# Peterande/SAST

Hardware: AMD Instinct MI355X
Metric: frames/sec (B=4) SAST backbone fwd+bwd, 1Mpx 640x360 (higher is better)
Workload: dtype f32; 1 GPU; 1Mpx 640x360 (padded 384x640) full SAST backbone + PAFPN, fwd+bwd + AdamW, B=4/GPU, binary events (rand>0.5), random-init, AMP=0.0002; global_batch=4, seq_len=1, parallelism=dp1, hipgraph=True, library=sast_amd/libsast_hip.so, product_library=True, segmented_backward_overlap=False, deferred_weight_gradients=False, backward_cuts=3, dw_discard_TIMING_PROBE_gradients_invalid=False, collective_ranks=1, collective_ranks_verified=1, gradient_bytes_per_rank=67663616, sync_batchnorm=False, event_dtype=int32, grads_finite=True

## Files before the change

### include/sast_hip.h

```cpp
#ifndef SAST_HIP_H
#define SAST_HIP_H
#include <stddef.h>
#include <stdint.h>

#ifdef __cplusplus
extern "C" {
#endif

typedef void* sast_stream_t;

enum { SAST_DT_F32 = 0, SAST_DT_I32 = 1, SAST_DT_U8 = 2, SAST_DT_I64 = 3, SAST_DT_I16 = 4, SAST_DT_I8 = 5 };

int sast_version(void);
int sast_mfma_split3(void);

int sast_nzratio(const void* x, int dtype, int B, int Cin, int H, int W, int32_t* cnt_ws, float* r, sast_stream_t stream);
int sast_nzratio_padded(const void* x, int dtype, int B, int Cin, int H, int W, int Hp, int Wp, int32_t* cnt_ws, float* r,
                        sast_stream_t stream);

int sast_input_prep(const void* x, int dtype, int B, int C, int H, int W, int Hp, int Wp, int32_t* ws, float* r, float* y,
                    sast_stream_t stream);
int sast_input_prep_flag(const void* x, int dtype, int B, int C, int H, int W, int Hp, int Wp, int32_t* ws, float* r, float* y,
                         uint32_t* nonexact, sast_stream_t stream);
int sast_input_prep_u8(const uint8_t* x, int B, int C, int H, int W, int Hp, int Wp, int32_t* ws, float* r, uint8_t* y, sast_stream_t stream);

int sast_nchw_to_nhwc(const void* x, int dtype, int B, int C, int H, int W, float* y, sast_stream_t stream);
int sast_nchw_to_nhwc_padded(const void* x, int dtype, int B, int C, int H, int W, int Hp, int Wp, float* y, sast_stream_t stream);
int sast_nhwc_to_nchw(const float* x, int B, int C, int H, int W, float* y, sast_stream_t stream);

int sast_add_rows(const float* x, const float* table, float* y, int rows, int C, int table_rows, sast_stream_t stream);

#define SAST_MEAN_SQUARE_BLOCKS 128
int sast_mean_square_fwd(const float* const* x, const size_t* n, int count, float* partials, sast_stream_t stream);
int sast_mean_square_bwd(const float* const* x, const size_t* n, int count, const float* d_partials, int d_stride, float* const* dx,
                         sast_stream_t stream);
int sast_mask_token_fwd(float* x, const uint8_t* mask, const float* token, const float* pos_emb, int rows, int C, int L, sast_stream_t stream);
int sast_mask_token_bwd(const float* dy, const uint8_t* mask, float* dx, float* d_token, int rows, int C, sast_stream_t stream);

typedef struct SastDownArgs {
  int32_t B, H, W, Cin, Cout, factor;
  const float* x;
  const float* w;
  const float* ln_w; const float* ln_b;
  const float* pe;
  float* conv_out;
  float* mean; float* rstd;
  float* y;
  const float* dy; float* dx;
  float* dw; float* d_ln_w; float* d_ln_b;
  float* ws;
  int32_t x_dtype;
  int32_t no_overlap;
  const uint32_t* x_nonexact;
} SastDownArgs;
int sast_downsample_ln_fwd(const SastDownArgs* a, sast_stream_t stream);
int sast_downsample_ln_bwd(const SastDownArgs* a, sast_stream_t stream);

typedef struct SastScoreArgs {
  int32_t B, L, C, r_stride;
  float amp;
  const float* xp;
  const float* r;
  const float* ws_w; const float* ws_b;
  const float* wc;
  float* scale;
  float* s;
  float* xw;
  float* tok;
  const float* dxw; float* dxp;
  float* d_ws_w; float* d_ws_b; float* d_wc;
  float* ws;
  float* dscale_ws;
} SastScoreArgs;
int sast_score_stp_fwd(const SastScoreArgs* a, sast_stream_t stream);
int sast_score_stp_bwd(const SastScoreArgs* a, sast_stream_t stream);

typedef struct SastSel {
  int32_t* win_keep;
  uint64_t* mask;
  int32_t* K;
  int32_t* row_off;
  int32_t* win_rank;
  int32_t* counts;
  int32_t* tok_slot;
  int32_t* row_tok;
  int32_t* pack_rows;
  int32_t* row_seg;
} SastSel;
int sast_select_packs(const SastSel* sel, int W, int T, sast_stream_t stream);
// ... 30 lines not shown
  float* d_act_w;
} SastMswsaArgs;
size_t sast_mswsa_fused_ws_floats(int C, int inner, int T, int dim_head, int cb_tps);
size_t sast_mswsa_raw_ws_floats(int C, int inner);
size_t sast_mswsa_bwd_ws_floats(int rows, int C, int inner);
int sast_mswsa_fwd(const SastMswsaArgs* a, sast_stream_t stream);
int sast_mswsa_bwd(const SastMswsaArgs* a, sast_stream_t stream);

typedef struct SastLstmArgs {
  int32_t B, L, C;
  const float* x; const float* h0; const float* c0;
  const float* w; const float* b;
  float* h1; float* c1;
  float* gates;
  const float* dh1; const float* dc1;
  float* dx; float* dh0; float* dc0;
  float* dw; float* db;
  float* ws;
  const float* dh1b;
  const float* drop;
} SastLstmArgs;
int sast_lstm_fwd(const SastLstmArgs* a, sast_stream_t stream);
int sast_lstm_bwd(const SastLstmArgs* a, sast_stream_t stream);

int sast_dwconv_fwd(const float* x, const float* w, const float* b, float* y, int B, int H, int W, int C, int k, sast_stream_t stream);
int sast_dwconv_bwd(const float* x, const float* w, const float* dy, float* dx, float* dw, float* db, int B, int H, int W, int C, int k,
                    sast_stream_t stream);

#define SAST_BN_STAT_COPIES 4
#define SAST_BN_WS_FLOATS(Cout) ((4 * SAST_BN_STAT_COPIES + 2 * SAST_BN_STAT_COPIES) * (Cout))
int sast_conv_bn_ws_floats(int Cout);
typedef struct SastConvBnArgs {
  int32_t B, H, W, Cin, Cout, ksize, stride, training;
  int32_t ldx, ldy, lddy, lddx;
  int32_t bn_ws_zeroed;
  int32_t bn_red_done;
  int32_t Cin1, ldx2;
  float momentum, eps;
  const float* x; const float* w; const float* bn_w; const float* bn_b;
  float* run_mean; float* run_var;
  float* conv_out;
  float* stats;
  float* y;
  const float* dy; float* dx; float* dw; float* d_bn_w; float* d_bn_b;
  float* bn_ws;
  float* ws;
  const float* x2;
  float* dx2;
  const float* p_conv_out; const float* p_stats; const float* p_bn_w; const float* p_bn_b; float* p_bn_ws;
  const float* p2_conv_out; const float* p2_stats; const float* p2_bn_w; const float* p2_bn_b; float* p2_bn_ws;
  const float* dy2;
  int32_t sync_phase, m_total;
  int32_t groups;
} SastConvBnArgs;
int sast_conv_bn_silu_fwd(const SastConvBnArgs* a, sast_stream_t stream);
int sast_conv_bn_silu_bwd(const SastConvBnArgs* a, sast_stream_t stream);

typedef struct SastConvBn2Args {
  int32_t B, H, W, Cin, Cout, ldx, Cin1, ldx2;
  int32_t bn_ws_zeroed, bn_red_done0, bn_red_done1;
  int32_t training;
  int32_t ksize;
  float momentum0, momentum1, eps0, eps1;
  const float* x; const float* x2;
  const float* w0; const float* w1; const float* bn_w0; const float* bn_w1; const float* bn_b0; const float* bn_b1;
  float* run_mean0; float* run_mean1; float* run_var0; float* run_var1;
  float* conv_out0; float* conv_out1; float* stats0; float* stats1; float* y0; float* y1; float* bn_ws0; float* bn_ws1;
  const float* dy0; const float* dy1; float* dw0; float* dw1; float* d_bn_w0; float* d_bn_w1; float* d_bn_b0; float* d_bn_b1;
  float* ws0; float* ws1;
  float* dx; float* dx2;
  const float* p_conv_out; const float* p_stats; const float* p_bn_w; const float* p_bn_b; float* p_bn_ws;
  const float* p2_conv_out; const float* p2_stats; const float* p2_bn_w; const float* p2_bn_b; float* p2_bn_ws;
} SastConvBn2Args;
int sast_conv_bn_silu2_fwd(const SastConvBn2Args* a, sast_stream_t stream);
int sast_conv_bn_silu2_bwd(const SastConvBn2Args* a, sast_stream_t stream);

int sast_upsample_cat_fwd(const float* a, const float* b, float* out, int B, int H, int W, int C1, int C2, sast_stream_t stream);
int sast_upsample_cat_bwd(const float* dout, float* da, float* db, int B, int H, int W, int C1, int C2, sast_stream_t stream);
int sast_cat2_fwd(const float* a, const float* b, float* out, int rows, int C1, int C2, sast_stream_t stream);
int sast_cat2_bwd(const float* dout, float* da, float* db, int rows, int C1, int C2, sast_stream_t stream);

typedef struct SastHeadGeom {
  int32_t n_levels;
  int32_t H[4], W[4];
  float stride[4];
} SastHeadGeom;
int sast_head_pred_fwd(const float* reg_feat, const float* cls_feat, const float* w_reg, const float* b_reg, const float* w_obj,
                       const float* b_obj, const float* w_cls, const float* b_cls, float* pred, float* train, int B, int H, int W, int hidden,
                       int num_classes, float stride, int anchor_offset, int anchors_total, int decode, sast_stream_t stream);
int sast_head_pred_decode(const float* reg_feat, const float* cls_feat, const float* w_reg, const float* b_reg, const float* w_obj,
                          const float* b_obj, const float* w_cls, const float* b_cls, float* out, int B, int H, int W, int hidden,
                          int num_classes, float stride, int anchor_offset, int anchors_total, int decode, sast_stream_t stream);
int sast_head_pred_bwd(const float* draw, const float* reg_feat, const float* cls_feat, const float* w_reg, const float* w_obj,
                       const float* w_cls, float* d_reg_feat, float* d_cls_feat, float* dw_reg, float* db_reg, float* dw_obj, float* db_obj,
                       float* dw_cls, float* db_cls, int B, int H, int W, int hidden, int num_classes, int anchor_offset, int anchors_total,
                       sast_stream_t stream);
size_t sast_yolox_loss_ws_bytes(int B, int anchors_total, int max_labels);
int sast_yolox_loss(const float* train_out, const float* labels, const SastHeadGeom* geom, int B, int max_labels, int num_classes, int use_l1,
                    float* losses, float* draw, int32_t* fg_mask, int32_t* matched_gt, float* matched_iou, void* ws, sast_stream_t stream);

size_t sast_postprocess_ws_bytes(int B, int anchors_total);
int sast_postprocess(const float* prediction, int B, int anchors_total, int num_classes, float conf_thre, float nms_thre, int class_agnostic,
                     float* out, int32_t* n_out, void* ws, sast_stream_t stream);

#define SAST_GATHER_MAX_SRC 32
#define SAST_GATHER_MAX_OUT 256
typedef struct {
  int32_t n_src, n_out, B, _pad;
  size_t sample_floats;
  const float* src[SAST_GATHER_MAX_SRC];
  float* dsrc[SAST_GATHER_MAX_SRC];
  float* out;
  uint8_t t_of[SAST_GATHER_MAX_OUT], b_of[SAST_GATHER_MAX_OUT];
} SastSampleGather;
int sast_gather_samples(const SastSampleGather* a, sast_stream_t stream);
int sast_gather_samples_bwd(const SastSampleGather* a, sast_stream_t stream);
typedef struct { uint8_t sel[256]; } SastSampleMask;
int sast_zero_samples(float* x, int B, size_t sample_floats, const SastSampleMask* sel, sast_stream_t stream);

int sast_adamw(float* p, const float* g, float* m, float* v, size_t n,
               const float* lr_step ,
               double beta1, double beta2, float eps, float weight_decay, float grad_scale,
               float clip_value , sast_stream_t stream);
int sast_adamw_onecycle(float* p, const float* g, float* m, float* v, size_t n, float* lr_step, double beta1, double beta2, float eps,
                        float weight_decay, float grad_scale, float clip_value, double initial_lr, double max_lr, double min_lr,
                        double end1, double end2, sast_stream_t stream);

int sast_dw_defer(int on);
int sast_dw_defer_rows(long min_rows, long max_rows);
int sast_dw_pending(void);
int sast_dw_discard(void);
// ... 178 lines not shown
```

### sast_amd/_lib.py

```python
from __future__ import annotations

import ctypes as C
import os
import re

_HERE = os.path.dirname(os.path.abspath(__file__))
DEFAULT_LIB_PATH = os.path.join(_HERE, "libsast_hip.so")
LIB_PATH = os.environ.get("SAST_LIB_PATH") or DEFAULT_LIB_PATH
HEADER_PATH = os.path.join(os.path.dirname(_HERE), "include", "sast_hip.h")

P = C.c_void_p
I32 = C.c_int32
F32 = C.c_float

DT_F32, DT_I32, DT_U8, DT_I64, DT_I16, DT_I8 = 0, 1, 2, 3, 4, 5
EVENT_WINDOW_DURATION, EVENT_WINDOW_COUNT = 0, 1
EVENT_SCAN_BLOCKS = 512
EVQUEUE_DT_DAT = 6
AUGMENT_PARAM_WORDS = 16
AUGMENT_NONE, AUGMENT_ZOOM_IN, AUGMENT_ZOOM_OUT = 0, 1, 2
EVAL_STATE_WORDS, EVAL_MAX_CLASSES = 32, 4
EVAL_IOU_THRS, EVAL_REC_THRS, EVAL_AREAS = 10, 101, 4
(LABELS_UNSORTED, LABELS_NEGATIVE_SIZE, LABELS_NO_LABELS, LABELS_BAD_RATE, LABELS_NO_ALIGNED_LABEL, LABELS_ZERO_COUNT, LABELS_TOO_MANY_FRAMES,
 LABELS_TOO_MANY_WINDOWS, LABELS_FRAME_OVERFULL, LABELS_FRAMES_TOO_CLOSE, LABELS_WINDOW_INDEX) = (1 << k for k in range(11))


def _struct(name, spec):
    fields = []
    for ct, names in spec:
        for n in names.split():
            fields.append((n, ct))
    return type(name, (C.Structure,), {"_fields_": fields})


SastDownArgs = _struct("SastDownArgs", [
    (I32, "B H W Cin Cout factor"),
    (P, "x w ln_w ln_b pe conv_out mean rstd y dy dx dw d_ln_w d_ln_b ws"),
    (I32, "x_dtype no_overlap"),
    (P, "x_nonexact"),
])
SastScoreArgs = _struct("SastScoreArgs", [
    (I32, "B L C r_stride"), (F32, "amp"),
    (P, "xp r ws_w ws_b wc scale s xw tok dxw dxp d_ws_w d_ws_b d_wc ws dscale_ws"),
])
SastSel = _struct("SastSel", [(P, "win_keep mask K row_off win_rank counts tok_slot row_tok pack_rows row_seg")])
SastMswsaArgs = _struct("SastMswsaArgs", [
    (I32, "B H W C ph pw mode inner"), (F32, "eps"), (I32, "cb_tps dim_head mlp_act"),
    (P, "xin out"), (SastSel, "sel"),
    (P, "ln1_w ln1_b ln2_w ln2_b qkv_w qkv_b proj_w proj_b ls1 fc1_w fc1_b fc2_w fc2_b ls2"),
    (P, "mean1 rstd1 mean2 rstd2 S QKV O lse Y UG Hh"),
    (P, "dout dxin"),
    (P, "d_ln1_w d_ln1_b d_ln2_w d_ln2_b d_qkv_w d_qkv_b d_proj_w d_proj_b d_ls1 d_fc1_w d_fc1_b d_fc2_w d_fc2_b d_ls2"),
    (P, "ws cb_m cb_sum raw_ws drop1 drop2 drop_ws drop_mlp fused_ws act_w d_act_w"),
])
SastConvBn2Args = _struct("SastConvBn2Args", [
    (I32, "B H W Cin Cout ldx Cin1 ldx2 bn_ws_zeroed bn_red_done0 bn_red_done1 training ksize"), (F32, "momentum0 momentum1 eps0 eps1"),
    (P, "x x2 w0 w1 bn_w0 bn_w1 bn_b0 bn_b1 run_mean0 run_mean1 run_var0 run_var1 conv_out0 conv_out1 stats0 stats1 y0 y1 "
        "bn_ws0 bn_ws1 dy0 dy1 dw0 dw1 d_bn_w0 d_bn_w1 d_bn_b0 d_bn_b1 ws0 ws1 dx dx2 "
        "p_conv_out p_stats p_bn_w p_bn_b p_bn_ws p2_conv_out p2_stats p2_bn_w p2_bn_b p2_bn_ws"),
])
SastHeadGeom = _struct("SastHeadGeom", [(I32, "n_levels"), (I32 * 4, "H"), (I32 * 4, "W"), (F32 * 4, "stride")])
SastLstmArgs = _struct("SastLstmArgs", [
    (I32, "B L C"),
    (P, "x h0 c0 w b h1 c1 gates dh1 dc1 dx dh0 dc0 dw db ws dh1b drop"),
])
SastConvBnArgs = _struct("SastConvBnArgs", [
    (I32, "B H W Cin Cout ksize stride training ldx ldy lddy lddx bn_ws_zeroed bn_red_done Cin1 ldx2"), (F32, "momentum eps"),
    (P, "x w bn_w bn_b run_mean run_var conv_out stats y dy dx dw d_bn_w d_bn_b bn_ws ws x2 dx2 "
        "p_conv_out p_stats p_bn_w p_bn_b p_bn_ws p2_conv_out p2_stats p2_bn_w p2_bn_b p2_bn_ws dy2"),
    (I32, "sync_phase m_total groups"),
])

SastSampleGather = _struct("SastSampleGather", [
    (I32, "n_src n_out B _pad"), (C.c_size_t, "sample_floats"), (P * 32, "src"), (P * 32, "dsrc"), (P, "out"),
    (C.c_uint8 * 256, "t_of"), (C.c_uint8 * 256, "b_of"),
])
SastSampleMask = _struct("SastSampleMask", [(C.c_uint8 * 256, "sel")])
SastEventArgs = _struct("SastEventArgs", [
    (P, "x y p t bounds out err ws"), (C.c_int64, "capacity window_capacity"),
    (I32, "x_dtype y_dtype p_dtype t_dtype B bins height width count_cutoff fastmode downsample_by_2 clip_negative_polarity"),
])
SastMdStackArgs = _struct("SastMdStackArgs", [
    (P, "x y p t bounds out err ws"), (C.c_int64, "capacity window_capacity"),
    (I32, "x_dtype y_dtype p_dtype t_dtype B bins height width count_cutoff downsample_by_2 clip_negative_polarity"),
])
SastEvQueueArgs = _struct("SastEvQueueArgs", [
    (P, "x y p t head count t_last retired retired_t err ws"), (C.c_int64, "capacity"), (I32, "S reserved"),
])
SastLabelArgs = _struct("SastLabelArgs", [
    (P, "ws ends_us n_windows frame_ts_us n_frames frame_2_window window_2_frame labels frame_start frame_count status"),
    (C.c_int64, "capacity base_delta_us align_t_us delta_t_us"), (I32, "S width height class_max"), (F32, "min_diag2 min_side max_width"),
    (I32, "reprs_per_frame downsample_by_2 max_frames max_windows max_labels_per_frame reserved"),
])
SastEvalArgs = _struct("SastEvalArgs", [
    (P, "labels counts det n_det"), (I32, "N M A K"), (F32, "min_diag2 min_side"), (I32, "max_images max_labels_per_frame"),
    (C.c_int64, "max_detections"),
    (P, "state info gt_box gt_cls gt_img img_t det_box det_cls det_img rec_key rec_match rec_ign iou_thr rec_thr sorted sort_ws"),
    (C.c_size_t, "sort_ws_bytes"), (P, "precision result"),
])

_SIGNATURES = {
    "sast_version": (C.c_int, []),
    "sast_mfma_split3": (C.c_int, []),
    "sast_nzratio": (C.c_int, [P, C.c_int, C.c_int, C.c_int, C.c_int, C.c_int, P, P, P]),
    "sast_nchw_to_nhwc": (C.c_int, [P, C.c_int, C.c_int, C.c_int, C.c_int, C.c_int, P, P]),
    "sast_nzratio_padded": (C.c_int, [P, C.c_int, C.c_int, C.c_int, C.c_int, C.c_int, C.c_int, C.c_int, P, P, P]),
    "sast_nchw_to_nhwc_padded": (C.c_int, [P, C.c_int, C.c_int, C.c_int, C.c_int, C.c_int, C.c_int, C.c_int, P, P]),
    "sast_nhwc_to_nchw": (C.c_int, [P, C.c_int, C.c_int, C.c_int, C.c_int, P, P]),
    "sast_input_prep": (C.c_int, [P] + [C.c_int] * 7 + [P, P, P, P]),
    "sast_input_prep_flag": (C.c_int, [P] + [C.c_int] * 7 + [P, P, P, P, P]),
    "sast_input_prep_u8": (C.c_int, [P] + [C.c_int] * 6 + [P, P, P, P]),
    "sast_add_rows": (C.c_int, [P, P, P, C.c_int, C.c_int, C.c_int, P]),
    "sast_mean_square_fwd": (C.c_int, [P, P, C.c_int, P, P]),
    "sast_mean_square_bwd": (C.c_int, [P, P, C.c_int, P, C.c_int, P, P]),
    "sast_downsample_ln_fwd": (C.c_int, [C.POINTER(SastDownArgs), P]),
    "sast_downsample_ln_bwd": (C.c_int, [C.POINTER(SastDownArgs), P]),
    "sast_score_stp_fwd": (C.c_int, [C.POINTER(SastScoreArgs), P]),
    "sast_score_stp_bwd": (C.c_int, [C.POINTER(SastScoreArgs), P]),
    "sast_select": (C.c_int, [P, C.c_int, C.c_int, C.c_int, C.c_int, C.c_int, C.c_int, C.c_double, C.POINTER(SastSel), P]),
    "sast_select_packs": (C.c_int, [C.POINTER(SastSel), C.c_int, C.c_int, P]),
    "sast_head_pred_decode": (C.c_int, [P] * 9 + [C.c_int] * 5 + [C.c_float, C.c_int, C.c_int, C.c_int, P]),
    "sast_head_pred_fwd": (C.c_int, [P] * 10 + [C.c_int] * 5 + [C.c_float, C.c_int, C.c_int, C.c_int, P]),
    "sast_head_pred_bwd": (C.c_int, [P] * 14 + [C.c_int] * 7 + [P]),
    "sast_postprocess_ws_bytes": (C.c_size_t, [C.c_int, C.c_int]),
    "sast_postprocess": (C.c_int, [P, C.c_int, C.c_int, C.c_int, C.c_float, C.c_float, C.c_int, P, P, P, P]),
    "sast_yolox_loss_ws_bytes": (C.c_size_t, [C.c_int, C.c_int, C.c_int]),
    "sast_yolox_loss": (C.c_int, [P, P, C.POINTER(SastHeadGeom), C.c_int, C.c_int, C.c_int, C.c_int, P, P, P, P, P, P, P]),
    "sast_mask_token_fwd": (C.c_int, [P, P, P, P, C.c_int, C.c_int, C.c_int, P]),
    "sast_mask_token_bwd": (C.c_int, [P, P, P, P, C.c_int, C.c_int, P]),
    "sast_select_pair": (C.c_int, [P, C.c_int, C.c_int, C.c_int, C.c_int, C.c_int, C.c_double, C.POINTER(SastSel), C.POINTER(SastSel), P]),
    "sast_mswsa_bwd_ws_floats": (C.c_size_t, [C.c_int, C.c_int, C.c_int]),
    "sast_mswsa_raw_ws_floats": (C.c_size_t, [C.c_int, C.c_int]),
    "sast_mswsa_fused_ws_floats": (C.c_size_t, [C.c_int] * 5),
    "sast_mswsa_fwd": (C.c_int, [C.POINTER(SastMswsaArgs), P]),
    "sast_mswsa_bwd": (C.c_int, [C.POINTER(SastMswsaArgs), P]),
    "sast_lstm_fwd": (C.c_int, [C.POINTER(SastLstmArgs), P]),
    "sast_lstm_bwd": (C.c_int, [C.POINTER(SastLstmArgs), P]),
    "sast_dwconv_fwd": (C.c_int, [P, P, P, P] + [C.c_int] * 5 + [P]),
    "sast_dwconv_bwd": (C.c_int, [P, P, P, P, P, P] + [C.c_int] * 5 + [P]),
    "sast_conv_bn_ws_floats": (C.c_int, [C.c_int]),
    "sast_conv_bn_silu_fwd": (C.c_int, [C.POINTER(SastConvBnArgs), P]),
    "sast_conv_bn_silu_bwd": (C.c_int, [C.POINTER(SastConvBnArgs), P]),
    "sast_conv_bn_silu2_fwd": (C.c_int, [C.POINTER(SastConvBn2Args), P]),
    "sast_conv_bn_silu2_bwd": (C.c_int, [C.POINTER(SastConvBn2Args), P]),
    "sast_upsample_cat_fwd": (C.c_int, [P, P, P, C.c_int, C.c_int, C.c_int, C.c_int, C.c_int, P]),
    "sast_upsample_cat_bwd": (C.c_int, [P, P, P, C.c_int, C.c_int, C.c_int, C.c_int, C.c_int, P]),
    "sast_cat2_fwd": (C.c_int, [P, P, P, C.c_int, C.c_int, C.c_int, P]),
    "sast_cat2_bwd": (C.c_int, [P, P, P, C.c_int, C.c_int, C.c_int, P]),
    "sast_gather_samples": (C.c_int, [C.POINTER(SastSampleGather), P]),
    "sast_gather_samples_bwd": (C.c_int, [C.POINTER(SastSampleGather), P]),
    "sast_zero_samples": (C.c_int, [P, C.c_int, C.c_size_t, C.POINTER(SastSampleMask), P]),
    "sast_adamw_onecycle": (C.c_int, [P, P, P, P, C.c_size_t, P, C.c_double, C.c_double, F32, F32, F32, F32, C.c_double, C.c_double, C.c_double,
                                      C.c_double, C.c_double, P]),
    "sast_dw_defer": (C.c_int, [C.c_int]),
    "sast_dw_defer_rows": (C.c_int, [C.c_long, C.c_long]),
    "sast_dw_pending": (C.c_int, []),
    "sast_dw_discard": (C.c_int, []),
    "sast_dw_flush": (C.c_int, [P]),
    "sast_launch_count": (C.c_ulonglong, []),
    "sast_config_reload": (C.c_int, []),
    "sast_config_get": (C.c_int, [C.c_char_p, C.c_int]),
    "sast_config_report": (C.c_size_t, [C.c_char_p, C.c_size_t]),
    "sast_prof_enable": (C.c_int, [C.c_int]),
    "sast_prof_calibrate": (C.c_float, [P, C.c_int]),
    "sast_prof_report": (C.c_size_t, [C.c_char_p, C.c_size_t]),
    "sast_adamw": (C.c_int, [P, P, P, P, C.c_size_t, P, C.c_double, C.c_double, F32, F32, F32, F32, P]),
    "sast_event_correct_time": (C.c_int, [P, C.c_int, P, C.c_int64, P, P, P, P]),
    "sast_event_window_bounds": (C.c_int, [P, P, C.c_int64, P, C.c_int, C.c_int, C.c_int64, P, P]),
    "sast_event_frames_ws_bytes": (C.c_size_t, [C.c_int] * 5 + [C.c_int64]),
    "sast_event_frames": (C.c_int, [C.POINTER(SastEventArgs), P]),
    "sast_mdstack_frames_ws_bytes": (C.c_size_t, [C.c_int] * 5 + [C.c_int64]),
    "sast_mdstack_frames": (C.c_int, [C.POINTER(SastMdStackArgs), P]),
    "sast_evstreams_ws_count": (C.c_size_t, [C.c_int]),
    "sast_evstreams_correct_time": (C.c_int, [P, C.c_int, P, C.c_int, C.c_int64, P, P, P, P, P]),
    "sast_evstreams_window_bounds": (C.c_int, [P, P, C.c_int, C.c_int64, P, C.c_int, C.c_int, C.c_int64, P, P]),
    "sast_evqueue_ws_count": (C.c_size_t, [C.c_int]),
    "sast_evqueue_push": (C.c_int, [C.POINTER(SastEvQueueArgs), P, P, P, P, C.c_int, C.c_int, C.c_int, C.c_int, P, C.c_int64, P, P]),
    "sast_evqueue_window_bounds": (C.c_int, [C.POINTER(SastEvQueueArgs), P, C.c_int, C.c_int, C.c_int64, P, P]),
    "sast_evqueue_retire": (C.c_int, [C.POINTER(SastEvQueueArgs), P, C.c_int, P]),
    "sast_labels_ws_bytes": (C.c_size_t, [C.c_int, C.c_int64, C.c_int]),
    "sast_labels_load": (C.c_int, [C.POINTER(SastLabelArgs), P, P, P, P]),
    "sast_labels_gather": (C.c_int, [C.POINTER(SastLabelArgs), P, C.c_int, P, P, P, P, P]),
    "sast_augment_frames": (C.c_int, [P, P, P] + [C.c_int] * 5 + [P]),
    "sast_augment_labels": (C.c_int, [P, P, P] + [C.c_int] * 4 + [P, P, P, P]),
    "sast_eval_reset": (C.c_int, [C.POINTER(SastEvalArgs), P]),
    "sast_eval_add": (C.c_int, [C.POINTER(SastEvalArgs), P]),
    "sast_eval_sort_ws_bytes": (C.c_size_t, [C.c_int64]),
    "sast_eval_accumulate": (C.c_int, [C.POINTER(SastEvalArgs), P]),
}

_lib = None


def declared_symbols():
    with open(HEADER_PATH) as f:
        src = f.read()
    return sorted(set(re.findall(r"\b(sast_[a-z0-9_]+)\s*\(", src)))


# ... 57 lines not shown
```

### sast_amd/csrc/gemm.cuh

```cuda
#pragma once
#include <type_traits>
#include <hip/hip_ext.h>
#include "common.cuh"
#include "../../include/sast_hip.h"

#if defined(SAST_TL_ENABLE) && !defined(SAST_TL)
static __device__ unsigned long long sast_tl_buf[8 * 8192];
#define SAST_TL(k)                                                                                          \
  do {                                                                                                      \
    const unsigned bid_ = blockIdx.x;                                                                       \
    if (threadIdx.x == 0 && bid_ < 8192) sast_tl_buf[bid_ * 8 + (k)] = wall_clock64();                      \
    if (threadIdx.x == 0 && bid_ < 8192 && (k) == 0) sast_tl_buf[bid_ * 8 + 7] = __smid();                 \
  } while (0)
#define SAST_TL_JOB(j) do { if (threadIdx.x == 0 && blockIdx.x < 8192) sast_tl_buf[blockIdx.x * 8 + 6] = (j); } while (0)
#endif
#ifndef SAST_TL
#define SAST_TL(k)
#endif
#ifndef SAST_TL_JOB
#define SAST_TL_JOB(j)
#endif
#ifndef SAST_TLF
#define SAST_TLF_DECL
#define SAST_TLF(k)
// ... 1480 lines not shown
};
struct EpStoreStats2 {
  static constexpr bool COLSTATS = true;
  float* c1; float* c2; int C; double* sums1; double* sums2;
  using Col = EpNone; using Aux = EpNone;
  __device__ __forceinline__ Col col(int) const { return Col{}; }
  __device__ __forceinline__ Aux pre(int, int) const { return Aux{}; }
  __device__ __forceinline__ void post(int m, int j, const float (&v)[1], const Col&, const Aux&) const {
    if (j < C) c1[(size_t)m * C + j] = v[0];
    else c2[(size_t)m * C + (j - C)] = v[0];
  }
  __device__ __forceinline__ void stat(float v, const Col&, const Aux&, float& a, float& b) const { a += v; b += v * v; }
  __device__ __forceinline__ void flush(int copy, int j, int, float s, float q) const {
    double* sp = (j < C ? sums1 : sums2) + (size_t)copy * 2 * C;
    const int jj = j < C ? j : j - C;
    atomicAdd(sp + jj, (double)s); atomicAdd(sp + C + jj, (double)q);
  }
};
struct EpAtomic2 {
  float* c1; float* c2; int ldc; int M1;
  using Col = EpNone; using Aux = EpNone;
  __device__ __forceinline__ Col col(int) const { return Col{}; }
  __device__ __forceinline__ Aux pre(int, int) const { return Aux{}; }
  __device__ __forceinline__ void post(int m, int j, const float (&v)[1], const Col&, const Aux&) const {
    atomicAdd((m < M1 ? c1 + (size_t)m * ldc : c2 + (size_t)(m - M1) * ldc) + j, v[0]);
  }
};
struct EpAtomic {
  float* c; int ldc;
  using Col = EpNone; using Aux = EpNone;
  __device__ __forceinline__ Col col(int) const { return Col{}; }
  __device__ __forceinline__ Aux pre(int, int) const { return Aux{}; }
  __device__ __forceinline__ void post(int m, int j, const float (&v)[1], const Col&, const Aux&) const {
    atomicAdd(c + (size_t)m * ldc + j, v[0]);
  }
};

struct EpStoreClass {
  float* c; int ldc; int H, W; ConvDxClasses k;
  using Col = EpNone;
  struct Aux { int p; };
  __device__ __forceinline__ Col col(int) const { return Col{}; }
  __device__ __forceinline__ Aux pre(int m, int) const {
    const int cls = fast_div(m, k.Mc, k.mc_mul), ic = m - cls * k.Mc;
    const int t = fast_div(ic, k.Wc, k.wc_mul), xx = ic - t * k.Wc, b = fast_div(t, k.Hc, k.hc_mul), yy = t - b * k.Hc;
    const int q = 3 - cls;
    return Aux{(b * H + 2 * yy + (q >> 1)) * W + 2 * xx + (q & 1)};
  }
  __device__ __forceinline__ void post(int, int j, const float (&v)[1], const Col&, const Aux& a) const {
    c[(size_t)a.p * ldc + j] = v[0];
  }
};

struct EpSplit2BnRed {
  static constexpr bool COLSTATS = true;
  float* a; float* b; int C1, C2; BnProducer pa, pb;
  using Col = BnCol;
  struct Aux { float x; };
  __device__ __forceinline__ Col col(int j) const {
    if (j < C1) return pa.x ? bn_col(pa, j) : BnCol{0.f, 0.f, 0.f, 0.f};
    return pb.x ? bn_col(pb, j - C1) : BnCol{0.f, 0.f, 0.f, 0.f};
  }
  __device__ __forceinline__ Aux pre(int m, int j) const {
    if (j < C1) return Aux{pa.x ? pa.x[(size_t)m * C1 + j] : 0.f};
    return Aux{pb.x ? pb.x[(size_t)m * C2 + (j - C1)] : 0.f};
  }
  __device__ __forceinline__ void post(int m, int j, const float (&v)[1], const Col&, const Aux&) const {
    if (j < C1) a[(size_t)m * C1 + j] = v[0];
    else if (b) b[(size_t)m * C2 + (j - C1)] = v[0];
  }
  __device__ __forceinline__ void stat(float v, const Col& k, const Aux& x, float& s, float& q) const { bn_stat(v, x.x, k, s, q); }
  __device__ __forceinline__ void flush(int copy, int j, int, float s, float q) const {
    if (j < C1) {
      if (pa.x) { float* sp = pa.sums + (size_t)copy * 2 * C1; atomicAdd(sp + j, s); atomicAdd(sp + C1 + j, q); }
    } else if (pb.x) {
      float* sp = pb.sums + (size_t)copy * 2 * C2; atomicAdd(sp + (j - C1), s); atomicAdd(sp + C2 + (j - C1), q);
    }
  }
};

struct EpSplit2 {
  float* a; float* b; int C1, C2;
  using Col = EpNone; using Aux = EpNone;
  __device__ __forceinline__ Col col(int) const { return Col{}; }
  __device__ __forceinline__ Aux pre(int, int) const { return Aux{}; }
  __device__ __forceinline__ void post(int m, int j, const float (&v)[1], const Col&, const Aux&) const {
    if (j < C1) a[(size_t)m * C1 + j] = v[0];
    else if (b) b[(size_t)m * C2 + (j - C1)] = v[0];
  }
};

}
```

### sast_amd/csrc/k_block.hip

```cpp
#include <cstdlib>
#include "gemm_dispatch.cuh"
#include "kernels.h"

using namespace sast;

namespace {

constexpr int ATTN_MAX_T = 256;

struct EpBiasRelu {
  float* c; int ldc; const float* bias;
  struct Col { float b; };
  using Aux = EpNone;
  __device__ __forceinline__ Col col(int j) const { return Col{bias[j]}; }
  __device__ __forceinline__ Aux pre(int, int) const { return Aux{}; }
  __device__ __forceinline__ void post(int m, int j, const float (&v)[1], const Col& k, const Aux&) const {
    c[(size_t)m * ldc + j] = fmaxf(v[0] + k.b, 0.f);
  }
};
struct EpBiasReluCtl : EpBiasRelu {
  static constexpr bool SIDE = true;
  ControlsJob k; int side_blocks;
  __device__ __forceinline__ void side(int sb) const { if (threadIdx.x < 256) controls_fwd_elem(k, sb * 256 + threadIdx.x); }
};
// ... 150 lines not shown
extern "C" {

int sast_version(void) { SAST_ENTRY(); return 100; }
int sast_mfma_split3(void) { SAST_ENTRY(); return SAST_MFMA_BF16 ? 2 : SAST_MFMA_SPLIT3; }

int sast_nzratio(const void* x, int dtype, int B, int Cin, int H, int W, int32_t* cnt_ws, float* r, sast_stream_t stream) { SAST_ENTRY();
  if (!x || !cnt_ws || !r || H % 32 || W % 32) return SAST_EINVAL;
  return nzr_dispatch(x, dtype, cnt_ws, r, B, Cin, H, W, H, W, (hipStream_t)stream);
}
int sast_nzratio_padded(const void* x, int dtype, int B, int Cin, int H, int W, int Hp, int Wp, int32_t* cnt_ws, float* r,
                        sast_stream_t stream) { SAST_ENTRY();
  if (!x || !cnt_ws || !r || Hp % 32 || Wp % 32 || H > Hp || W > Wp || H % 4 || W % 4) return SAST_EINVAL;
  return nzr_dispatch(x, dtype, cnt_ws, r, B, Cin, H, W, Hp, Wp, (hipStream_t)stream);
}
int sast_nchw_to_nhwc(const void* x, int dtype, int B, int C, int H, int W, float* y, sast_stream_t stream) { SAST_ENTRY();
  return nchw_to_nhwc_dispatch(x, dtype, y, B, C, H, W, H, W, (hipStream_t)stream);
}
int sast_nchw_to_nhwc_padded(const void* x, int dtype, int B, int C, int H, int W, int Hp, int Wp, float* y, sast_stream_t stream) { SAST_ENTRY();
  if (!x || !y || H > Hp || W > Wp) return SAST_EINVAL;
  return nchw_to_nhwc_dispatch(x, dtype, y, B, C, H, W, Hp, Wp, (hipStream_t)stream);
}
int sast_input_prep(const void* x, int dtype, int B, int C, int H, int W, int Hp, int Wp, int32_t* ws, float* r, float* y, sast_stream_t stream) { SAST_ENTRY();
  if (!x || !ws || !r || !y || H > Hp || W > Wp || H % 4 || W % 4 || Hp % 32 || Wp % 32 || C != 20 || ((Hp / 32) * (Wp / 32)) % 2) return SAST_EINVAL;
  return input_prep_dispatch(x, dtype, y, ws, r, B, C, H, W, Hp, Wp, (hipStream_t)stream);
}
int sast_input_prep_flag(const void* x, int dtype, int B, int C, int H, int W, int Hp, int Wp, int32_t* ws, float* r, float* y, uint32_t* nonexact,
                         sast_stream_t stream) { SAST_ENTRY();
  if (!x || !ws || !r || !y || !nonexact || H > Hp || W > Wp || H % 4 || W % 4 || Hp % 32 || Wp % 32 || C != 20 || ((Hp / 32) * (Wp / 32)) % 2) return SAST_EINVAL;
  return input_prep_dispatch(x, dtype, y, ws, r, B, C, H, W, Hp, Wp, (hipStream_t)stream, nonexact);
}
int sast_input_prep_u8(const uint8_t* x, int B, int C, int H, int W, int Hp, int Wp, int32_t* ws, float* r, uint8_t* y, sast_stream_t stream) { SAST_ENTRY();
  if (!x || !ws || !r || !y || H > Hp || W > Wp || H % 4 || W % 4 || Hp % 32 || Wp % 32 || C != 20 || ((Hp / 32) * (Wp / 32)) % 2) return SAST_EINVAL;
  return input_prep_u8(x, y, ws, r, B, C, H, W, Hp, Wp, (hipStream_t)stream);
}
int sast_nhwc_to_nchw(const float* x, int B, int C, int H, int W, float* y, sast_stream_t stream) { SAST_ENTRY();
  return nhwc_to_nchw_launch(x, y, B, C, H * W, (hipStream_t)stream);
}

int sast_add_rows(const float* x, const float* table, float* y, int rows, int C, int table_rows, sast_stream_t stream) { SAST_ENTRY();
  if (C % 4) return SAST_EINVAL;
  return add_rows_launch(x, table, y, rows, C, table_rows, (hipStream_t)stream);
}

int sast_mean_square_fwd(const float* const* x, const size_t* n, int count, float* partials, sast_stream_t stream) { SAST_ENTRY();
  if (!x || !n || !partials || count < 1 || count > 4) return SAST_EINVAL;
  for (int t = 0; t < count; ++t) if (!x[t] || n[t] % 4) return SAST_EINVAL;
  return mean_square_launch(x, nullptr, n, count, SAST_MEAN_SQUARE_BLOCKS, partials, nullptr, 1, (hipStream_t)stream);
}
int sast_mean_square_bwd(const float* const* x, const size_t* n, int count, const float* d_partials, int d_stride, float* const* dx,
                         sast_stream_t stream) { SAST_ENTRY();
  if (!x || !n || !d_partials || !dx || count < 1 || count > 4 || (d_stride != 0 && d_stride != 1)) return SAST_EINVAL;
  for (int t = 0; t < count; ++t) if (!x[t] || !dx[t] || n[t] % 4) return SAST_EINVAL;
  return mean_square_launch(x, dx, n, count, SAST_MEAN_SQUARE_BLOCKS, nullptr, d_partials, d_stride, (hipStream_t)stream);
}

int sast_mask_token_fwd(float* x, const uint8_t* mask, const float* token, const float* pos_emb, int rows, int C, int L, sast_stream_t stream) { SAST_ENTRY();
  if (!x || !mask || !token || C % 4 || L < 1) return SAST_EINVAL;
  return mask_token_fwd_launch(x, mask, token, pos_emb, rows, C, L, (hipStream_t)stream);
}
int sast_gather_samples(const SastSampleGather* a, sast_stream_t stream) { SAST_ENTRY();
  if (!a || !a->out || a->n_src < 1 || a->n_src > SAST_GATHER_MAX_SRC || a->n_out < 0 || a->n_out > SAST_GATHER_MAX_OUT || a->sample_floats % 4) return SAST_EINVAL;
  for (int j = 0; j < a->n_out; ++j) if (a->t_of[j] >= a->n_src || a->b_of[j] >= a->B || !a->src[a->t_of[j]]) return SAST_EINVAL;
  if (a->n_out == 0) return SAST_OK;
  return sample_gather_launch(*a, false, (hipStream_t)stream);
}
int sast_gather_samples_bwd(const SastSampleGather* a, sast_stream_t stream) { SAST_ENTRY();
  if (!a || a->n_src < 1 || a->n_src > SAST_GATHER_MAX_SRC || a->n_out < 0 || a->n_out > SAST_GATHER_MAX_OUT || a->B < 1 || a->B > 256 ||
      a->sample_floats % 4 || (a->n_out && !a->out)) return SAST_EINVAL;
  for (int t = 0; t < a->n_src; ++t) if (!a->dsrc[t]) return SAST_EINVAL;
  return sample_gather_launch(*a, true, (hipStream_t)stream);
}
int sast_zero_samples(float* x, int B, size_t sample_floats, const SastSampleMask* sel, sast_stream_t stream) { SAST_ENTRY();
  if (!x || !sel || B < 1 || B > 256 || sample_floats % 4) return SAST_EINVAL;
  return zero_samples_launch(x, B, sample_floats, *sel, (hipStream_t)stream);
}
int sast_mask_token_bwd(const float* dy, const uint8_t* mask, float* dx, float* d_token, int rows, int C, sast_stream_t stream) { SAST_ENTRY();
  if (!dy || !mask || !dx || !d_token || C % 4) return SAST_EINVAL;
  return mask_token_bwd_launch(dy, mask, dx, d_token, rows, C, (hipStream_t)stream);
}

int sast_select(const float* tok, int B, int H, int W, int ph, int pw, int mode, double bounce, const SastSel* s,
                sast_stream_t stream) { SAST_ENTRY();
  if (!tok || !s) return SAST_EINVAL;
  const int N = (H / ph) * (W / pw), T = ph * pw;
  const float thr_w = (float)((1.0 / N) / (1.0 + bounce));
  const float thr_t = (float)((1.0 / T) / (1.0 + bounce));
  return select_launch(tok, B, H, W, ph, pw, mode, thr_w, thr_t, s, (hipStream_t)stream);
}
int sast_select_packs(const SastSel* s, int W, int T, sast_stream_t stream) { SAST_ENTRY();
  if (!s || !s->K || !s->row_off || !s->pack_rows || !s->row_seg || W < 1 || T < 1 || T > ATTN_MAX_T) return SAST_EINVAL;
  return select_packs_launch(s, W, T, (hipStream_t)stream);
}

int sast_select_pair(const float* tok, int B, int H, int W, int ph, int pw, double bounce, const SastSel* win, const SastSel* grid,
                     sast_stream_t stream) { SAST_ENTRY();
  if (!tok || !win || !grid) return SAST_EINVAL;
  const int N = (H / ph) * (W / pw), T = ph * pw;
  const float thr_w = (float)((1.0 / N) / (1.0 + bounce));
  const float thr_t = (float)((1.0 / T) / (1.0 + bounce));
  return select_pair_launch(tok, B, H, W, ph, pw, thr_w, thr_t, win, grid, (hipStream_t)stream);
}

int sast_score_stp_fwd(const SastScoreArgs* a, sast_stream_t stream) { SAST_ENTRY();
  hipStream_t st = (hipStream_t)stream;
  ProfScope ps_("score_fwd", a ? a->C : 0, a ? a->B * a->L : 0, st);
  if (!a || a->C % 4) return SAST_EINVAL;
// ... 243 lines not shown
```

### sast_amd/csrc/k_conv.hip

```cpp
#include <cstdlib>
#include "gemm_dispatch.cuh"
#include "kernels.h"

using namespace sast;

namespace {

inline double bn_unbias(long M) { return M > 1 ? (double)M / (double)(M - 1) : 1.0; }
struct BnFwdJob {
  const float* x; const double* sums; float* run_mean; float* run_var; float* stats; const float* gamma; const float* beta;
  float* y; int ldy; float momentum, eps;
};
__global__ __launch_bounds__(256) void bn_silu_apply_kernel(BnFwdJob j0, BnFwdJob j1, double invM, double unbias, size_t n4, int C, int training, int iters,
                                                            unsigned c4_mul) {
  SAST_KERNARG_WARM_SELF(bn_silu_apply_kernel);
  const BnFwdJob& jb = blockIdx.y == 0 ? j0 : j1;
  const float* __restrict__ x = jb.x; const double* __restrict__ sums = jb.sums;
  float* __restrict__ run_mean = jb.run_mean; float* __restrict__ run_var = jb.run_var; float* __restrict__ stats = jb.stats;
  const float* __restrict__ gamma = jb.gamma; const float* __restrict__ beta = jb.beta; float* __restrict__ y = jb.y;
  const int ldy = jb.ldy; const float momentum = jb.momentum, eps = jb.eps;
  extern __shared__ float bn_sm[];
  const int c4 = C / 4;
  const size_t e0 = (size_t)blockIdx.x * 256 * iters + threadIdx.x;
#ifndef SAST_BN_EARLY_LOADS
#define SAST_BN_EARLY_LOADS 0
#endif
  float4 v0 = zero4(), g0 = zero4(), b0 = zero4();
  size_t m0 = 0; int cc0 = 0;
  if (SAST_BN_EARLY_LOADS) {
    const size_t ec = e0 < n4 ? e0 : 0;
    m0 = fast_div((int)ec, c4, c4_mul); cc0 = (int)(ec - m0 * c4) * 4;
    v0 = ld4(x + m0 * C + cc0); g0 = ld4(gamma + cc0); b0 = ld4(beta + cc0);
  }
  for (int c = threadIdx.x; c < C; c += 256) {
    float mu, rs;
    if (training) {
      double sk[BN_STAT_COPIES], qk[BN_STAT_COPIES];
#pragma unroll
      for (int k = 0; k < BN_STAT_COPIES; ++k) { sk[k] = sums[(size_t)k * 2 * C + c]; qk[k] = sums[(size_t)k * 2 * C + C + c]; }
      double s = 0.0, q = 0.0;
#pragma unroll
      for (int k = 0; k < BN_STAT_COPIES; ++k) { s += sk[k]; q += qk[k]; }
      const double mean = s * invM;
      double var = q * invM - mean * mean;
      if (var < 0) var = 0;
      mu = (float)mean;
#if SAST_FAST_DIV
      rs = rsqrt_hw((float)var + eps);
#else
      rs = (float)(1.0 / sqrt(var + (double)eps));
#endif
      if (blockIdx.x == 0 && run_mean) {
        const double unb = var * unbias;
        run_mean[c] = (1.f - momentum) * run_mean[c] + momentum * (float)mean;
        run_var[c] = (1.f - momentum) * run_var[c] + momentum * (float)unb;
      }
    } else {
      mu = run_mean[c];
      rs = rsqrt_hw(run_var[c] + eps);
    }
    if (blockIdx.x == 0) { stats[c] = mu; stats[C + c] = rs; }
    bn_sm[c] = mu; bn_sm[C + c] = rs;
  }
  __syncthreads();
  for (int it = 0; it < iters; ++it) {
    const size_t e = e0 + (size_t)it * 256;
    if (e >= n4) return;
    size_t m; int c; float4 v, g, b;
    if (SAST_BN_EARLY_LOADS && it == 0) { m = m0; c = cc0; v = v0; g = g0; b = b0; }
    else { m = fast_div((int)e, c4, c4_mul); c = (int)(e - m * c4) * 4; v = ld4(x + m * C + c); g = ld4(gamma + c); b = ld4(beta + c); }
    const float4 mu = *(const float4*)(bn_sm + c), rs = *(const float4*)(bn_sm + C + c);
    float4 z = make_float4((v.x - mu.x) * rs.x * g.x + b.x, (v.y - mu.y) * rs.y * g.y + b.y, (v.z - mu.z) * rs.z * g.z + b.z,
                           (v.w - mu.w) * rs.w * g.w + b.w);
    z.x *= sigmoid_hw(z.x); z.y *= sigmoid_hw(z.y); z.z *= sigmoid_hw(z.z); z.w *= sigmoid_hw(z.w);
    st4(y + m * ldy + c, z);
  }
}
struct EpBnSilu {
  float* y; int ldy; const float* run_mean; const float* run_var; const float* gamma; const float* beta; float eps;
  struct Col { float mu, rs, g, b; };
  using Aux = EpNone;
  __device__ __forceinline__ Col col(int j) const { return Col{run_mean[j], 1.0f / sqrtf(run_var[j] + eps), gamma[j], beta[j]}; }
  __device__ __forceinline__ Aux pre(int, int) const { return Aux{}; }
  __device__ __forceinline__ void post(int m, int j, const float (&v)[1], const Col& k, const Aux&) const {
    const float z = (v[0] - k.mu) * k.rs * k.g + k.b;
    y[(size_t)m * ldy + j] = z * sigmoid_hw(z);
  }
};
struct EpBnSilu2 {
  float* y0; float* y1; int C; const float* rm0; const float* rv0; const float* g0; const float* b0; float eps0;
  const float* rm1; const float* rv1; const float* g1; const float* b1; float eps1;
  struct Col { float mu, rs, g, b; };
  using Aux = EpNone;
  __device__ __forceinline__ Col col(int j) const {
    return j < C ? Col{rm0[j], 1.0f / sqrtf(rv0[j] + eps0), g0[j], b0[j]} : Col{rm1[j - C], 1.0f / sqrtf(rv1[j - C] + eps1), g1[j - C], b1[j - C]};
  }
  __device__ __forceinline__ Aux pre(int, int) const { return Aux{}; }
  __device__ __forceinline__ void post(int m, int j, const float (&v)[1], const Col& k, const Aux&) const {
    const float z = (v[0] - k.mu) * k.rs * k.g + k.b;
    (j < C ? y0 + (size_t)m * C + j : y1 + (size_t)m * C + (j - C))[0] = z * sigmoid_hw(z);
  }
};
__global__ __launch_bounds__(256) void bn_stats_kernel(const float* __restrict__ x, int M, int C, double* __restrict__ sums,
                                                       int rows_per_block) {
  extern __shared__ double redd[];
  const int c4n = C / 4;
  const int RP = 256 / c4n > 0 ? 256 / c4n : 1;
  const int r0 = blockIdx.x * rows_per_block, r1 = min(M, r0 + rows_per_block);
  for (int cq = threadIdx.x % min(c4n, 256); cq < c4n; cq += 256) {
    const int rl = threadIdx.x / c4n, c = cq * 4;
    double s[4] = {0, 0, 0, 0}, q[4] = {0, 0, 0, 0};
    if (rl < RP) {
      for (int r = r0 + rl; r < r1; r += RP) {
        const float4 v = ld4(x + (size_t)r * C + c);
        s[0] += v.x; s[1] += v.y; s[2] += v.z; s[3] += v.w;
        q[0] += (double)v.x * v.x; q[1] += (double)v.y * v.y; q[2] += (double)v.z * v.z; q[3] += (double)v.w * v.w;
      }
#pragma unroll
      for (int e = 0; e < 4; ++e) { redd[((rl * C) + c + e) * 2] = s[e]; redd[((rl * C) + c + e) * 2 + 1] = q[e]; }
    }
    __syncthreads();
    if (rl == 0) {
#pragma unroll
      for (int e = 0; e < 4; ++e) {
        double a = s[e], b = q[e];
        for (int k = 1; k < RP; ++k) { a += redd[((k * C) + c + e) * 2]; b += redd[((k * C) + c + e) * 2 + 1]; }
        atomicAdd(sums + c + e, a);
        atomicAdd(sums + C + c + e, b);
// ... 109 lines not shown
  }
}
__global__ __launch_bounds__(256) void bn_publish_affine_kernel(const float* __restrict__ sums, float* __restrict__ dgamma, float* __restrict__ dbeta, int C) {
  const int c = blockIdx.x * 256 + threadIdx.x;
  if (c >= C) return;
  float s1 = 0.f, s2 = 0.f;
#pragma unroll
  for (int k = 0; k < BN_STAT_COPIES; ++k) { s1 += sums[(size_t)k * 2 * C + c]; s2 += sums[(size_t)k * 2 * C + C + c]; }
  dbeta[c] += s1;
  dgamma[c] += s2;
}
template <class IDX>
__global__ __launch_bounds__(256) void upsample_cat_fwd_kernel(const float* __restrict__ a, const float* __restrict__ b,
                                                               float* __restrict__ out, int H, int W, int C1, int C2, size_t n4) {
  const size_t e64 = (size_t)blockIdx.x * 256 + threadIdx.x;
  if (e64 >= n4) return;
  const IDX e = (IDX)e64;
  const int Ct = C1 + C2;
  const IDX c4n = (IDX)(Ct / 4);
  const IDX row = e / c4n; const int c = (int)(e - row * c4n) * 4;
  float4 v;
  if (c < C1) {
    const IDX W2 = (IDX)(2 * W), H2 = (IDX)(2 * H);
    const IDX t = row / W2; const int x = (int)(row - t * W2); const IDX bb = t / H2; const int y = (int)(t - bb * H2);
    v = ld4(a + (((size_t)bb * H + (y >> 1)) * W + (x >> 1)) * C1 + c);
  } else {
    v = ld4(b + (size_t)row * C2 + (c - C1));
  }
  st4(out + (size_t)row * Ct + c, v);
}
template <class IDX>
__global__ __launch_bounds__(256) void upsample_cat_bwd_kernel(const float* __restrict__ dout, float* __restrict__ da, float* __restrict__ db,
                                                               int H, int W, int C1, int Ct, size_t n4, size_t n4b) {
  const size_t e64 = (size_t)blockIdx.x * 256 + threadIdx.x;
  if (e64 >= n4) {
    const size_t eb64 = e64 - n4;
    if (eb64 >= n4b) return;
    const IDX eb = (IDX)eb64;
    const int C2 = Ct - C1;
    const IDX c4b = (IDX)(C2 / 4);
    const IDX row = eb / c4b; const int c = (int)(eb - row * c4b) * 4;
    st4(db + (size_t)row * C2 + c, ld4(dout + (size_t)row * Ct + C1 + c));
    return;
  }
  const IDX e = (IDX)e64;
  const IDX c4n = (IDX)(C1 / 4);
  const IDX row = e / c4n; const int c = (int)(e - row * c4n) * 4;
  const IDX t = row / (IDX)W; const int x = (int)(row - t * (IDX)W); const IDX bb = t / (IDX)H; const int y = (int)(t - bb * (IDX)H);
  const size_t base = (((size_t)bb * 2 * H + 2 * y) * 2 * W + 2 * x);
  const float4 p = ld4(dout + base * Ct + c), q = ld4(dout + (base + 1) * Ct + c);
  const float4 r = ld4(dout + (base + 2 * W) * Ct + c), s = ld4(dout + (base + 2 * W + 1) * Ct + c);
  st4(da + (size_t)row * C1 + c, make_float4((p.x + q.x) + (r.x + s.x), (p.y + q.y) + (r.y + s.y), (p.z + q.z) + (r.z + s.z), (p.w + q.w) + (r.w + s.w)));
}
__global__ __launch_bounds__(256) void slice_copy_kernel(const float* __restrict__ src, int lds, int soff, float* __restrict__ dst,
                                                         int ldd, int doff, int Cs, size_t n4) {
  const size_t e = (size_t)blockIdx.x * 256 + threadIdx.x;
  if (e >= n4) return;
  const int c4n = Cs / 4;
  const size_t row = e / c4n; const int c = (int)(e % c4n) * 4;
  st4(dst + row * ldd + doff + c, ld4(src + row * lds + soff + c));
}
int slice_copy(const float* src, int lds, int soff, float* dst, int ldd, int doff, int Cs, size_t rows, hipStream_t st) {
  const size_t n4 = rows * (Cs / 4);
  if (!n4) return SAST_OK;
  SAST_LAUNCH(slice_copy_kernel, dim3((unsigned)((n4 + 255) / 256)), dim3(256), 0, st, src, lds, soff, dst, ldd, doff, Cs, n4);
  SAST_CHECK_LAUNCH();
  return SAST_OK;
}

struct OneCycle { int on; double initial_lr, max_lr, min_lr, end1, end2; };
__global__ __launch_bounds__(256) void adamw_kernel(float* __restrict__ p, const float* __restrict__ g, float* __restrict__ m,
                                                    float* __restrict__ v, size_t n4, const float* __restrict__ lr_step, double b1d,
                                                    double b2d, float eps, float wd, float gscale, float clip, OneCycle oc) {
  SAST_KERNARG_WARM_SELF(adamw_kernel);
  __shared__ float s_bc[3];
  if (threadIdx.x == 0) {
    const double step = (double)lr_step[1];
    s_bc[0] = (float)(1.0 - pow(b1d, step));
    s_bc[1] = (float)sqrt(1.0 - pow(b2d, step));
    double lr = (double)lr_step[0];
    if (oc.on) {
      const double sn = step - 1.0;
      if (sn <= oc.end1) lr = oc.initial_lr + (oc.max_lr - oc.initial_lr) * (oc.end1 > 0.0 ? sn / oc.end1 : 1.0);
      else lr = oc.max_lr + (oc.min_lr - oc.max_lr) * ((sn - oc.end1) / (oc.end2 - oc.end1));
    }
    s_bc[2] = (float)lr;
  }
  __syncthreads();
  const size_t e = (size_t)blockIdx.x * 256 + threadIdx.x;
  if (e >= n4) return;
  const float lr = s_bc[2];
  const float bc1 = s_bc[0], bc2s = s_bc[1];
  const float b1 = (float)b1d, b2 = (float)b2d, omb1 = (float)(1.0 - b1d), omb2 = (float)(1.0 - b2d);
  float4 pv = ld4(p + e * 4), gv = ld4(g + e * 4), mv = ld4(m + e * 4), vv = ld4(v + e * 4);
  float* pp = &pv.x; float* gp = &gv.x; float* mp = &mv.x; float* vp = &vv.x;
#pragma unroll
  for (int k = 0; k < 4; ++k) {
    float gr = gp[k] * gscale;
    if (clip > 0.f) gr = fminf(fmaxf(gr, -clip), clip);
    pp[k] *= 1.f - lr * wd;
    mp[k] = b1 * mp[k] + omb1 * gr;
    vp[k] = b2 * vp[k] + omb2 * gr * gr;
    const float denom = sqrtf(vp[k]) / bc2s + eps;
    pp[k] -= (lr / bc1) * (mp[k] / denom);
  }
  st4(p + e * 4, pv); st4(m + e * 4, mv); st4(v + e * 4, vv);
}

void bn_bwd_reduce_launch(const BnBwdJob& j0, const BnBwdJob& j1, int njobs, int M, int C, hipStream_t st) {
  const int target = SAST_KNOB("SAST_BN_BLOCKS", 32);
  int rpb = (M + target - 1) / target;
  rpb = rpb < 8 ? 8 : (rpb > 512 ? 512 : rpb);
  const int c4n = C / 4, RP = BN_RED_THREADS / c4n > 0 ? BN_RED_THREADS / c4n : 1;
  SAST_LAUNCH(bn_bwd_reduce_kernel, dim3((M + rpb - 1) / rpb, njobs), dim3(BN_RED_THREADS), sizeof(float4) * 2 * RP * c4n, st, j0, j1, M, C,
                     rpb);
}
void bn_bwd_apply_launch(const BnBwdJob& j0, const BnBwdJob& j1, int njobs, int M, int C, int training, hipStream_t st, int m_stat = 0) {
  const size_t n4 = (size_t)M * (C / 4);
  int iters = (int)(n4 / (256 * 512));
  iters = iters < 1 ? 1 : (iters > 8 ? 8 : iters);
  SAST_LAUNCH(bn_bwd_apply_kernel, dim3((unsigned)((n4 + 256 * iters - 1) / (256 * iters)), njobs), dim3(256), sizeof(float) * 6 * C, st,
                     j0, j1, n4, C, 1.0f / (float)(m_stat > 0 ? m_stat : M), training, iters, div_mul_of((unsigned)(C / 4), n4));
}

inline ConvGeom geom_of(int B, int H, int W, int Cin, int k, int stride, int pad, int replicate, int ldx) {
  ConvGeom g;
  g.B = B; g.H = H; g.W = W; g.Cin = Cin; g.KH = k; g.KW = k; g.stride = stride; g.pad = pad; g.replicate = replicate; g.ldx = ldx;
  g.Ho = (H + 2 * pad - k) / stride + 1;
  g.Wo = (W + 2 * pad - k) / stride + 1;
  g.stride_shift = pow2_shift(stride);
  g.kw_mul = small_div_mul(k);
  const unsigned long long rows = (unsigned long long)B * g.Ho * g.Wo;
  g.wo_mul = div_mul_of((unsigned)g.Wo, rows);
  g.ho_mul = div_mul_of((unsigned)g.Ho, rows);
  g.cin_mul = div_mul_of((unsigned)Cin, (unsigned long long)k * k * Cin);
  g.w_mul = div_mul_of((unsigned)W, (unsigned long long)B * H * W);
  g.h_mul = div_mul_of((unsigned)H, (unsigned long long)B * H * W);
  return g;
}

template <class LB, class EP>
int conv_gemm(const float* x, const ConvGeom& g, const LB& lb, const EP& ep, int M, int NJ, int K, hipStream_t st) {
  if (!g.cin_mul) return SAST_EINVAL;
  if (g.Cin % 16 == 0) return gemm_auto(LdIm2colU{{x, g}}, lb, ep, M, NJ, K, st);
  return gemm_auto(LdIm2col{x, g}, lb, ep, M, NJ, K, st);
}

int conv_bwd_pair(const float* dconv, const float* x, const ConvGeom& g, int Cout, const float* w, float* dw, float* dx, int lddx,
                  hipStream_t st, const BnProducer* prod = nullptr) {
  const int k = g.KH, K = k * k * g.Cin, M = g.B * g.Ho * g.Wo;
  const unsigned shift = div_mul_of((unsigned)Cout, (unsigned long long)k * k * Cout);
  if (!shift || !g.cin_mul || g.stride_shift < 0) return SAST_EINVAL;
  const LdRowsT ta{dconv, Cout};
  const LdIm2colT tb{x, g};
  if (!dx) return gemm_tn(ta, tb, dw, K, Cout, K, M, st);
  const int parity = SAST_KNOB("SAST_CONVDX_PARITY", 1);
  const int Mc = g.B * (g.H / 2) * (g.W / 2);
  if (prod && prod->x) {
    if (g.stride != 1 || lddx != g.Cin || prod->C != g.Cin) return SAST_EINVAL;
    if (Cout % 16 == 0)
      return gemm_pair(ta, tb, dw, K, Cout, K, M, nullptr, nullptr, LdConvDxU{{dconv, g, Cout, Cout, shift}},
                       LdWeightConvDxU{{w, Cout, k * k, g.Cin, shift}}, EpStoreBnRed{dx, lddx, *prod}, g.B * g.H * g.W, g.Cin, k * k * Cout, nullptr, st, pair_tn_blocks_conv());
    return gemm_pair(ta, tb, dw, K, Cout, K, M, nullptr, nullptr, LdConvDx{dconv, g, Cout, Cout, shift},
                     LdWeightConvDx{w, Cout, k * k, g.Cin, shift}, EpStoreBnRed{dx, lddx, *prod}, g.B * g.H * g.W, g.Cin, k * k * Cout, nullptr, st, pair_tn_blocks_conv());
  }
  if (!(parity && g.stride == 2 && k == 3 && g.pad == 1 && g.H % 2 == 0 && g.W % 2 == 0 && Mc % 64 == 0)) {
    if (Cout % 16 == 0)
      return gemm_pair(ta, tb, dw, K, Cout, K, M, nullptr, nullptr, LdConvDxU{{dconv, g, Cout, Cout, shift}},
                       LdWeightConvDxU{{w, Cout, k * k, g.Cin, shift}}, EpStore{dx, lddx, nullptr}, g.B * g.H * g.W, g.Cin, k * k * Cout, nullptr, st, pair_tn_blocks_conv());
    return gemm_pair(ta, tb, dw, K, Cout, K, M, nullptr, nullptr, LdConvDx{dconv, g, Cout, Cout, shift},
                     LdWeightConvDx{w, Cout, k * k, g.Cin, shift}, EpStore{dx, lddx, nullptr}, g.B * g.H * g.W, g.Cin, k * k * Cout, nullptr, st, pair_tn_blocks_conv());
  }
  ConvDxClasses c;
  c.Hc = g.H / 2; c.Wc = g.W / 2; c.Mc = Mc;
  c.mc_mul = div_mul_of((unsigned)c.Mc, 4ull * Mc); c.wc_mul = div_mul_of((unsigned)c.Wc, 4ull * Mc); c.hc_mul = div_mul_of((unsigned)c.Hc, 4ull * Mc);
  for (int cls = 0; cls < 4; ++cls) {
    const int py = (3 - cls) >> 1, px = (3 - cls) & 1;
    int ty[2] = {15, 15}, tx[2] = {15, 15}, ny = 0, nx = 0;
    for (int kk = 0; kk < k; ++kk) {
      if ((py + g.pad - kk) % 2 == 0 || (g.replicate && py == 0 && kk < g.pad)) ty[ny++] = kk;
      if ((px + g.pad - kk) % 2 == 0 || (g.replicate && px == 0 && kk < g.pad)) tx[nx++] = kk;
    }
    c.kh_pack[cls] = c.kw_pack[cls] = 0;
    int slot = 0;
    for (int pass = 0; pass < 2; ++pass)
      for (int a = 0; a < 2; ++a)
        for (int b = 0; b < 2; ++b) {
          const bool used = ty[a] != 15 && tx[b] != 15;
          if (used != (pass == 0)) continue;
          c.kh_pack[cls] |= (unsigned)(used ? ty[a] : 15) << (4 * slot);
          c.kw_pack[cls] |= (unsigned)(used ? tx[b] : 15) << (4 * slot);
          ++slot;
        }
    c.nslot[cls] = ny * nx;
  }
  return gemm_pair(ta, tb, dw, K, Cout, K, M, nullptr, nullptr, LdConvDxP{dconv, g, Cout, Cout, shift, c},
                   LdWeightConvDxP{w, Cout, k * k, g.Cin, shift, g.KW, c}, EpStoreClass{dx, lddx, g.H, g.W, c}, 4 * Mc, g.Cin, 4 * Cout,
                   nullptr, st, pair_tn_blocks_conv());
}

inline bool stem_exact_bf16() { return SAST_KNOB("SAST_STEM_EXACT_BF16", 1) != 0; }
bool down_size_ok(const SastDownArgs* a) {
  if (a->factor < 1 || a->B < 1 || a->H < a->factor || a->W < a->factor) return false;
  return a->no_overlap || (a->H % a->factor == 0 && a->W % a->factor == 0);
}

}

extern "C" {

int sast_downsample_ln_fwd(const SastDownArgs* a, sast_stream_t stream) { SAST_ENTRY();
  hipStream_t st = (hipStream_t)stream;
  ProfScope ps_("down_fwd", a ? a->Cout : 0, a ? a->B * a->H * a->W : 0, st);
  if (!a || a->Cin % 4 || a->Cout % 4 || !down_size_ok(a)) return SAST_EINVAL;
  const int k = a->no_overlap ? a->factor : 2 * a->factor - 1;
  const ConvGeom g = geom_of(a->B, a->H, a->W, a->Cin, k, a->factor, a->no_overlap ? 0 : a->factor - 1, 1, a->Cin);
  const int M = a->B * g.Ho * g.Wo, K = k * k * a->Cin;
  int rc;
  const bool exact_ok = stem_exact_bf16();
  if (a->x_dtype == SAST_DT_U8 && exact_ok)
    rc = !g.cin_mul ? SAST_EINVAL : gemm_auto(LdIm2colQ8X{{(const unsigned char*)a->x, g}}, LdWeightNT{a->w, K, 0}, EpStore{a->conv_out, a->Cout, nullptr}, M, a->Cout, K, st);
  else if (a->x_dtype == SAST_DT_U8)
    rc = !g.cin_mul ? SAST_EINVAL : gemm_auto(LdIm2colQ8{(const unsigned char*)a->x, g}, LdWeightNT{a->w, K, 0}, EpStore{a->conv_out, a->Cout, nullptr}, M, a->Cout, K, st);
  else if (a->x_dtype != SAST_DT_F32) return SAST_EINVAL;
  else if (a->x_nonexact && exact_ok && g.Cin % 16)
    rc = !g.cin_mul ? SAST_EINVAL : gemm_auto(LdIm2colX{{a->x, g}, a->x_nonexact}, LdWeightNT{a->w, K, 0}, EpStore{a->conv_out, a->Cout, nullptr}, M, a->Cout, K, st);
  else rc = conv_gemm(a->x, g, LdWeightNT{a->w, K, 0}, EpStore{a->conv_out, a->Cout, nullptr}, M, a->Cout, K, st);
  if (rc) return rc;
  return ln_fwd_launch(a->conv_out, a->y, a->ln_w, a->ln_b, a->pe, g.Ho * g.Wo, a->mean, a->rstd, M, a->Cout, 1e-5f, st);
}

int sast_downsample_ln_bwd(const SastDownArgs* a, sast_stream_t stream) { SAST_ENTRY();
  hipStream_t st = (hipStream_t)stream;
  ProfScope ps_("down_bwd", a->Cout, a->B * a->H * a->W, st);
  if (a->Cin % 4 || a->Cout % 4 || !down_size_ok(a) || (a->x_dtype == SAST_DT_U8 && a->dx)) return SAST_EINVAL;
  const int k = a->no_overlap ? a->factor : 2 * a->factor - 1;
  const ConvGeom g = geom_of(a->B, a->H, a->W, a->Cin, k, a->factor, a->no_overlap ? 0 : a->factor - 1, 1, a->Cin);
  const int M = a->B * g.Ho * g.Wo, K = k * k * a->Cin;
  float* dconv = a->ws;
  int rc = ln_bwd_launch(a->conv_out, a->dy, a->ln_w, a->mean, a->rstd, dconv, a->d_ln_w, a->d_ln_b, M, a->Cout, st);
  if (rc) return rc;
  if (a->x_dtype == SAST_DT_U8) {
    if (a->dx || !g.cin_mul) return SAST_EINVAL;
    if (stem_exact_bf16()) return gemm_tn(LdRowsT{dconv, a->Cout}, LdIm2colTQ8X{{(const unsigned char*)a->x, g}}, a->dw, K, a->Cout, K, M, st);
    return gemm_tn(LdRowsT{dconv, a->Cout}, LdIm2colTQ8{(const unsigned char*)a->x, g}, a->dw, K, a->Cout, K, M, st);
  }
  if (a->x_dtype != SAST_DT_F32) return SAST_EINVAL;
  if (a->x_nonexact && !a->dx && stem_exact_bf16() && g.Cin % 16) {
// ... 21 lines not shown
  if (phase < 0 || phase > 2 || (phase == 2 && a->m_total < M)) return SAST_EINVAL;
  if (a->training && !a->bn_ws_zeroed && phase != 2) zero_fill(a->bn_ws, sizeof(float) * SAST_BN_WS_FLOATS(C), st);
  int rc = SAST_OK;
  const int sep = SAST_KNOB("SAST_BN_STATS_SEPARATE", 0);
  const bool one = k == 1 && a->stride == 1;
  if (a->x2 && (!one || a->Cin1 % 4 || a->Cin1 <= 0 || a->Cin1 >= a->Cin)) return SAST_EINVAL;
  const LdRows2 la2{a->x, a->ldx, a->Cin1, a->x2, a->ldx2};
  if (!a->training && !a->conv_out) {
    if (!a->run_mean || !a->run_var) return SAST_EINVAL;
    if (dw) {
      if (a->ldy != C) return SAST_EINVAL;
      const DwBnSilu bn{a->run_mean, a->run_var, a->bn_w, a->bn_b, a->eps};
      rc = dwconv_fwd_launch(a->x, a->w, nullptr, a->y, a->B, dg, &bn, st);
      if (rc) return rc;
      SAST_CHECK_LAUNCH();
      return SAST_OK;
    }
    const EpBnSilu ep{a->y, a->ldy, a->run_mean, a->run_var, a->bn_w, a->bn_b, a->eps};
    return one ? (a->x2 ? gemm_auto(la2, LdWeightNT{a->w, K, 0}, ep, M, C, K, st)
                        : gemm_auto(LdRows{a->x, a->ldx, nullptr}, LdWeightNT{a->w, K, 0}, ep, M, C, K, st))
               : conv_gemm(a->x, g, LdWeightNT{a->w, K, 0}, ep, M, C, K, st);
  }
  if (phase == 2) {
  } else if (dw) {
    rc = dwconv_fwd_launch(a->x, a->w, nullptr, a->conv_out, a->B, dg, nullptr, st);
    if (!rc && a->training) {
      int rpb = (M + 127) / 128;
      rpb = rpb < 8 ? 8 : rpb;
      const int c4n = C / 4, RP = 256 / c4n > 0 ? 256 / c4n : 1;
      SAST_LAUNCH(bn_stats_kernel, dim3((M + rpb - 1) / rpb), dim3(256), sizeof(double) * 2 * RP * C, st, a->conv_out, M, C, sums, rpb);
    }
  } else if (a->training && !sep) {
    const EpStoreStats ep{a->conv_out, C, sums};
    rc = one ? (a->x2 ? gemm_auto(la2, LdWeightNT{a->w, K, 0}, ep, M, C, K, st)
                      : gemm_auto(LdRows{a->x, a->ldx, nullptr}, LdWeightNT{a->w, K, 0}, ep, M, C, K, st))
             : conv_gemm(a->x, g, LdWeightNT{a->w, K, 0}, ep, M, C, K, st);
  } else {
    const EpStore ep{a->conv_out, C, nullptr};
    rc = one ? (a->x2 ? gemm_auto(la2, LdWeightNT{a->w, K, 0}, ep, M, C, K, st)
                      : gemm_auto(LdRows{a->x, a->ldx, nullptr}, LdWeightNT{a->w, K, 0}, ep, M, C, K, st))
             : conv_gemm(a->x, g, LdWeightNT{a->w, K, 0}, ep, M, C, K, st);
  }
  if (rc) return rc;
  if (a->training && sep && phase != 2 && !dw) {
    int rpb = (M + sep - 1) / sep;
    rpb = rpb < 8 ? 8 : rpb;
    const int c4n = C / 4, RP = 256 / c4n > 0 ? 256 / c4n : 1;
    SAST_LAUNCH(bn_stats_kernel, dim3((M + rpb - 1) / rpb), dim3(256), sizeof(double) * 2 * RP * C, st, a->conv_out, M, C, sums, rpb);
  }
  if (phase == 1) { SAST_CHECK_LAUNCH(); return SAST_OK; }
  const size_t n4 = (size_t)M * (C / 4);
  int iters = (int)(n4 / (256 * 512));
  iters = iters < 1 ? 1 : (iters > 8 ? 8 : iters);
  {
    const BnFwdJob jb{a->conv_out, sums, a->run_mean, a->run_var, a->stats, a->bn_w, a->bn_b, a->y, a->ldy, a->momentum, a->eps};
    SAST_LAUNCH(bn_silu_apply_kernel, dim3((unsigned)((n4 + 256 * iters - 1) / (256 * iters)), 1), dim3(256), sizeof(float) * 2 * C, st,
                       jb, jb, 1.0 / (double)(phase == 2 ? a->m_total : M), bn_unbias(phase == 2 ? a->m_total : M), n4, C, a->training, iters,
                       div_mul_of((unsigned)(C / 4), n4));
  }
  SAST_CHECK_LAUNCH();
  return SAST_OK;
}

int sast_conv_bn_silu_bwd(const SastConvBnArgs* a, sast_stream_t stream) { SAST_ENTRY();
  hipStream_t st = (hipStream_t)stream;
  ProfScope ps_("convbn_bwd", a->Cout * 10 + a->ksize, a->B * a->H * a->W, st);
  const int k = a->ksize, pad = (k - 1) / 2;
  const ConvGeom g = geom_of(a->B, a->H, a->W, a->Cin, k, a->stride, pad, 0, a->ldx);
  const int M = a->B * g.Ho * g.Wo, K = k * k * a->Cin, C = a->Cout;
  float* sums = a->bn_ws + 4 * BN_STAT_COPIES * C;
  float* dconv = a->ws;
  const int phase = a->training ? a->sync_phase : 0;
  if (phase < 0 || phase > 2 || (phase == 2 && a->m_total < M)) return SAST_EINVAL;
  if (!a->bn_ws_zeroed && phase != 2) {
    if (a->bn_red_done) return SAST_EINVAL;
    zero_fill(sums, sizeof(float) * 2 * BN_STAT_COPIES * C, st);
  }
  const BnBwdJob jb{a->conv_out, a->stats, a->bn_w, a->bn_b, a->dy, a->lddy, sums, dconv, a->d_bn_w, a->d_bn_b, a->dy2, C};
  if (!a->bn_red_done && phase != 2) bn_bwd_reduce_launch(jb, jb, 1, M, C, st);
  if (phase == 1) {
    if (a->d_bn_w && a->d_bn_b) SAST_LAUNCH(bn_publish_affine_kernel, dim3((C + 255) / 256), dim3(256), 0, st, sums, a->d_bn_w, a->d_bn_b, C);
    SAST_CHECK_LAUNCH();
    return SAST_OK;
  }
  bn_bwd_apply_launch(jb, jb, 1, M, C, a->training, st, phase == 2 ? a->m_total : 0);
  SAST_CHECK_LAUNCH();
  const int C2 = a->Cin - a->Cin1;
  BnProducer p1{a->p_conv_out, a->p_stats, a->p_bn_w, a->p_bn_b, a->p_bn_ws ? a->p_bn_ws + 4 * BN_STAT_COPIES * a->Cin1 : nullptr, a->Cin1};
  BnProducer p2{a->p2_conv_out, a->p2_stats, a->p2_bn_w, a->p2_bn_b, a->p2_bn_ws ? a->p2_bn_ws + 4 * BN_STAT_COPIES * C2 : nullptr, C2};
  const bool fold = a->training && a->dx && (p1.x || p2.x);
  if (a->groups > 1) {
    if (a->groups != a->Cin || a->Cin != C || a->x2 || fold || a->ldx != a->Cin || (a->dx && a->lddx != a->Cin)) return SAST_EINVAL;
    int rc = dwconv_bwd_launch(a->x, a->w, dconv, a->dx, a->dw, nullptr, a->B, DwGeom{a->H, a->W, g.Ho, g.Wo, C, k, a->stride}, st);
    if (rc) return rc;
    SAST_CHECK_LAUNCH();
    return SAST_OK;
  }
  if (fold && (a->stride != 1 || (p1.x && !(p1.stats && p1.gamma && p1.beta && p1.sums)) || (p2.x && !(a->x2 && p2.stats && p2.gamma && p2.beta && p2.sums))))
    return SAST_EINVAL;
  if (k == 1 && a->stride == 1 && a->x2) {
    const LdRowsT2 tb{a->x, a->ldx, a->Cin1, a->x2, a->ldx2};
    if (!a->dx) return gemm_tn(LdRowsT{dconv, C}, tb, a->dw, K, C, K, M, st);
    if (a->lddx != a->Cin1) return SAST_EINVAL;
    if (fold) {
      if ((p1.x && a->ldx != a->Cin1) || (p2.x && (a->ldx2 != C2 || !a->dx2))) return SAST_EINVAL;
      return gemm_pair(LdRowsT{dconv, C}, tb, a->dw, K, C, K, M, nullptr, nullptr, LdRows{dconv, C, nullptr}, LdWeightNN{a->w, K},
                       EpSplit2BnRed{a->dx, a->dx2, a->Cin1, C2, p1, p2}, M, a->Cin, C, nullptr, st, pair_tn_blocks_1x1());
    }
    return gemm_pair(LdRowsT{dconv, C}, tb, a->dw, K, C, K, M, nullptr, nullptr,
                     LdRows{dconv, C, nullptr}, LdWeightNN{a->w, K}, EpSplit2{a->dx, a->dx2, a->Cin1, C2}, M, a->Cin, C, nullptr, st, pair_tn_blocks_1x1());
  }
  if (k == 1 && a->stride == 1) {
    if (!a->dx) return gemm_tn(LdRowsT{dconv, C}, LdRowsT{a->x, a->ldx}, a->dw, K, C, K, M, st);
    if (fold) {
      if (a->lddx != a->Cin || a->ldx != a->Cin) return SAST_EINVAL;
      return gemm_pair(LdRowsT{dconv, C}, LdRowsT{a->x, a->ldx}, a->dw, K, C, K, M, nullptr, nullptr, LdRows{dconv, C, nullptr},
                       LdWeightNN{a->w, K}, EpStoreBnRed{a->dx, a->lddx, p1}, M, a->Cin, C, nullptr, st, pair_tn_blocks_1x1());
    }
    return gemm_pair(LdRowsT{dconv, C}, LdRowsT{a->x, a->ldx}, a->dw, K, C, K, M, nullptr, nullptr,
                     LdRows{dconv, C, nullptr}, LdWeightNN{a->w, K}, EpStore{a->dx, a->lddx, nullptr}, M, a->Cin, C, nullptr, st, pair_tn_blocks_1x1());
  }
  return conv_bwd_pair(dconv, a->x, g, C, a->w, a->dw, a->dx, a->lddx, st, fold ? &p1 : nullptr);
}

int sast_conv_bn_silu2_fwd(const SastConvBn2Args* a, sast_stream_t stream) { SAST_ENTRY();
  hipStream_t st = (hipStream_t)stream;
  if (!a || a->Cin % 4 || a->Cout % 4 || a->Cin1 % 4 || a->Cin1 <= 0 || a->Cin1 > a->Cin || (a->Cin1 < a->Cin && !a->x2)) return SAST_EINVAL;
  ProfScope ps_("convbn2_fwd", a->Cout * 10 + 1, a->B * a->H * a->W, st);
  const int M = a->B * a->H * a->W, C = a->Cout;
  if (!a->training) {
    if (!a->run_mean0 || !a->run_var0 || !a->run_mean1 || !a->run_var1 || (a->ksize != 1 && a->ksize != 3)) return SAST_EINVAL;
    const EpBnSilu2 ep{a->y0, a->y1, C, a->run_mean0, a->run_var0, a->bn_w0, a->bn_b0, a->eps0, a->run_mean1, a->run_var1, a->bn_w1, a->bn_b1, a->eps1};
    if (a->ksize == 3) {
      if (a->Cin1 != a->Cin) return SAST_EINVAL;
      const ConvGeom g = geom_of(a->B, a->H, a->W, a->Cin, 3, 1, 1, 0, a->ldx);
      return conv_gemm(a->x, g, LdWeightNT2{a->w0, a->w1, 9 * a->Cin, C}, ep, M, 2 * C, 9 * a->Cin, st);
    }
    return gemm_auto(LdRows2{a->x, a->ldx, a->Cin1, a->Cin1 < a->Cin ? a->x2 : nullptr, a->ldx2}, LdWeightNT2{a->w0, a->w1, a->Cin, C}, ep, M,
                     2 * C, a->Cin, st);
  }
  if (a->ksize != 1 && !(a->ksize == 3 && a->Cin1 == a->Cin)) return SAST_EINVAL;
  const int K = a->ksize * a->ksize * a->Cin;
  if (!a->bn_ws_zeroed) {
    zero_fill(a->bn_ws0, sizeof(float) * SAST_BN_WS_FLOATS(C), st);
    zero_fill(a->bn_ws1, sizeof(float) * SAST_BN_WS_FLOATS(C), st);
  }
  const LdRows2 la{a->x, a->ldx, a->Cin1, a->Cin1 < a->Cin ? a->x2 : nullptr, a->ldx2};
  const EpStoreStats2 ep{a->conv_out0, a->conv_out1, C, (double*)a->bn_ws0, (double*)a->bn_ws1};
  int rc = a->ksize == 3 ? conv_gemm(a->x, geom_of(a->B, a->H, a->W, a->Cin, 3, 1, 1, 0, a->ldx), LdWeightNT2{a->w0, a->w1, K, C}, ep, M,
                                     2 * C, K, st)
                         : gemm_auto(la, LdWeightNT2{a->w0, a->w1, K, C}, ep, M, 2 * C, K, st);
// ... 34 lines not shown
  const EpAtomic2 ep1{a->dw0, a->dw1, K, C};
  BnProducer p1{a->p_conv_out, a->p_stats, a->p_bn_w, a->p_bn_b, a->p_bn_ws ? a->p_bn_ws + 4 * BN_STAT_COPIES * a->Cin1 : nullptr, a->Cin1};
  if (a->ksize == 3) {
    const ConvGeom g = geom_of(a->B, a->H, a->W, a->Cin, 3, 1, 1, 0, a->ldx);
    const LdIm2colT tbc{a->x, g};
    if (!a->dx) return launch_gemm_split<TileSplitR>(ta, tbc, ep1, 2 * C, K, M, nullptr, tn_splits(2 * C, K, M), nullptr, st);
    const unsigned shift = div_mul_of((unsigned)(2 * C), 9ull * 2 * C);
    if (!shift || !g.cin_mul) return SAST_EINVAL;
    const LdConvDx lac{dconv, g, 2 * C, 2 * C, shift};
    const LdWeightConvDx2 lbc{a->w0, a->w1, 2 * C, C, 9, a->Cin, shift};
    if (p1.x) {
      if (a->ldx != a->Cin || !(p1.stats && p1.gamma && p1.beta && p1.sums)) return SAST_EINVAL;
      return gemm_pair_ep(ta, tbc, ep1, 2 * C, K, M, nullptr, nullptr, lac, lbc, EpStoreBnRed{a->dx, a->Cin, p1}, M, a->Cin, 9 * 2 * C, nullptr, st,
                          pair_tn_blocks_conv());
    }
    return gemm_pair_ep(ta, tbc, ep1, 2 * C, K, M, nullptr, nullptr, lac, lbc, EpStore{a->dx, a->Cin, nullptr}, M, a->Cin, 9 * 2 * C, nullptr, st,
                        pair_tn_blocks_conv());
  }
  const LdRowsT2 tb{a->x, a->ldx, a->Cin1, C2 > 0 ? a->x2 : nullptr, a->ldx2};
  if (!a->dx) return launch_gemm_split<TileSplitR>(ta, tb, ep1, 2 * C, K, M, nullptr, tn_splits(2 * C, K, M), nullptr, st);
  if (C2 > 0 && !a->dx2) return SAST_EINVAL;
  const LdRows la{dconv, 2 * C, nullptr};
  const LdWeightNN2 lb{a->w0, a->w1, K, C};
  BnProducer p2{a->p2_conv_out, a->p2_stats, a->p2_bn_w, a->p2_bn_b, a->p2_bn_ws ? a->p2_bn_ws + 4 * BN_STAT_COPIES * C2 : nullptr, C2};
  if (p1.x || p2.x) {
    if ((p1.x && (a->ldx != a->Cin1 || !(p1.stats && p1.gamma && p1.beta && p1.sums))) ||
        (p2.x && (C2 <= 0 || a->ldx2 != C2 || !(p2.stats && p2.gamma && p2.beta && p2.sums))))
      return SAST_EINVAL;
    return gemm_pair_ep(ta, tb, ep1, 2 * C, K, M, nullptr, nullptr, la, lb, EpSplit2BnRed{a->dx, a->dx2, a->Cin1, C2, p1, p2}, M, K, 2 * C,
                        nullptr, st, pair_tn_blocks_1x1());
  }
  return gemm_pair_ep(ta, tb, ep1, 2 * C, K, M, nullptr, nullptr, la, lb, EpSplit2{a->dx, a->dx2, a->Cin1, C2}, M, K, 2 * C, nullptr, st, pair_tn_blocks_1x1());
}

int sast_upsample_cat_fwd(const float* a, const float* b, float* out, int B, int H, int W, int C1, int C2, sast_stream_t stream) { SAST_ENTRY();
  if (C1 % 4 || C2 % 4) return SAST_EINVAL;
  const size_t n4 = (size_t)B * 4 * H * W * ((C1 + C2) / 4);
  if (n4 < (1ull << 32)) SAST_LAUNCH(upsample_cat_fwd_kernel<unsigned>, dim3((unsigned)((n4 + 255) / 256)), dim3(256), 0, (hipStream_t)stream, a, b, out, H, W, C1, C2, n4);
  else SAST_LAUNCH(upsample_cat_fwd_kernel<size_t>, dim3((unsigned)((n4 + 255) / 256)), dim3(256), 0, (hipStream_t)stream, a, b, out, H, W, C1, C2, n4);
  SAST_CHECK_LAUNCH();
  return SAST_OK;
}
int sast_upsample_cat_bwd(const float* dout, float* da, float* db, int B, int H, int W, int C1, int C2, sast_stream_t stream) { SAST_ENTRY();
  hipStream_t st = (hipStream_t)stream;
  if (C1 % 4 || C2 % 4) return SAST_EINVAL;
  const size_t n4 = (size_t)B * H * W * (C1 / 4), n4b = (size_t)B * 4 * H * W * (C2 / 4);
  if (n4 + n4b < (1ull << 32)) SAST_LAUNCH(upsample_cat_bwd_kernel<unsigned>, dim3((unsigned)((n4 + n4b + 255) / 256)), dim3(256), 0, st, dout, da, db, H, W, C1, C1 + C2, n4,
                     n4b);
  else SAST_LAUNCH(upsample_cat_bwd_kernel<size_t>, dim3((unsigned)((n4 + n4b + 255) / 256)), dim3(256), 0, st, dout, da, db, H, W, C1, C1 + C2, n4,
                     n4b);
  SAST_CHECK_LAUNCH();
  return SAST_OK;
}
int sast_cat2_fwd(const float* a, const float* b, float* out, int rows, int C1, int C2, sast_stream_t stream) { SAST_ENTRY();
  hipStream_t st = (hipStream_t)stream;
  if (C1 % 4 || C2 % 4) return SAST_EINVAL;
  int rc = slice_copy(a, C1, 0, out, C1 + C2, 0, C1, rows, st);
  if (rc) return rc;
  return slice_copy(b, C2, 0, out, C1 + C2, C1, C2, rows, st);
}
int sast_cat2_bwd(const float* dout, float* da, float* db, int rows, int C1, int C2, sast_stream_t stream) { SAST_ENTRY();
  hipStream_t st = (hipStream_t)stream;
  int rc = slice_copy(dout, C1 + C2, 0, da, C1, 0, C1, rows, st);
  if (rc) return rc;
  return slice_copy(dout, C1 + C2, C1, db, C2, 0, C2, rows, st);
}

int sast_adamw(float* p, const float* g, float* m, float* v, size_t n, const float* lr_step, double beta1, double beta2, float eps,
               float weight_decay, float grad_scale, float clip_value, sast_stream_t stream) { SAST_ENTRY();
  if (n % 4) return SAST_EINVAL;
  const size_t n4 = n / 4;
  SAST_LAUNCH(adamw_kernel, dim3((unsigned)((n4 + 255) / 256)), dim3(256), 0, (hipStream_t)stream, p, g, m, v, n4, lr_step, beta1,
                     beta2, eps, weight_decay, grad_scale, clip_value, OneCycle{0, 0, 0, 0, 0, 0});
  SAST_CHECK_LAUNCH();
  return SAST_OK;
}
int sast_adamw_onecycle(float* p, const float* g, float* m, float* v, size_t n, float* lr_step, double beta1, double beta2, float eps,
                        float weight_decay, float grad_scale, float clip_value, double initial_lr, double max_lr, double min_lr,
                        double end1, double end2, sast_stream_t stream) { SAST_ENTRY();
  if (n % 4 || !(end2 > end1)) return SAST_EINVAL;
  const size_t n4 = n / 4;
  const OneCycle oc{1, initial_lr, max_lr, min_lr, end1, end2};
  SAST_LAUNCH(adamw_kernel, dim3((unsigned)((n4 + 255) / 256)), dim3(256), 0, (hipStream_t)stream, p, g, m, v, n4, lr_step, beta1,
                     beta2, eps, weight_decay, grad_scale, clip_value, oc);
  SAST_CHECK_LAUNCH();
  return SAST_OK;
}

#ifdef SAST_TL_ENABLE
int sast_tl_reset(void) { SAST_ENTRY();
  static unsigned long long zeros[8 * 8192];
  return hipMemcpyToSymbol(HIP_SYMBOL(sast_tl_buf), zeros, sizeof(zeros)) == hipSuccess ? 0 : -5;
}
int sast_tl_read(unsigned long long* host_out, int nblocks) { SAST_ENTRY();
  if (nblocks > 8192) nblocks = 8192;
  return hipMemcpyFromSymbol(host_out, HIP_SYMBOL(sast_tl_buf), sizeof(unsigned long long) * 8 * nblocks) == hipSuccess ? 0 : -5;
}
#endif

}
```

### sast_amd/csrc/k_rows.hip

```cpp
#include <cstdlib>
#include "common.cuh"
#include "kernels.h"

namespace sast {

__global__ __launch_bounds__(256) void zero_fill_kernel(float* __restrict__ p, size_t n) {
  const size_t i = (size_t)blockIdx.x * 256 + threadIdx.x;
  if (i < n) p[i] = 0.f;
}
int zero_fill(void* p, size_t bytes, hipStream_t st) {
  const size_t n = (bytes + 3) / 4;
  if (!n) return SAST_OK;
  SAST_LAUNCH(zero_fill_kernel, dim3((unsigned)((n + 255) / 256)), dim3(256), 0, st, (float*)p, n);
  SAST_CHECK_LAUNCH();
  return SAST_OK;
}

template <typename T>
__global__ __launch_bounds__(256) void nzr_count_kernel(const T* __restrict__ x, int* __restrict__ cnt, int C, int H, int W) {
  __shared__ float cell[8][33];
  const int plane = blockIdx.z;
  const int cy = threadIdx.x >> 5, cx = threadIdx.x & 31;
  const int y0 = blockIdx.y * 32 + cy * 4;
  int n1 = 0, n2 = 0, n3 = 0, n4 = 0;
// ... 794 lines not shown
__global__ __launch_bounds__(64) void ls_linear_finish_kernel(LsFinish p0, LsFinish p1, int C0) {
  const LsFinish& p = blockIdx.y == 0 ? p0 : p1;
  const int c = blockIdx.x;
  if (blockIdx.y == 0 && c >= C0) return;
  ls_finish_row(p, c, threadIdx.x);
}
int ls_linear_finish_launch(const float* w, const float* b, const float* gamma, const float* raw, const float* s, float* dw,
                            float* db, float* dgamma, int C, int K, hipStream_t st) {
  const LsFinish p{w, b, gamma, raw, s, dw, db, dgamma, K};
  SAST_LAUNCH(ls_linear_finish_kernel, dim3(C, 1), dim3(64), 0, st, p, p, C);
  SAST_CHECK_LAUNCH();
  return SAST_OK;
}
int ls_linear_finish2_launch(const float* w0, const float* b0, const float* g0, const float* raw0, const float* s0, float* dw0, float* db0,
                             float* dg0, int K0, const float* w1, const float* b1, const float* g1, const float* raw1, const float* s1,
                             float* dw1, float* db1, float* dg1, int K1, int C, hipStream_t st) {
  const LsFinish p0{w0, b0, g0, raw0, s0, dw0, db0, dg0, K0}, p1{w1, b1, g1, raw1, s1, dw1, db1, dg1, K1};
  SAST_LAUNCH(ls_linear_finish_kernel, dim3(C, 2), dim3(64), 0, st, p0, p1, C);
  SAST_CHECK_LAUNCH();
  return SAST_OK;
}

struct MsqJob { const float* x[4]; float* dx[4]; unsigned long long n[4]; };
__global__ __launch_bounds__(1024) void mean_square_fwd_kernel(MsqJob j, float* __restrict__ partials) {
  __shared__ float red[16];
  const int t = blockIdx.y;
  const float* __restrict__ x = j.x[t];
  const size_t n4 = j.n[t] / 4;
  float s = 0.f;
  for (size_t i = (size_t)blockIdx.x * 1024 + threadIdx.x; i < n4; i += (size_t)gridDim.x * 1024) {
    const float4 v = ld4(x + 4 * i);
    s += v.x * v.x + v.y * v.y + v.z * v.z + v.w * v.w;
  }
  s = wave_sum(s);
  if ((threadIdx.x & 63) == 0) red[threadIdx.x >> 6] = s;
  __syncthreads();
  if (threadIdx.x == 0) {
    float a = 0.f;
    for (int w = 0; w < 16; ++w) a += red[w];
    partials[t * gridDim.x + blockIdx.x] = a / (float)j.n[t];
  }
}
__global__ __launch_bounds__(1024) void mean_square_bwd_kernel(MsqJob j, const float* __restrict__ g, int g_stride) {
  const int t = blockIdx.y;
  const float* __restrict__ x = j.x[t];
  float* __restrict__ dx = j.dx[t];
  const size_t n4 = j.n[t] / 4;
  const float k = 2.f * g[(size_t)(t * gridDim.x + blockIdx.x) * g_stride] / (float)j.n[t];
  for (size_t i = (size_t)blockIdx.x * 1024 + threadIdx.x; i < n4; i += (size_t)gridDim.x * 1024) {
    const float4 v = ld4(x + 4 * i);
    st4(dx + 4 * i, make_float4(k * v.x, k * v.y, k * v.z, k * v.w));
  }
}
int mean_square_launch(const float* const* x, float* const* dx, const size_t* n, int count, int blocks, float* partials,
                       const float* g, int g_stride, hipStream_t st) {
  MsqJob j{};
  for (int t = 0; t < count; ++t) { j.x[t] = x[t]; j.dx[t] = dx ? dx[t] : nullptr; j.n[t] = n[t]; }
  if (!dx) SAST_LAUNCH(mean_square_fwd_kernel, dim3(blocks, count), dim3(1024), 0, st, j, partials);
  else SAST_LAUNCH(mean_square_bwd_kernel, dim3(blocks, count), dim3(1024), 0, st, j, g, g_stride);
  SAST_CHECK_LAUNCH();
  return SAST_OK;
}

__global__ __launch_bounds__(256) void gather_samples_kernel(SastSampleGather a) {
  const int j = blockIdx.y;
  const float* __restrict__ src = a.src[a.t_of[j]] + (size_t)a.b_of[j] * a.sample_floats;
  float* __restrict__ dst = a.out + (size_t)j * a.sample_floats;
  const size_t n4 = a.sample_floats / 4;
  for (size_t i = (size_t)blockIdx.x * 256 + threadIdx.x; i < n4; i += (size_t)gridDim.x * 256) st4(dst + 4 * i, ld4(src + 4 * i));
}
__global__ __launch_bounds__(256) void scatter_samples_kernel(SastSampleGather a) {
  const int t = blockIdx.y / a.B, b = blockIdx.y % a.B;
  int j = -1;
  for (int k = 0; k < a.n_out; ++k) if (a.t_of[k] == t && a.b_of[k] == b) j = k;
  float* __restrict__ dst = a.dsrc[t] + (size_t)b * a.sample_floats;
  const size_t n4 = a.sample_floats / 4;
  if (j < 0) {
    for (size_t i = (size_t)blockIdx.x * 256 + threadIdx.x; i < n4; i += (size_t)gridDim.x * 256) st4(dst + 4 * i, zero4());
  } else {
    const float* __restrict__ src = a.out + (size_t)j * a.sample_floats;
    for (size_t i = (size_t)blockIdx.x * 256 + threadIdx.x; i < n4; i += (size_t)gridDim.x * 256) st4(dst + 4 * i, ld4(src + 4 * i));
  }
}
int sample_gather_launch(const SastSampleGather& a, bool backward, hipStream_t st) {
  const size_t n4 = a.sample_floats / 4;
  int bx = (int)((n4 + 256 * 8 - 1) / (256 * 8));
  bx = bx < 1 ? 1 : (bx > 64 ? 64 : bx);
  if (!backward) SAST_LAUNCH(gather_samples_kernel, dim3(bx, a.n_out), dim3(256), 0, st, a);
  else SAST_LAUNCH(scatter_samples_kernel, dim3(bx, a.n_src * a.B), dim3(256), 0, st, a);
  SAST_CHECK_LAUNCH();
  return SAST_OK;
}
__global__ __launch_bounds__(256) void zero_samples_kernel(float* __restrict__ x, size_t sample_floats, SastSampleMask m) {
  if (!m.sel[blockIdx.y]) return;
  float* __restrict__ dst = x + (size_t)blockIdx.y * sample_floats;
  const size_t n4 = sample_floats / 4;
  for (size_t i = (size_t)blockIdx.x * 256 + threadIdx.x; i < n4; i += (size_t)gridDim.x * 256) st4(dst + 4 * i, zero4());
}
int zero_samples_launch(float* x, int B, size_t sample_floats, const SastSampleMask& m, hipStream_t st) {
  const size_t n4 = sample_floats / 4;
  int bx = (int)((n4 + 256 * 8 - 1) / (256 * 8));
  bx = bx < 1 ? 1 : (bx > 64 ? 64 : bx);
  SAST_LAUNCH(zero_samples_kernel, dim3(bx, B), dim3(256), 0, st, x, sample_floats, m);
  SAST_CHECK_LAUNCH();
  return SAST_OK;
}

__global__ __launch_bounds__(256) void cb_sample_sum_kernel(const float* __restrict__ src, int ld, const int* __restrict__ gather,
                                                            const int* __restrict__ row_tok, const int* __restrict__ nrows_dev,
                                                            int tps, int C, int strip, float* __restrict__ out, const float* __restrict__ rs) {
  __shared__ float4 red[256];
  const int nrows = *nrows_dev;
// ... 89 lines not shown
```

### sast_amd/csrc/kernels.h

```cpp
#pragma once
#include <hip/hip_runtime.h>
#include "../../include/sast_hip.h"

namespace sast {

int zero_fill(void* p, size_t bytes, hipStream_t st);
int nzr_dispatch(const void* x, int dtype, int* cnt, float* r, int B, int C, int H, int W, int Hp, int Wp, hipStream_t st);
int nchw_to_nhwc_dispatch(const void* x, int dtype, float* y, int B, int C, int H, int W, int Hp, int Wp, hipStream_t st);
int input_prep_dispatch(const void* x, int dtype, float* y, int* ws, float* r, int B, int C, int H, int W, int Hp, int Wp, hipStream_t st,
                        unsigned* nonexact = nullptr);
int input_prep_u8(const unsigned char* x, unsigned char* y, int* ws, float* r, int B, int C, int H, int W, int Hp, int Wp, hipStream_t st);
int nhwc_to_nchw_launch(const float* x, float* y, int B, int C, int HW, hipStream_t st);
int ln_fwd_launch(const float* x, float* y, const float* gamma, const float* beta, const float* add, int add_rows,
                  float* mean, float* rstd, int rows, int C, float eps, hipStream_t st);
int ln_bwd_launch(const float* x, const float* dy, const float* gamma, const float* mean, const float* rstd, float* dx,
                  float* dgamma, float* dbeta, int rows, int C, hipStream_t st);
int ln1_gather_fwd_launch(const float* xin, float* out, float* sc, const int* tok_slot, const float* g1, const float* b1,
                          const float* g2, const float* b2, float* mean1, float* rstd1, float* mean2, float* rstd2,
                          int rows, int C, float eps, float* zero_ptr, size_t zero_floats, hipStream_t st);
int ln1_gather_bwd_launch(const float* xin, const float* dout, const float* dsc, const int* tok_slot, const float* g1,
                          const float* b1, const float* g2, const float* mean1, const float* rstd1, const float* mean2,
                          const float* rstd2, float* dxin, float* dg1, float* db1, float* dg2, float* db2, int rows, int C,
                          hipStream_t st);
int controls_fwd_launch(const float* wc, const float* r, int r_stride, float* scale, int B, int C, int J, float* zero_bc,
                        hipStream_t st);
int controls_bwd_launch(const float* wc, const float* r, int r_stride, const float* dscale, float* dwc, int B, int C, int J,
                        hipStream_t st);
int stp_fwd_launch(const float* xp, const float* s, const float* scale, float amp, float* xw, float* tok, int B, int L, int C,
                   hipStream_t st);
int stp_bwd_launch(const float* xp, const float* s, const float* scale, const float* g, float* direct, float* dz,
                   float* dscale, int B, int L, int C, hipStream_t st);
int add_rows_launch(const float* x, const float* t, float* y, int rows, int C, int table_rows, hipStream_t st);
int row_scale_launch(const float* src, const int* idx, const float* rs, float* dst, const int* nrows_dev, int rows_max, int C, hipStream_t st);
int mask_token_fwd_launch(float* x, const unsigned char* mask, const float* token, const float* pe, int rows, int C, int L, hipStream_t st);
int mask_token_bwd_launch(const float* dy, const unsigned char* mask, float* dx, float* dtoken, int rows, int C, hipStream_t st);
int colsum_launch(const float* x, int ld, const int* idx, int rows, const int* drows, int C, float* out, hipStream_t st);
int mean_square_launch(const float* const* x, float* const* dx, const size_t* n, int count, int blocks, float* partials,
                       const float* g, int g_stride, hipStream_t st);
int ls_linear_finish_launch(const float* w, const float* b, const float* gamma, const float* raw, const float* s, float* dw,
                            float* db, float* dgamma, int C, int K, hipStream_t st);
int ls_linear_finish2_launch(const float* w0, const float* b0, const float* g0, const float* raw0, const float* s0, float* dw0, float* db0,
                             float* dg0, int K0, const float* w1, const float* b1, const float* g1, const float* raw1, const float* s1,
                             float* dw1, float* db1, float* dg1, int K1, int C, hipStream_t st);
int cb_sample_sum_launch(const float* src, int ld, bool gather, const int* row_tok, const int* nrows_dev, int rows_max, int tps,
                         int n_samples, int C, float* out, hipStream_t st, const float* rs = nullptr);
int cb_apply_fwd_launch(const float* m, const float* y, const float* gamma, const float* sum, const int* row_tok,
                        const int* nrows_dev, int rows_max, int tps, int C, float* out, hipStream_t st, const float* rs = nullptr);
int cb_apply_bwd_launch(const float* dout, const float* gsum, const int* row_tok, const int* nrows_dev, int rows_max, int tps, int C,
                        float* dz, hipStream_t st, const float* rs = nullptr);

int sample_gather_launch(const SastSampleGather& a, bool backward, hipStream_t st);
int zero_samples_launch(float* x, int B, size_t sample_floats, const SastSampleMask& m, hipStream_t st);

int select_launch(const float* tok, int B, int H, int W, int ph, int pw, int mode, float thr_win, float thr_tok, const SastSel* s,
                  hipStream_t st);
int select_packs_launch(const SastSel* s, int W, int T, hipStream_t st);
int attn_pack_limit(int T);

int select_pair_launch(const float* tok, int B, int H, int W, int ph, int pw, float thr_win, float thr_tok, const SastSel* win,
                       const SastSel* grid, hipStream_t st);

int attn_fwd_mfma_launch(const float* qkv, float* o, float* lse, const int* row_off, const int* Kw, int W, int T, int C, int dh, hipStream_t st);
struct LsFinish;
int attn_bwd_mfma_launch(const float* qkv, const float* dout, const float* lse, float* dqkv, const int* row_off, const int* Kw,
                         int W, int T, int C, int dh, hipStream_t st,
                         const LsFinish* f0 = nullptr, const LsFinish* f1 = nullptr, int fC = 0, float* dbuf = nullptr);

struct DwGeom { int Hi, Wi, Ho, Wo, C, k, stride; };
struct DwBnSilu { const float* mean; const float* var; const float* gamma; const float* beta; float eps; };
int dwconv_fwd_launch(const float* x, const float* w, const float* bias, float* y, int B, DwGeom g, const DwBnSilu* bn, hipStream_t st);
int dwconv_bwd_launch(const float* x, const float* w, const float* dy, float* dx, float* dw, float* db, int B, DwGeom g, hipStream_t st);

bool mswsa_fused_supported(int C, int inner, int T, int dim_head, int cb_tps);
size_t mswsa_fused_plane_floats(int C, int inner);
int mswsa_fused_planes_launch(const SastMswsaArgs* a, float* planes, hipStream_t st);
int mswsa_fused_fwd_launch(const SastMswsaArgs* a, const float* planes, hipStream_t st);



}
```

### sast_amd/detection/network_blocks.py

```python
from __future__ import annotations

import torch
import torch.nn as nn

from .. import functional as SF
from ..layers.ops import channels_last_conv_weight


class BaseConv(nn.Module):

    def __init__(self, in_channels, out_channels, ksize, stride, groups=1, bias=False, act="silu"):
        super().__init__()
        depthwise = groups > 1 and groups == in_channels == out_channels
        if (groups != 1 and not depthwise) or bias or act != "silu" or ksize not in (1, 3):
            raise NotImplementedError("sast_amd: BaseConv implements groups=1 or groups=in=out (depth-wise), bias=False, act='silu', "
                                      "ksize in {1,3}")
        self.ksize, self.stride, self.groups = ksize, stride, groups
        self.conv = nn.Module()
        self.conv.weight = channels_last_conv_weight(out_channels, in_channels // groups, ksize)
        self.bn = nn.BatchNorm2d(out_channels)
        self.sync_bn = None

    def sync_group(self):
        if self.sync_bn is None and isinstance(self.bn, nn.SyncBatchNorm):
            self.sync_bn = SF.sync_group_for(self.bn.process_group)
        return self.sync_bn

    def forward_nhwc(self, x, arena=None, sole=False, two_outputs=False):
        bn = self.bn
        ws = arena.take(SF.bn_ws_floats(bn.num_features)) if arena is not None else None
        sync = self.sync_group()
        if sync is not None and arena is None and self.training and sync.active():
            x0 = x[0] if isinstance(x, (tuple, list)) else x
            sync.exchange_batch(x0.shape[0], x0.device)
        y = SF.conv_bn_silu(x, self.conv.weight, bn.weight, bn.bias, bn.running_mean, bn.running_var, self.ksize, self.stride,
                            self.training, bn.momentum, bn.eps, ws, sole_consumer=sole, two_outputs=two_outputs, sync=sync)
        if self.training and bn.num_batches_tracked is not None:
            if arena is not None:
                arena.counters.append(bn.num_batches_tracked)
            else:
                bn.num_batches_tracked.add_(1)
        return y

    def sync_item(self, x, arena=None, sole=False, two_outputs=False):
        bn = self.bn
        return dict(x_nhwc=x, w=self.conv.weight, bn_w=bn.weight, bn_b=bn.bias, run_mean=bn.running_mean, run_var=bn.running_var,
                    ksize=self.ksize, stride=self.stride, momentum=bn.momentum, eps=bn.eps, sole_consumer=sole, two_outputs=two_outputs,
                    bn_ws=arena.take(SF.bn_ws_floats(bn.num_features)) if arena is not None else None)

    def forward(self, x):
        if isinstance(x, (tuple, list)):
            raise TypeError("sast_amd: the two-source (virtual concat) input is an internal NHWC feature; use forward_nhwc")
        return SF.as_nchw_view(self.forward_nhwc(SF.as_nhwc(x)))


def forward_sync_group(grp, convs, xs, arena, sole=False):
    soles = sole if isinstance(sole, (tuple, list)) else (sole,) * len(convs)
    if arena is None:
        x0 = xs[0][0] if isinstance(xs[0], (tuple, list)) else xs[0]
        grp.exchange_batch(x0.shape[0], x0.device)
    ys = SF.conv_bn_silu_sync_group(grp, [c.sync_item(x, arena, sole=s) for c, x, s in zip(convs, xs, soles)])
    for c in convs:
        if c.bn.num_batches_tracked is not None:
            if arena is not None:
                arena.counters.append(c.bn.num_batches_tracked)
            else:
                c.bn.num_batches_tracked.add_(1)
    return ys


class DWConv(nn.Module):

    def __init__(self, in_channels, out_channels, ksize, stride=1, act="silu"):
        super().__init__()
        self.dconv = BaseConv(in_channels, in_channels, ksize=ksize, stride=stride, groups=in_channels, act=act)
        self.pconv = BaseConv(in_channels, out_channels, ksize=1, stride=1, groups=1, act=act)

    def forward_nhwc(self, x, arena=None, sole=False, two_outputs=False):
        return self.pconv.forward_nhwc(self.dconv.forward_nhwc(x, arena), arena, sole=True, two_outputs=two_outputs)

    def forward(self, x):
        return SF.as_nchw_view(self.forward_nhwc(SF.as_nhwc(x)))


def sync_active(conv: "BaseConv") -> bool:
    grp = conv.sync_group()
    return grp is not None and grp.active()


def bn_scratch_floats(module: nn.Module) -> int:
    return sum(SF.bn_ws_floats(m.num_features) for m in module.modules() if isinstance(m, nn.modules.batchnorm._BatchNorm))


def pass_sync_group(module: nn.Module):
    grp = getattr(module, "_sync_group", None)
# ... 110 lines not shown
```

### sast_amd/detection/yolo_head.py

```python
from __future__ import annotations

import math
from typing import Dict, Optional

import torch
import torch.nn as nn

from .. import _lib as L
from .. import functional as SF
from .network_blocks import BaseConv, BnArena, DWConv, bn_scratch_floats, forward_sync_group, pass_sync_group


class _PredConv(nn.Module):

    def __init__(self, cin: int, cout: int):
        super().__init__()
        k = 1.0 / math.sqrt(cin)
        self.weight = nn.Parameter((torch.rand(cout, cin, 1, 1) * 2 - 1) * k)
        self.bias = nn.Parameter((torch.rand(cout) * 2 - 1) * k)


class YOLOXHead(nn.Module):
    def __init__(self, num_classes=80, strides=(8, 16, 32), in_channels=(256, 512, 1024), act="silu", depthwise=False,
                 compile_cfg: Optional[Dict] = None):
        super().__init__()
        Conv = DWConv if depthwise else BaseConv
        self.depthwise = bool(depthwise)
        self.num_classes = num_classes
        self.decode_in_inference = True
        self.strides = tuple(strides)
        hidden = int(256 * (in_channels[-1] / 1024))
        self.hidden_dim = hidden
        self.cls_convs, self.reg_convs = nn.ModuleList(), nn.ModuleList()
        self.cls_preds, self.reg_preds, self.obj_preds, self.stems = nn.ModuleList(), nn.ModuleList(), nn.ModuleList(), nn.ModuleList()
        for c in in_channels:
            self.stems.append(BaseConv(int(c), hidden, 1, stride=1, act=act))
            self.cls_convs.append(nn.Sequential(Conv(hidden, hidden, 3, stride=1, act=act), Conv(hidden, hidden, 3, stride=1, act=act)))
            self.reg_convs.append(nn.Sequential(Conv(hidden, hidden, 3, stride=1, act=act), Conv(hidden, hidden, 3, stride=1, act=act)))
            self.cls_preds.append(_PredConv(hidden, num_classes))
            self.reg_preds.append(_PredConv(hidden, 4))
            self.obj_preds.append(_PredConv(hidden, 1))
        self.use_l1 = False
        self._sync_group = None
        self.hw = None
        self.initialize_biases(prior_prob=0.01)

    def initialize_biases(self, prior_prob):
        with torch.no_grad():
            for conv in list(self.cls_preds) + list(self.obj_preds):
                conv.bias.fill_(-math.log((1 - prior_prob) / prior_prob))

    def forward_train_nhwc(self, feats, labels):
        per_level, levels = [], []
        if not hasattr(self, "_bn_floats"):
            self._bn_floats = bn_scratch_floats(self)
        ar = BnArena(self._bn_floats, feats[0].device)
        grp = pass_sync_group(self) if self.training else None
        sync = grp is not None and grp.active()
        if sync and not grp.same_pass(feats[0]):
            grp.exchange_batch(feats[0].shape[0], feats[0].device)
        if sync and SF.SYNC_BN_GROUPS and not self.depthwise:
            n = len(feats)
            xs = forward_sync_group(grp, list(self.stems), list(feats), ar)
            t = forward_sync_group(grp, [self.cls_convs[k][0] for k in range(n)] + [self.reg_convs[k][0] for k in range(n)], xs + xs, ar)
            t = forward_sync_group(grp, [self.cls_convs[k][1] for k in range(n)] + [self.reg_convs[k][1] for k in range(n)], t, ar, sole=True)
            for k, (x, stride) in enumerate(zip(xs, self.strides)):
                cp, rp, op = self.cls_preds[k], self.reg_preds[k], self.obj_preds[k]
                per_level.append((t[n + k], t[k], rp.weight, rp.bias, op.weight, op.bias, cp.weight, cp.bias))
                levels.append((x.shape[1], x.shape[2], stride))
        else:
            for k, (x, stride) in enumerate(zip(feats, self.strides)):
                x = self.stems[k].forward_nhwc(x, ar)
                if SF.CONV_PAIR and not sync and not self.depthwise:
                    c0, r0 = self.cls_convs[k][0], self.reg_convs[k][0]
                    args = [(c.conv.weight, c.bn.weight, c.bn.bias, c.bn.running_mean, c.bn.running_var, c.bn.momentum, c.bn.eps) for c in (c0, r0)]
                    ws = tuple(ar.take(SF.bn_ws_floats(c.bn.num_features)) for c in (c0, r0))
                    cf, rf = SF.conv_bn_silu2(x, args[0], args[1], ws, sole_consumer=True, ksize=3)
                    ar.counters.extend(c.bn.num_batches_tracked for c in (c0, r0) if c.bn.num_batches_tracked is not None)
                    first = 1
                else:
                    cf, rf = x, x
                    first = 0
                for i, conv in enumerate(self.cls_convs[k]):
                    if i >= first:
                        cf = conv.forward_nhwc(cf, ar, sole=i > 0)
                for i, conv in enumerate(self.reg_convs[k]):
                    if i >= first:
                        rf = conv.forward_nhwc(rf, ar, sole=i > 0)
                cp, rp, op = self.cls_preds[k], self.reg_preds[k], self.obj_preds[k]
                per_level.append((rf, cf, rp.weight, rp.bias, op.weight, op.bias, cp.weight, cp.bias))
                levels.append((x.shape[1], x.shape[2], stride))
        ar.finish()
        losses, pred, fg, mg, piou = SF.head_pred_loss(labels, levels, self.num_classes, self.decode_in_inference, per_level, self.use_l1)
        self.last_assignment = (fg, mg, piou)
        self.hw = [(h, w) for h, w, _ in levels]
        det = losses.detach()
        return pred, {"loss": losses[0], "iou_loss": det[1], "conf_loss": det[2], "cls_loss": det[3], "l1_loss": det[4] if self.use_l1 else 0.0,
                      "num_fg": det[5]}

    @torch.no_grad()
    def forward_nhwc(self, feats):
        if self.training:
            raise RuntimeError("sast_amd: YOLOXHead.forward_nhwc is the inference path; in training mode call forward(xin, labels)")
        B = feats[0].shape[0]
        dev = feats[0].device
        hw = [tuple(f.shape[1:3]) for f in feats]
        A = sum(h * w for h, w in hw)
        no = 5 + self.num_classes
        out = torch.empty(B, A, no, device=dev)
        off = 0
        for k, (x, stride) in enumerate(zip(feats, self.strides)):
            x = self.stems[k].forward_nhwc(x)
            if SF.CONV_PAIR and not self.depthwise:
                c0, r0 = self.cls_convs[k][0], self.reg_convs[k][0]
                cf, rf = SF.conv_bn_silu2_infer(x, *[(c.conv.weight, c.bn.weight, c.bn.bias, c.bn.running_mean, c.bn.running_var,
                                                     c.bn.momentum, c.bn.eps) for c in (c0, r0)], ksize=3)
                for conv in list(self.cls_convs[k])[1:]:
                    cf = conv.forward_nhwc(cf)
                for conv in list(self.reg_convs[k])[1:]:
                    rf = conv.forward_nhwc(rf)
            else:
                cf, rf = x, x
                for conv in self.cls_convs[k]:
                    cf = conv.forward_nhwc(cf)
                for conv in self.reg_convs[k]:
# ... 20 lines not shown
```

### sast_amd/detection/yolo_pafpn.py

```python
from __future__ import annotations

from typing import Dict, Optional, Tuple

import torch.nn as nn

from .. import functional as SF
from .network_blocks import BaseConv, BnArena, CSPLayer, DWConv, bn_scratch_floats, pass_sync_group


class YOLOPAFPN(nn.Module):

    def __init__(self, depth: float = 1.0, in_stages: Tuple[int, ...] = (2, 3, 4), in_channels: Tuple[int, ...] = (256, 512, 1024),
                 depthwise: bool = False, act: str = "silu", compile_cfg: Optional[Dict] = None):
        super().__init__()
        assert len(in_stages) == len(in_channels) == 3, 'Current implementation only for 3 feature maps'
        if compile_cfg is not None and compile_cfg.get('enable', False):
            import warnings
            warnings.warn("sast_amd: compile.enable is ignored (no torch.compile: capture the step in a hipGraph, sast_amd.training.TrainStep)")
        self.in_features, self.in_channels = in_stages, in_channels
        c0, c1, c2 = in_channels
        n = round(3 * depth)
        Conv = DWConv if depthwise else BaseConv
        self.lateral_conv0 = BaseConv(c2, c1, 1, 1, act=act)
        self.C3_p4 = CSPLayer(2 * c1, c1, n, False, depthwise=depthwise, act=act)
        self.reduce_conv1 = BaseConv(c1, c0, 1, 1, act=act)
        self.C3_p3 = CSPLayer(2 * c0, c0, n, False, depthwise=depthwise, act=act)
        self.bu_conv2 = Conv(c0, c0, 3, 2, act=act)
        self.C3_n3 = CSPLayer(2 * c0, c1, n, False, depthwise=depthwise, act=act)
        self.bu_conv1 = Conv(c1, c1, 3, 2, act=act)
        self.C3_n4 = CSPLayer(2 * c1, c2, n, False, depthwise=depthwise, act=act)
        self._sync_group = None

    def forward_nhwc(self, feats: Dict[int, object]):
        x2, x1, x0 = (feats[f] for f in self.in_features)
        if not hasattr(self, "_bn_floats"):
            self._bn_floats = bn_scratch_floats(self)
        ar = BnArena(self._bn_floats, x0.device)
        grp = pass_sync_group(self) if self.training else None
        token = None
        if grp is not None and grp.active():
            token = grp.exchange_batch(x0.shape[0], x0.device)
        fpn_out0, fpn_out0b = self.lateral_conv0.forward_nhwc(x0, ar, two_outputs=True)
        f_out0 = self.C3_p4.forward_nhwc(SF.upsample_cat(fpn_out0, x1), ar, sole_input=True)
        fpn_out1, fpn_out1b = self.reduce_conv1.forward_nhwc(f_out0, ar, sole=True, two_outputs=True)
        pan_out2, pan_out2b = self.C3_p3.forward_nhwc(SF.upsample_cat(fpn_out1, x2), ar, sole_input=True, two_outputs=True)
        p_out1 = (self.bu_conv2.forward_nhwc(pan_out2b, ar), fpn_out1b)
        pan_out1, pan_out1b = self.C3_n3.forward_nhwc(p_out1, ar, sole_input=(True, False), two_outputs=True)
        p_out0 = (self.bu_conv1.forward_nhwc(pan_out1b, ar), fpn_out0b)
        pan_out0 = self.C3_n4.forward_nhwc(p_out0, ar, sole_input=(True, False))
        ar.finish()
        if token is not None:
            pan_out2._sast_sync_pass = pan_out1._sast_sync_pass = pan_out0._sast_sync_pass = token
        return pan_out2, pan_out1, pan_out0

    def forward(self, input):
        feats = {f: SF.as_nhwc(input[f]) for f in self.in_features}
        return tuple(SF.as_nchw_view(o) for o in self.forward_nhwc(feats))
```

### sast_amd/functional.py

```python
from __future__ import annotations

import collections
import ctypes as C
import os
from typing import Optional, Tuple

import torch

from . import _lib as L

_DT = {torch.float32: L.DT_F32, torch.int32: L.DT_I32, torch.uint8: L.DT_U8, torch.int8: L.DT_I8}


_raw_stream = getattr(torch._C, "_cuda_getCurrentRawStream", None)


def _stream():
    if _raw_stream is not None:
        return C.c_void_p(_raw_stream(torch.cuda.current_device()))
    return C.c_void_p(torch.cuda.current_stream().cuda_stream)


def _need_gpu(*ts):
    for t in ts:
# ... 185 lines not shown
@torch.no_grad()
def input_prep(x: torch.Tensor, pad_hw=None, ws_cache: Optional[dict] = None, keep_bytes: bool = False):
    _need_gpu(x)
    if x.dtype not in _DT:
        x = x.float()
    x = x.contiguous()
    B, Cc, H, W = x.shape
    Hp, Wp = (int(pad_hw[0]), int(pad_hw[1])) if pad_hw is not None else (H, W)
    if H % 4 or W % 4 or Hp % 32 or Wp % 32 or Cc != 20 or ((Hp // 32) * (Wp // 32)) % 2 or Hp < H or Wp < W:
        pad = (Hp, Wp) if (Hp, Wp) != (H, W) else None
        return non_zero_ratio(x, pad), nchw_to_nhwc_float(x, pad)
    cache = _PREP_WS if ws_cache is None else ws_cache
    key = (x.device, B, Cc) if ws_cache is not None else (x.device, torch.cuda.current_stream().cuda_stream, B, Cc)
    ws = cache.get(key)
    if ws is None:
        if torch.cuda.is_current_stream_capturing():
            raise RuntimeError("sast_amd: input_prep needs one un-captured warm-up call (per model and batch size) before graph capture")
        ws = cache[key] = torch.zeros(B * 4 * Cc + 2, device=x.device, dtype=torch.int32)
    r = torch.empty(B, 4, Cc, device=x.device, dtype=torch.float32)
    u8 = keep_bytes and x.dtype == torch.uint8
    if u8:
        y = torch.empty(B, Hp, Wp, Cc, device=x.device, dtype=torch.uint8)
    else:
        n = B * Hp * Wp * Cc
        buf = torch.empty(n + 4, device=x.device, dtype=torch.float32)
        y = buf[:n].view(B, Hp, Wp, Cc)
        y.sast_nonexact = buf[n:n + 1].view(torch.int32)
    try:
        if u8:
            L.check(L.lib().sast_input_prep_u8(x.data_ptr(), B, Cc, H, W, Hp, Wp, ws.data_ptr(), r.data_ptr(), y.data_ptr(), _stream()), "input_prep_u8")
        else:
            L.check(L.lib().sast_input_prep_flag(x.data_ptr(), _DT[x.dtype], B, Cc, H, W, Hp, Wp, ws.data_ptr(), r.data_ptr(), y.data_ptr(),
                                                 y.sast_nonexact.data_ptr(), _stream()), "input_prep")
    except Exception:
        cache.pop(key, None)
        raise
    return r, y


def as_nhwc(x: torch.Tensor) -> torch.Tensor:
    v = x.permute(0, 2, 3, 1)
    return v if v.is_contiguous() else v.contiguous()


def as_nchw_view(x_nhwc: torch.Tensor) -> torch.Tensor:
    return x_nhwc.permute(0, 3, 1, 2)


MEAN_SQUARE_BLOCKS = 128


class _MeanSquares(torch.autograd.Function):
    @staticmethod
    def forward(ctx, *xs):
        _need_gpu(*xs)
        xs = tuple(x.contiguous() for x in xs)
        k = len(xs)
        ptrs = (C.c_void_p * k)(*[x.data_ptr() for x in xs])
        ns = (C.c_size_t * k)(*[x.numel() for x in xs])
        partials = torch.empty(k * MEAN_SQUARE_BLOCKS, device=xs[0].device, dtype=torch.float32)
        L.check(L.lib().sast_mean_square_fwd(ptrs, ns, k, partials.data_ptr(), _stream()), "mean_square_fwd")
        ctx.save_for_backward(*xs)
        return partials

    @staticmethod
    def backward(ctx, g):
        xs = ctx.saved_tensors
        k = len(xs)
        g_stride = 1
        if g.stride(0) == 0:
            g, g_stride = g.as_strided((1,), (1,)), 0
        else:
            g = g.contiguous()
        dxs = tuple(torch.empty_like(x) for x in xs)
        ptrs = (C.c_void_p * k)(*[x.data_ptr() for x in xs])
        dptrs = (C.c_void_p * k)(*[d.data_ptr() for d in dxs])
        ns = (C.c_size_t * k)(*[x.numel() for x in xs])
        L.check(L.lib().sast_mean_square_bwd(ptrs, ns, k, g.data_ptr(), g_stride, dptrs, _stream()), "mean_square_bwd")
        return dxs


def mean_squares(*xs: torch.Tensor) -> torch.Tensor:
    if not 1 <= len(xs) <= 4 or any(x.dtype != torch.float32 or x.numel() % 4 for x in xs):
        raise ValueError("mean_squares: 1..4 fp32 tensors with numel % 4 == 0")
    return _MeanSquares.apply(*xs).sum()


class _AddRows(torch.autograd.Function):
    @staticmethod
    def forward(ctx, x, table):
        _need_gpu(x, table)
        x = x.contiguous()
        y = torch.empty_like(x)
        Cc = x.shape[-1]
        rows = x.numel() // Cc
        L.check(L.lib().sast_add_rows(x.data_ptr(), table.data_ptr(), y.data_ptr(), rows, Cc, table.numel() // Cc, _stream()), "add_rows")
        return y

    @staticmethod
    def backward(ctx, dy):
        return dy, None


def add_pos_embedding(x: torch.Tensor, table: torch.Tensor) -> torch.Tensor:
    return _AddRows.apply(x, table)


def downsample_out_hw(H: int, W: int, factor: int, k: int) -> Tuple[int, int]:
    H, W, factor, k = int(H), int(W), int(factor), int(k)
    if factor < 1 or k not in (factor, 2 * factor - 1):
        raise RuntimeError(f"sast_amd: a factor-{factor} downsampling conv has a {2 * factor - 1}x{2 * factor - 1} (overlap) or "
                           f"{factor}x{factor} (no overlap) kernel, not {k}x{k}")
    if k == factor:
        if H < factor or W < factor:
            raise RuntimeError(f"sast_amd: downsample_ln: the map H = {H}, W = {W} is smaller than the factor-{factor} patch")
        return H // factor, W // factor
    if H % factor or W % factor or H < factor or W < factor:
        raise RuntimeError(f"sast_amd: downsample_ln: the overlapping factor-{factor} conv needs H and W that are multiples of {factor}, "
                           f"got H = {H}, W = {W} (factor {factor})")
    return H // factor, W // factor


class _DownsampleLN(torch.autograd.Function):
    @staticmethod
    def forward(ctx, x, w, ln_w, ln_b, pe, factor, nonexact=None):
        _need_gpu(x, w)
        x = x.contiguous()
        if not is_channels_last_weight(w):
            raise RuntimeError("sast_amd: conv weights must be stored channels_last ([Cout][KH][KW][Cin])")
        B, H, W, Cin = x.shape
        Cout = w.shape[0]
        k = w.shape[-1]
        if k not in (factor, 2 * factor - 1) or w.shape[-2] != k:
            raise RuntimeError(f"sast_amd: a factor-{factor} downsampling conv has a {2 * factor - 1}x{2 * factor - 1} (overlap) or "
                               f"{factor}x{factor} (no overlap) kernel, not {tuple(w.shape[-2:])}")
        no_overlap = int(k == factor)
        Ho, Wo = downsample_out_hw(H, W, factor, k)
        M = B * Ho * Wo
# ... 471 lines not shown
        dc0 = torch.empty_like(x) if need_c else None
        ws = torch.empty(B * Lt * 4 * Cc, device=x.device)
        pg = _ParamGrads(w, b)
        a = _fill(L.SastLstmArgs(), B=B, L=Lt, C=Cc, x=x, h0=_ptr(h0), c0=_ptr(c0), w=w, b=b, c1=c1, gates=gates, dh1=dh1,
                  dc1=_ptr(dc1), dx=dx, dh0=_ptr(dh0), dc0=_ptr(dc0), dw=pg[0], db=pg[1], ws=ws, dh1b=_ptr(dh1b), drop=_ptr(drop))
        L.check(L.lib().sast_lstm_bwd(C.byref(a), _stream()), "lstm_bwd")
        _dw_hold((x, h0, c0, c1, gates, drop, dh1, dh1b, dc1, ws, pg))
        return (dx, dh0, dc0) + pg.out() + (None,)


def conv_lstm(x_nhwc, h0, c0, w, b, two_h=False, drop_mask=None):
    h1, h1b, c1 = _LSTM.apply(x_nhwc, h0, c0, w, b, drop_mask)
    return (h1, h1b if TWO_OUT else h1, c1) if two_h else (h1, c1)


class _DwConv(torch.autograd.Function):

    @staticmethod
    def forward(ctx, x, w, b, c0):
        _need_gpu(x, w)
        x = x.contiguous()
        B, H, W, Cc = x.shape
        k = w.shape[-1]
        if w.dim() != 4 or w.shape[1] != 1 or w.shape[2] != k or not w.is_contiguous() or c0 < 0 or c0 + Cc > w.shape[0]:
            raise RuntimeError("sast_amd: dwconv needs the contiguous Conv2d(groups=C) weight [C, 1, k, k]")
        y = torch.empty_like(x)
        L.check(L.lib().sast_dwconv_fwd(x.data_ptr(), w.data_ptr() + 4 * c0 * k * k, (b.data_ptr() + 4 * c0) if b is not None else None,
                                        y.data_ptr(), B, H, W, Cc, k, _stream()), "dwconv_fwd")
        ctx.save_for_backward(x)
        ctx.params = (w, b, c0)
        return y

    @staticmethod
    def backward(ctx, dy):
        (x,) = ctx.saved_tensors
        w, b, c0 = ctx.params
        B, H, W, Cc = x.shape
        k = w.shape[-1]
        dy = dy.contiguous()
        dx = torch.empty_like(x) if ctx.needs_input_grad[0] else None
        pg = _ParamGrads(w, b)
        gw = pg[0]
        gb = pg[1] if b is not None else torch.zeros(w.shape[0], device=x.device)
        L.check(L.lib().sast_dwconv_bwd(x.data_ptr(), w.data_ptr() + 4 * c0 * k * k, dy.data_ptr(), _ptr(dx), gw.data_ptr() + 4 * c0 * k * k,
                                        gb.data_ptr() + 4 * c0, B, H, W, Cc, k, _stream()), "dwconv_bwd")
        return (dx,) + pg.out() + (None,)


def dwconv(x_nhwc: torch.Tensor, w: torch.Tensor, b: Optional[torch.Tensor], c0: int = 0) -> torch.Tensor:
    return _DwConv.apply(x_nhwc, w, b, int(c0))


class BnHandle:
    __slots__ = ("conv_out", "stats", "bn_w", "bn_b", "bn_ws", "cout", "red_done")

    def __init__(self):
        self.conv_out = self.stats = self.bn_w = self.bn_b = self.bn_ws = None
        self.cout = -1
        self.red_done = False

    def fill(self, conv_out, stats, bn_w, bn_b, bn_ws, cout):
        self.conv_out, self.stats, self.bn_w, self.bn_b, self.bn_ws, self.cout = conv_out, stats, bn_w, bn_b, bn_ws, cout
        return self


class SyncBatchNormGroup:

    def __init__(self, process_group=None, force: bool = False):
        import torch.distributed as dist
        self.dist, self.group = dist, process_group
        self._world = None
        self._ratio = None
        self._comm = None
        self.force = bool(force)
        self.n_collectives = 0
        self._epoch = None

    def _validate(self):
        d = self.dist
        cur = d.group.WORLD if d.is_initialized() else None
        if cur is not self._epoch:
            self._world = self._ratio = self._comm = None
            self._epoch = cur

    @property
    def world(self) -> int:
        self._validate()
        if self._world is None:
            if not self.dist.is_initialized():
                return 1
            self._world = self.dist.get_world_size(self.group)
        return self._world

    def active(self) -> bool:
        return self.world > 1 or self.force

    def capturable(self) -> bool:
        if not self.dist.is_initialized():
            return True
        return self.dist.get_backend(self.group) == "nccl"

    def communicator(self):
        self._validate()
        if self._comm is None:
            d = self.dist
            if d.get_backend(self.group) == "nccl" and os.environ.get("SAST_SYNC_BN_PRIVATE_COMM", "1") != "0":
                if torch.cuda.is_available() and torch.cuda.is_current_stream_capturing():
                    raise RuntimeError("sast_amd: SyncBatchNormGroup needs one eager pass before a hipGraph capture (it creates the "
                                       "private RCCL communicator of the statistics all-reduces)")
                ranks = d.get_process_group_ranks(self.group if self.group is not None else d.group.WORLD)
                self._comm = d.new_group(ranks=ranks, backend="nccl", use_local_synchronization=True)
            else:
# ... 57 lines not shown


def sync_group_for(process_group=None) -> SyncBatchNormGroup:
    key = id(process_group) if process_group is not None else None
    g = _SYNC_GROUPS.get(key)
    if g is None:
        g = _SYNC_GROUPS[key] = SyncBatchNormGroup(process_group)
    return g


def _bn_ws_blocks(bn_ws, Cout):
    n = bn_ws.numel() // 6
    raw = bn_ws.data
    return raw[:4 * n].view(torch.float64), raw[4 * n:]


def _cbs_fwd_args(x, x2, w, bn_w, bn_b, run_mean, run_var, ksize, stride, training, momentum, eps, bn_ws):
    _need_gpu(x, w)
    x = x.contiguous()
    if not is_channels_last_weight(w):
        raise RuntimeError("sast_amd: conv weights must be stored channels_last ([Cout][KH][KW][Cin])")
    B, H, W, Cin = x.shape
    Cin1 = Cin
    if x2 is not None:
        if ksize != 1 or stride != 1 or x2.shape[:3] != x.shape[:3]:
            raise RuntimeError("sast_amd: a two-source input is supported for 1x1 stride-1 convs of equal spatial size")
        x2 = x2.contiguous()
        Cin = Cin1 + x2.shape[-1]
    Cout = w.shape[0]
    groups = _conv_groups(w, Cin, x2)
    pad = (ksize - 1) // 2
    Ho, Wo = (H + 2 * pad - ksize) // stride + 1, (W + 2 * pad - ksize) // stride + 1
    M = B * Ho * Wo
    dev = x.device
    conv_out = torch.empty(M, Cout, device=dev)
    stats = torch.empty(2 * Cout, device=dev)
    y = torch.empty(B, Ho, Wo, Cout, device=dev)
    if bn_ws is None:
        bn_ws = torch.zeros(bn_ws_floats(Cout), device=dev)
    a = _fill(L.SastConvBnArgs(), B=B, H=H, W=W, Cin=Cin, Cout=Cout, ksize=ksize, stride=stride, training=int(training), ldx=Cin1,
              ldy=Cout, bn_ws_zeroed=1, momentum=momentum, eps=eps, x=x, w=w, bn_w=bn_w, bn_b=bn_b, run_mean=_ptr(run_mean),
              run_var=_ptr(run_var), conv_out=conv_out, stats=stats, y=y, bn_ws=bn_ws, x2=_ptr(x2), Cin1=Cin1, ldx2=Cin - Cin1, groups=groups)
    st = dict(saved=(x, x2, conv_out, stats, bn_ws), params=(w, bn_w, bn_b), groups=groups, y=y,
              meta=(B, H, W, Cin, Cin1, Cout, ksize, stride, int(training), momentum, eps, M))
    return a, st


def _cbs_fwd_links(st, training, producers, handle):
    x, x2, conv_out, stats, bn_ws = st["saved"]
    w, bn_w, bn_b = st["params"]
    B, H, W, Cin, Cin1, Cout, ksize, stride = st["meta"][:8]
    own = handle.fill(conv_out, stats, bn_w, bn_b, bn_ws, Cout) if (training and handle is not None) else None
    p1, p2 = producers if (training and stride == 1 and st["groups"] == 1) else (None, None)
    if p1 is not None and p1.cout != Cin1:
        p1 = None
    if p2 is not None and (x2 is None or p2.cout != Cin - Cin1):
        p2 = None
    return own, (p1, p2)


def _cbs_bwd_args(saved, params, meta, groups, own, producers, need1, need2, dy, dy2):
    x, x2, conv_out, stats, bn_ws = saved
    if dy is None:
        dy, dy2 = dy2, None
    if dy is None:
        dy = torch.zeros(conv_out.shape, device=conv_out.device)
    dy2 = dy2.contiguous() if dy2 is not None else None
    w, bn_w, bn_b = params
    B, H, W, Cin, Cin1, Cout, ksize, stride, training, momentum, eps, M = meta
    dy = dy.contiguous()
    need = need1 or (x2 is not None and need2)
    dx = torch.empty_like(x) if need else None
    dx2 = torch.empty_like(x2) if (need and x2 is not None) else None
    ws = torch.empty(M * Cout, device=x.device)
    p1, p2 = producers if need else (None, None)
    if p1 is not None and p1.red_done:
        p1 = None
    if p2 is not None and (p2.red_done or dx2 is None):
        p2 = None
    pk = {}
    for pre, h in (("p_", p1), ("p2_", p2)):
        if h is not None:
            pk.update({pre + "conv_out": h.conv_out, pre + "stats": h.stats, pre + "bn_w": h.bn_w, pre + "bn_b": h.bn_b,
                       pre + "bn_ws": h.bn_ws})
    pg = _ParamGrads(w, bn_w, bn_b)
    a = _fill(L.SastConvBnArgs(), B=B, H=H, W=W, Cin=Cin, Cout=Cout, ksize=ksize, stride=stride, training=training, ldx=Cin1,
              ldy=Cout, lddy=Cout, lddx=Cin1, bn_ws_zeroed=1, bn_red_done=int(own is not None and own.red_done), momentum=momentum,
              eps=eps, x=x, w=w, bn_w=bn_w, bn_b=bn_b, conv_out=conv_out, stats=stats, dy=dy, dx=_ptr(dx), dw=pg[0],
              d_bn_w=pg[1], d_bn_b=pg[2], bn_ws=bn_ws, ws=ws, x2=_ptr(x2), dx2=_ptr(dx2), Cin1=Cin1, ldx2=Cin - Cin1, dy2=_ptr(dy2),
              groups=groups, **pk)
    return a, dx, dx2, pg, (p1, p2), (dy, dy2, ws)


class _ConvBnSilu(torch.autograd.Function):
    @staticmethod
    def forward(ctx, x, x2, w, bn_w, bn_b, run_mean, run_var, ksize, stride, training, momentum, eps, bn_ws, producers, handle, two_y,
                sync=None):
        a, st = _cbs_fwd_args(x, x2, w, bn_w, bn_b, run_mean, run_var, ksize, stride, training, momentum, eps, bn_ws)
        M, B, Cout = st["meta"][11], st["meta"][0], st["meta"][5]
        bn_ws = st["saved"][4]
        m_total = 0
        if sync is not None and training and sync.active():
            a.sync_phase = 1
            L.check(L.lib().sast_conv_bn_silu_fwd(C.byref(a), _stream()), "conv_bn_silu_fwd")
            sync.all_reduce(_bn_ws_blocks(bn_ws, Cout)[0])
            m_total = sync.rows_total(M, B)
            a.sync_phase, a.m_total = 2, m_total
        L.check(L.lib().sast_conv_bn_silu_fwd(C.byref(a), _stream()), "conv_bn_silu_fwd")
        ctx.sync = (sync, m_total) if m_total else None
        ctx.save_for_backward(*st["saved"])
        ctx.params, ctx.meta, ctx.groups = st["params"], st["meta"], st["groups"]
        ctx.handle, ctx.producers = _cbs_fwd_links(st, training, producers, handle)
        ctx.two_y = bool(two_y)
        y = st["y"]
        return (y, y.view_as(y)) if two_y else y

    @staticmethod
    def backward(ctx, dy, dy2=None):
        _consume(ctx, "conv_bn_silu")
        Cout = ctx.meta[5]
        a, dx, dx2, pg, served, _keep = _cbs_bwd_args(ctx.saved_tensors, ctx.params, ctx.meta, ctx.groups, ctx.handle, ctx.producers,
                                                      ctx.needs_input_grad[0], ctx.needs_input_grad[1], dy, dy2)
        if ctx.sync is not None:
            sync, m_total = ctx.sync
            a.sync_phase = 1
            L.check(L.lib().sast_conv_bn_silu_bwd(C.byref(a), _stream()), "conv_bn_silu_bwd")
            sync.all_reduce(_bn_ws_blocks(ctx.saved_tensors[4], Cout)[1])
            a.sync_phase, a.m_total, a.d_bn_w, a.d_bn_b = 2, m_total, None, None
        L.check(L.lib().sast_conv_bn_silu_bwd(C.byref(a), _stream()), "conv_bn_silu_bwd")
        _dw_hold((ctx.saved_tensors, _keep, pg))
        for h in served:
            if h is not None:
                h.red_done = True
        return (dx, dx2) + pg.out() + (None,) * 12


_CBS_UNIT_IN = 7


class _ConvBnSiluSyncGroup(torch.autograd.Function):

    @staticmethod
    def forward(ctx, sync, units, *tensors):
        n = len(units)
        jobs, saved, outs = [], [], []
        for i, (ksize, stride, momentum, eps, bn_ws, producers, handle, two_y) in enumerate(units):
            x, x2, w, bn_w, bn_b, rm, rv = tensors[_CBS_UNIT_IN * i:_CBS_UNIT_IN * (i + 1)]
            a, st = _cbs_fwd_args(x, x2, w, bn_w, bn_b, rm, rv, ksize, stride, True, momentum, eps, bn_ws)
            a.sync_phase = 1
            L.check(L.lib().sast_conv_bn_silu_fwd(C.byref(a), _stream()), "conv_bn_silu_fwd")
            jobs.append((a, st))
        sync.all_reduce_many([_bn_ws_blocks(st["saved"][4], st["meta"][5])[0] for _a, st in jobs])
        ctx.units = []
        for (a, st), (ksize, stride, momentum, eps, bn_ws, producers, handle, two_y) in zip(jobs, units):
            m_total = sync.rows_total(st["meta"][11], st["meta"][0])
            a.sync_phase, a.m_total = 2, m_total
            L.check(L.lib().sast_conv_bn_silu_fwd(C.byref(a), _stream()), "conv_bn_silu_fwd")
            own, prods = _cbs_fwd_links(st, True, producers, handle)
            ctx.units.append((st["params"], st["meta"], st["groups"], own, prods, bool(two_y), m_total, [t is not None for t in st["saved"]]))
            saved.extend(t for t in st["saved"] if t is not None)
            y = st["y"]
            outs.extend((y, y.view_as(y)) if two_y else (y,))
        ctx.sync = sync
        ctx.save_for_backward(*saved)
        return tuple(outs)

    @staticmethod
    def backward(ctx, *dys):
        _consume(ctx, "conv_bn_silu (SyncBatchNorm group)")
        sv, k, d = list(ctx.saved_tensors), 0, 0
        jobs = []
        for i, (params, meta, groups, own, prods, two_y, m_total, present) in enumerate(ctx.units):
            saved = []
            for has in present:
                saved.append(sv[k] if has else None)
                k += has
            dy, dy2 = (dys[d], dys[d + 1]) if two_y else (dys[d], None)
            d += 2 if two_y else 1
            a, dx, dx2, pg, served, keep = _cbs_bwd_args(tuple(saved), params, meta, groups, own, prods,
                                                         ctx.needs_input_grad[2 + _CBS_UNIT_IN * i], ctx.needs_input_grad[3 + _CBS_UNIT_IN * i], dy, dy2)
            a.sync_phase = 1
            L.check(L.lib().sast_conv_bn_silu_bwd(C.byref(a), _stream()), "conv_bn_silu_bwd")
            jobs.append((a, dx, dx2, pg, served, keep, saved[4], meta[5], m_total))
        ctx.sync.all_reduce_many([_bn_ws_blocks(ws, cout)[1] for (_a, _dx, _dx2, _pg, _s, _k, ws, cout, _m) in jobs])
        grads = [None, None]
        for a, dx, dx2, pg, served, _keep, _ws, _cout, m_total in jobs:
            a.sync_phase, a.m_total, a.d_bn_w, a.d_bn_b = 2, m_total, None, None
            L.check(L.lib().sast_conv_bn_silu_bwd(C.byref(a), _stream()), "conv_bn_silu_bwd")
            for h in served:
                if h is not None:
                    h.red_done = True
            grads.extend((dx, dx2) + pg.out() + (None, None))
        _dw_hold((sv, jobs))
        return tuple(grads)


def conv_bn_silu_sync_group(sync: "SyncBatchNormGroup", items):
    units, tensors = [], []
    for it in items:
        xin = it["x_nhwc"]
        x, x2 = xin if isinstance(xin, (tuple, list)) else (xin, None)
        two = bool(it.get("two_outputs", False)) and TWO_OUT and torch.is_grad_enabled()
        handle = None if two else BnHandle()
        units.append((int(it["ksize"]), int(it["stride"]), float(it.get("momentum", 0.1)), float(it.get("eps", 1e-5)), it.get("bn_ws"),
                      _producers(x, x2, it.get("sole_consumer", False)), handle, two))
        tensors.extend((x, x2, it["w"], it["bn_w"], it["bn_b"], it["run_mean"], it["run_var"]))
    flat = _ConvBnSiluSyncGroup.apply(sync, units, *tensors)
    outs, k = [], 0
    for it, u in zip(items, units):
        if u[7]:
            outs.append((flat[k], flat[k + 1]))
            k += 2
        else:
            y = flat[k]
            y._sast_bn = u[6]
            k += 1
            outs.append((y, y) if it.get("two_outputs", False) else y)
    return outs


def _conv_groups(w, cin: int, x2=None) -> int:
    if w.shape[1] == cin:
        return 1
    if w.shape[1] == 1 and w.shape[0] == cin and x2 is None:
        return cin
    raise RuntimeError(f"sast_amd: conv weight {tuple(w.shape)} fits neither a dense conv of {cin} input channels nor a depth-wise one")


def bn_ws_floats(cout: int) -> int:
    return int(L.lib().sast_conv_bn_ws_floats(int(cout)))


class _ConvBnSilu2(torch.autograd.Function):

    @staticmethod
    def forward(ctx, x, x2, w0, bnw0, bnb0, rm0, rv0, w1, bnw1, bnb1, rm1, rv1, mom0, eps0, mom1, eps1, ws0, ws1, producers, handles, ksize):
        _need_gpu(x, w0, w1)
        x = x.contiguous()
        for w in (w0, w1):
            if not is_channels_last_weight(w):
                raise RuntimeError("sast_amd: conv weights must be stored channels_last ([Cout][KH][KW][Cin])")
        B, H, W, Cin1 = x.shape
        Cin = Cin1
        if x2 is not None:
            if x2.shape[:3] != x.shape[:3]:
                raise RuntimeError("sast_amd: the two sources of a virtual concat need equal spatial size")
            x2 = x2.contiguous()
            Cin = Cin1 + x2.shape[-1]
        Cout = w0.shape[0]
        if w1.shape[0] != Cout or tuple(w0.shape[1:]) != (Cin, ksize, ksize) or tuple(w1.shape[1:]) != (Cin, ksize, ksize) or \
                ksize not in (1, 3) or (ksize == 3 and x2 is not None):
            raise RuntimeError("sast_amd: conv_bn_silu2 needs two 1x1 (or 3x3, single-source) convs of the same input with equal Cout")
        M, dev = B * H * W, x.device
        co = [torch.empty(M, Cout, device=dev) for _ in range(2)]
        st = [torch.empty(2 * Cout, device=dev) for _ in range(2)]
        ys = [torch.empty(B, H, W, Cout, device=dev) for _ in range(2)]
        if ws0 is None or ws1 is None:
            ws0, ws1 = torch.zeros(bn_ws_floats(Cout), device=dev), torch.zeros(bn_ws_floats(Cout), device=dev)
        a = _fill(L.SastConvBn2Args(), B=B, H=H, W=W, Cin=Cin, Cout=Cout, ldx=Cin1, Cin1=Cin1, ldx2=Cin - Cin1, bn_ws_zeroed=1, training=1, ksize=ksize,
                  momentum0=mom0, momentum1=mom1, eps0=eps0, eps1=eps1, x=x, x2=_ptr(x2), w0=w0, w1=w1, bn_w0=bnw0, bn_w1=bnw1,
                  bn_b0=bnb0, bn_b1=bnb1, run_mean0=_ptr(rm0), run_mean1=_ptr(rm1), run_var0=_ptr(rv0), run_var1=_ptr(rv1),
                  conv_out0=co[0], conv_out1=co[1], stats0=st[0], stats1=st[1], y0=ys[0], y1=ys[1], bn_ws0=ws0, bn_ws1=ws1)
        L.check(L.lib().sast_conv_bn_silu2_fwd(C.byref(a), _stream()), "conv_bn_silu2_fwd")
        ctx.save_for_backward(x, x2, co[0], co[1], st[0], st[1], ws0, ws1)
        ctx.params = (w0, bnw0, bnb0, w1, bnw1, bnb1)
        ctx.meta = (B, H, W, Cin, Cin1, Cout, mom0, eps0, mom1, eps1, M, ksize)
        ctx.handles = (handles[0].fill(co[0], st[0], bnw0, bnb0, ws0, Cout), handles[1].fill(co[1], st[1], bnw1, bnb1, ws1, Cout))
        p1, p2 = producers
        if p1 is not None and p1.cout != Cin1:
            p1 = None
        if p2 is not None and (x2 is None or p2.cout != Cin - Cin1):
            p2 = None
        ctx.producers = (p1, p2)
        return ys[0], ys[1]

    @staticmethod
    def backward(ctx, dy0, dy1):
        x, x2, co0, co1, st0, st1, ws0, ws1 = ctx.saved_tensors
        _consume(ctx, "conv_bn_silu2")
        w0, bnw0, bnb0, w1, bnw1, bnb1 = ctx.params
        B, H, W, Cin, Cin1, Cout, mom0, eps0, mom1, eps1, M, ksize = ctx.meta
        dy0 = dy0.contiguous() if dy0 is not None else torch.zeros(B, H, W, Cout, device=x.device)
        dy1 = dy1.contiguous() if dy1 is not None else torch.zeros(B, H, W, Cout, device=x.device)
        need = ctx.needs_input_grad[0] or (x2 is not None and ctx.needs_input_grad[1])
        dx = torch.empty_like(x) if need else None
        dx2 = torch.empty_like(x2) if (need and x2 is not None) else None
        dws = torch.empty(M, 2 * Cout, device=x.device)
        p1, p2 = ctx.producers if need else (None, None)
        if p1 is not None and p1.red_done:
            p1 = None
        if p2 is not None and (p2.red_done or dx2 is None):
            p2 = None
        pk = {}
        for pre, h in (("p_", p1), ("p2_", p2)):
            if h is not None:
                pk.update({pre + "conv_out": h.conv_out, pre + "stats": h.stats, pre + "bn_w": h.bn_w, pre + "bn_b": h.bn_b,
                           pre + "bn_ws": h.bn_ws})
        h0, h1 = ctx.handles
        pg = _ParamGrads(w0, bnw0, bnb0, w1, bnw1, bnb1)
        a = _fill(L.SastConvBn2Args(), B=B, H=H, W=W, Cin=Cin, Cout=Cout, ldx=Cin1, Cin1=Cin1, ldx2=Cin - Cin1, bn_ws_zeroed=1, training=1, ksize=ksize,
                  bn_red_done0=int(h0.red_done), bn_red_done1=int(h1.red_done), momentum0=mom0, momentum1=mom1, eps0=eps0, eps1=eps1,
                  x=x, x2=_ptr(x2), w0=w0, w1=w1, bn_w0=bnw0, bn_w1=bnw1, bn_b0=bnb0, bn_b1=bnb1, conv_out0=co0, conv_out1=co1,
                  stats0=st0, stats1=st1, bn_ws0=ws0, bn_ws1=ws1, dy0=dy0, dy1=dy1, dw0=pg[0], dw1=pg[3], d_bn_w0=pg[1],
                  d_bn_w1=pg[4], d_bn_b0=pg[2], d_bn_b1=pg[5], ws0=dws, dx=_ptr(dx), dx2=_ptr(dx2), **pk)
        L.check(L.lib().sast_conv_bn_silu2_bwd(C.byref(a), _stream()), "conv_bn_silu2_bwd")
        _dw_hold((x, x2, co0, co1, st0, st1, ws0, ws1, dy0, dy1, dws, pg))
        for h in (p1, p2):
            if h is not None:
                h.red_done = True
        g = pg.out()
        return (dx, dx2) + g[0:3] + (None, None) + g[3:6] + (None,) * 11


@torch.no_grad()
def conv_bn_silu2_infer(x_nhwc, conv0, conv1, ksize=1):
    x, x2 = x_nhwc if isinstance(x_nhwc, (tuple, list)) else (x_nhwc, None)
    _need_gpu(x)
    x = x.contiguous()
    (w0, g0, b0, rm0, rv0, _m0, e0), (w1, g1, b1, rm1, rv1, _m1, e1) = conv0, conv1
    for w in (w0, w1):
        if not is_channels_last_weight(w):
            raise RuntimeError("sast_amd: conv weights must be stored channels_last ([Cout][KH][KW][Cin])")
    B, H, W, Cin1 = x.shape
    Cin = Cin1
    if x2 is not None:
        if ksize != 1 or x2.shape[:3] != x.shape[:3]:
            raise RuntimeError("sast_amd: a two-source input is supported for 1x1 convs of equal spatial size")
        x2 = x2.contiguous()
        Cin = Cin1 + x2.shape[-1]
    Cout = w0.shape[0]
    if w1.shape[0] != Cout or tuple(w0.shape[1:]) != (Cin, ksize, ksize) or tuple(w1.shape[1:]) != (Cin, ksize, ksize):
        raise RuntimeError("sast_amd: conv_bn_silu2_infer needs two convs of the same input with equal shapes")
    y0, y1 = torch.empty(B, H, W, Cout, device=x.device), torch.empty(B, H, W, Cout, device=x.device)
    a = _fill(L.SastConvBn2Args(), B=B, H=H, W=W, Cin=Cin, Cout=Cout, ldx=Cin1, Cin1=Cin1, ldx2=Cin - Cin1, training=0, ksize=ksize,
              eps0=float(e0), eps1=float(e1), x=x, x2=_ptr(x2), w0=w0, w1=w1, bn_w0=g0, bn_w1=g1, bn_b0=b0, bn_b1=b1, run_mean0=rm0,
              run_mean1=rm1, run_var0=rv0, run_var1=rv1, y0=y0, y1=y1)
    L.check(L.lib().sast_conv_bn_silu2_fwd(C.byref(a), _stream()), "conv_bn_silu2_fwd")
    return y0, y1


def conv_bn_silu2(x_nhwc, conv0, conv1, bn_ws=(None, None), sole_consumer=False, ksize=1):
    x, x2 = x_nhwc if isinstance(x_nhwc, (tuple, list)) else (x_nhwc, None)
    prods = _producers(x, x2, sole_consumer)
    (w0, g0, b0, rm0, rv0, m0, e0), (w1, g1, b1, rm1, rv1, m1, e1) = conv0, conv1
    hs = (BnHandle(), BnHandle())
    y0, y1 = _ConvBnSilu2.apply(x, x2, w0, g0, b0, rm0, rv0, w1, g1, b1, rm1, rv1, float(m0), float(e0), float(m1), float(e1),
                                bn_ws[0], bn_ws[1], prods, hs, int(ksize))
    y0._sast_bn, y1._sast_bn = hs
    return y0, y1


def _producers(x, x2, sole):
    s1, s2 = sole if isinstance(sole, (tuple, list)) else (sole, sole)
    if not BN_FOLD:
        return (None, None)
    return (getattr(x, "_sast_bn", None) if s1 else None, getattr(x2, "_sast_bn", None) if (s2 and x2 is not None) else None)
TWO_OUT = os.environ.get("SAST_TWO_OUT", "1") != "0"
CONV_PAIR = os.environ.get("SAST_CONV_PAIR", "1") != "0"
BN_FOLD = os.environ.get("SAST_BN_FOLD", "1") != "0"
SYNC_BN_GROUPS = os.environ.get("SAST_SYNC_BN_GROUPS", "1") != "0"


def conv_bn_silu(x_nhwc, w, bn_w, bn_b, run_mean, run_var, ksize, stride, training, momentum=0.1, eps=1e-5, bn_ws=None,
                 sole_consumer=False, two_outputs=False, sync=None):
    x, x2 = x_nhwc if isinstance(x_nhwc, (tuple, list)) else (x_nhwc, None)
    if sync is not None and not (training and sync.active()):
        sync = None
    if two_outputs and (not TWO_OUT or not training or not torch.is_grad_enabled()):
        y = conv_bn_silu(x_nhwc, w, bn_w, bn_b, run_mean, run_var, ksize, stride, training, momentum, eps, bn_ws, sole_consumer, sync=sync)
        return y, y
    if not training and not (torch.is_grad_enabled() and any(t is not None and t.requires_grad for t in (x, x2, w, bn_w, bn_b))):
        return _conv_bn_silu_infer(x, x2, w, bn_w, bn_b, run_mean, run_var, ksize, stride, float(eps))
    prods = _producers(x, x2, sole_consumer)
    if two_outputs:
        return _ConvBnSilu.apply(x, x2, w, bn_w, bn_b, run_mean, run_var, ksize, stride, True, float(momentum), float(eps), bn_ws, prods,
                                 None, True, sync)
    handle = BnHandle() if training else None
    y = _ConvBnSilu.apply(x, x2, w, bn_w, bn_b, run_mean, run_var, ksize, stride, bool(training), float(momentum), float(eps), bn_ws, prods,
                          handle, False, sync)
    if handle is not None:
        y._sast_bn = handle
    return y


def _conv_bn_silu_infer(x, x2, w, bn_w, bn_b, run_mean, run_var, ksize, stride, eps):
    _need_gpu(x, w)
    x = x.contiguous()
    if not is_channels_last_weight(w):
        raise RuntimeError("sast_amd: conv weights must be stored channels_last ([Cout][KH][KW][Cin])")
    B, H, W, Cin = x.shape
    Cin1 = Cin
    if x2 is not None:
        if ksize != 1 or stride != 1 or x2.shape[:3] != x.shape[:3]:
            raise RuntimeError("sast_amd: a two-source input is supported for 1x1 stride-1 convs of equal spatial size")
        x2 = x2.contiguous()
        Cin = Cin1 + x2.shape[-1]
    Cout = w.shape[0]
    pad = (ksize - 1) // 2
    Ho, Wo = (H + 2 * pad - ksize) // stride + 1, (W + 2 * pad - ksize) // stride + 1
    y = torch.empty(B, Ho, Wo, Cout, device=x.device)
    a = _fill(L.SastConvBnArgs(), B=B, H=H, W=W, Cin=Cin, Cout=Cout, ksize=ksize, stride=stride, training=0, ldx=Cin1, ldy=Cout,
              bn_ws_zeroed=1, momentum=0.0, eps=eps, x=x, w=w, bn_w=bn_w, bn_b=bn_b, run_mean=run_mean, run_var=run_var, y=y,
              x2=_ptr(x2), Cin1=Cin1, ldx2=Cin - Cin1, groups=_conv_groups(w, Cin, x2))
    L.check(L.lib().sast_conv_bn_silu_fwd(C.byref(a), _stream()), "conv_bn_silu_fwd")
    return y


class _UpsampleCat(torch.autograd.Function):
    @staticmethod
    def forward(ctx, a, b):
        _need_gpu(a, b)
        a, b = a.contiguous(), b.contiguous()
        B, H, W, C1 = a.shape
        C2 = b.shape[-1]
        assert b.shape[:3] == (B, 2 * H, 2 * W)
        out = torch.empty(B, 2 * H, 2 * W, C1 + C2, device=a.device)
        L.check(L.lib().sast_upsample_cat_fwd(a.data_ptr(), b.data_ptr(), out.data_ptr(), B, H, W, C1, C2, _stream()), "upsample_cat_fwd")
        ctx.meta = (B, H, W, C1, C2)
        return out

    @staticmethod
    def backward(ctx, dout):
        B, H, W, C1, C2 = ctx.meta
        dout = dout.contiguous()
        da = torch.empty(B, H, W, C1, device=dout.device)
        db = torch.empty(B, 2 * H, 2 * W, C2, device=dout.device)
        L.check(L.lib().sast_upsample_cat_bwd(dout.data_ptr(), da.data_ptr(), db.data_ptr(), B, H, W, C1, C2, _stream()), "upsample_cat_bwd")
        return da, db


def upsample_cat(a, b):
    return _UpsampleCat.apply(a, b)


class _Cat2(torch.autograd.Function):
    @staticmethod
    def forward(ctx, a, b):
        _need_gpu(a, b)
        a, b = a.contiguous(), b.contiguous()
        C1, C2 = a.shape[-1], b.shape[-1]
        rows = a.numel() // C1
        out = torch.empty(*a.shape[:-1], C1 + C2, device=a.device)
        L.check(L.lib().sast_cat2_fwd(a.data_ptr(), b.data_ptr(), out.data_ptr(), rows, C1, C2, _stream()), "cat2_fwd")
        ctx.meta = (a.shape, b.shape, rows, C1, C2)
        return out

    @staticmethod
    def backward(ctx, dout):
        sa, sb, rows, C1, C2 = ctx.meta
        dout = dout.contiguous()
        da, db = torch.empty(sa, device=dout.device), torch.empty(sb, device=dout.device)
        L.check(L.lib().sast_cat2_bwd(dout.data_ptr(), da.data_ptr(), db.data_ptr(), rows, C1, C2, _stream()), "cat2_bwd")
        return da, db


def cat2(a, b):
    return _Cat2.apply(a, b)


class _GatherSamples(torch.autograd.Function):

    @staticmethod
    def forward(ctx, table, *xs):
        _need_gpu(*xs)
        xs = tuple(x.contiguous() for x in xs)
        B = xs[0].shape[0]
        sample = xs[0][0].numel()
        if any(x.shape != xs[0].shape or x.dtype != torch.float32 for x in xs):
            raise RuntimeError("sast_amd: gather_samples needs fp32 tensors of one shape (one feature map over the timesteps)")
        if len(xs) > 32 or len(table) > 256 or B > 256 or sample % 4:
            raise RuntimeError("sast_amd: gather_samples supports <= 32 timesteps, <= 256 selected samples, batch <= 256")
        out = torch.empty((len(table),) + tuple(xs[0].shape[1:]), device=xs[0].device)
        a = L.SastSampleGather()
        a.n_src, a.n_out, a.B, a.sample_floats, a.out = len(xs), len(table), B, sample, out.data_ptr()
        for t, x in enumerate(xs):
            a.src[t] = x.data_ptr()
        for j, (t, b) in enumerate(table):
            a.t_of[j], a.b_of[j] = t, b
        L.check(L.lib().sast_gather_samples(C.byref(a), _stream()), "gather_samples")
        ctx.table, ctx.meta = table, (len(xs), B, sample, tuple(xs[0].shape))
        return out

    @staticmethod
    def backward(ctx, dout):
        n_src, B, sample, shape = ctx.meta
# ... 153 lines not shown
```

### sast_amd/training.py

```python
from __future__ import annotations

import os
from typing import Dict, List, Optional, Sequence

import torch
import torch.distributed as dist

from . import functional as SF
from .detection.network_blocks import pass_sync_group
from .dist import FlatParams, FusedAdamW, OneCycleLR


class TrainStep:
    def __init__(self, net, fpn, head=None, *, lr: float = 2e-4, weight_decay: float = 0.0, clip_value: float = 0.0, eps: float = 1e-8,
                 schedule: Optional[OneCycleLR] = None, world: int = 1, group=None, segmented: bool = True, defer_dw: bool = False,
                 dw_rows=(0, 0), dw_discard: bool = False, cuts: Sequence[int] = (3,)):
        self.net, self.fpn, self.head = net, fpn, head
        self.world, self.group = world, group
        self.defer_dw, self.dw_rows, self.dw_discard = bool(defer_dw), tuple(dw_rows), bool(dw_discard)
        stages = list(net.stages)
        first = [fpn] + ([head] if head is not None else [])
        if segmented:
            why = None
            if len(stages) != 4:
# ... 10 lines not shown
            if why is not None:
                import warnings
                warnings.warn(f"sast_amd.TrainStep: segmented backward disabled ({why}); running the monolithic step")
                segmented = False
        self.segmented = segmented
        self.cuts = tuple(sorted({int(c) for c in cuts}, reverse=True))
        if segmented and (not self.cuts or self.cuts[0] != 3 or min(self.cuts) < 1):
            raise ValueError(f"TrainStep(cuts={cuts}): the segmented backward needs the cut before the last stage (3) and cuts in 1 .. 3")
        if len(stages) == 4:
            buckets = [first, [stages[3]], [stages[2], stages[1], stages[0]]]
        else:
            buckets = [first, list(reversed(stages))]
        self.flat = FlatParams([], buckets=buckets)
        self.opt = FusedAdamW(self.flat, lr=lr, weight_decay=weight_decay, clip_value=clip_value, eps=eps, schedule=schedule)
        dev = self.flat.flat.device
        self._one = torch.ones((), device=dev)
        prio = int(os.environ.get("SAST_SIDE_PRIORITY", "1" if defer_dw else "0"))
        self.side = torch.cuda.Stream(priority=prio) if dev.type == "cuda" else None
        self.loss = self.P = self.losses = None
        self._graphs = None
        self._dw_graphs = None
        self._seg_state = None
        self.measure_exposed = False
        self._exposed = []
        self._bucket_ev = {}

    def forward(self, xs: Sequence[torch.Tensor], states=None, labels=None, indices=None, token_masks=None):
        if self.defer_dw and SF.dw_pending():
            SF.dw_discard()
            SF.dw_release()
        self.flat.zero_grad()
        single = len(xs) == 1 and self.segmented
        feats_seq, Ps = [], []
        for t, x in enumerate(xs):
            feats, states, P = self.net.forward_nhwc(x, states, token_masks[t] if token_masks is not None else None,
                                                     cut_before_stage=self.cuts if single else None)
            feats_seq.append(feats)
            Ps.append(P)
        cut = dict(self.net.last_cuts) if (single and self.net.last_cuts) else None
        if indices is not None:
            from .detection.sequence import BackboneFeatureSelector
            sel = BackboneFeatureSelector()
            for f, idx in zip(feats_seq, indices):
                if idx is not None and len(idx) > 0:
                    sel.add_backbone_features({k: f[k] for k in self.fpn.in_features}, idx)
            fpn_in = sel.get_batched_backbone_features()
        else:
            fpn_in = {k: feats_seq[-1][k] for k in self.fpn.in_features}
        leaves = None
        if self.segmented:
            leaves = {k: v.detach().requires_grad_(True) for k, v in fpn_in.items()}
        outs = self.fpn.forward_nhwc(leaves if leaves is not None else fpn_in)
        if labels is not None:
            _pred, self.losses = self.head.forward_train_nhwc(outs, labels)
            loss = self.losses["loss"]
        else:
            loss = SF.mean_squares(*outs)
        self.loss, self.P, self.states = loss, Ps[-1], states
        self._seg_state = (loss, fpn_in, leaves, cut)
        return loss

    def _stage_groups(self):
        cut = self._seg_state[3]
        bounds = sorted(cut.keys(), reverse=True)
        groups, hi = [], len(self.net.stages) - 1
        for c in bounds:
            groups.append(list(range(hi, c - 1, -1)))
            hi = c - 1
        groups.append(list(range(hi, -1, -1)))
        return groups

    def n_segments(self) -> int:
        if not self.segmented:
            return 1
        return 1 + len(self._stage_groups()) if self._seg_state[3] is not None else 2

    def _side_path(self) -> bool:
        return self.side is not None and (self.segmented or self.defer_dw)

    def backward_segment(self, i: int):
        if self.defer_dw:
            prev = SF.dw_defer(True, *self.dw_rows)
            try:
                self._backward_segment(i)
            finally:
                SF.dw_defer(prev)
            return
        self._backward_segment(i)

    def _backward_segment(self, i: int):
        loss, fpn_in, leaves, cut = self._seg_state
        if i == 0:
            loss.backward(gradient=self._one)
            return
        keys = list(fpn_in.keys())
        if cut is None:
            torch.autograd.backward([fpn_in[k] for k in keys], [leaves[k].grad for k in keys])
            return
        grp = self._stage_groups()[i - 1]
        roots, grads = [], []
        above = max(grp) + 1
        if above in cut:
            roots.append(cut[above][0])
            grads.append(cut[above][1].grad)
        for k in keys:
            if k - 1 in grp:
                roots.append(fpn_in[k])
                grads.append(leaves[k].grad)
        torch.autograd.backward(roots, grads)

# ... 170 lines not shown
```

Before: 859.1 frames/s.

## Fold BN backward reductions into multi-consumer epilogues and fuse upsample-concat into BN apply

Extends the BN-backward statistic folding so producers with several consumers (two-output convs, upsample-cat, the mean-square loss, strided parity conv dx) accumulate the BN gradient sums inside the consumer's epilogue, using a counted handle instead of a one-shot flag. It also adds a BN+SiLU apply kernel that writes the 2x-upsampled output directly into the concat buffer and copies the second source in the same launch, removing a separate upsample_cat forward pass. The aim is fewer full-tensor passes and launches in the PAFPN, paid for with more shared-memory and global atomics and more complex bookkeeping for handle readiness.

```diff
diff --git a/include/sast_hip.h b/include/sast_hip.h
--- a/include/sast_hip.h
+++ b/include/sast_hip.h
@@ -35,6 +35,9 @@
 int sast_mean_square_bwd(const float* const* x, const size_t* n, int count, const float* d_partials, int d_stride, float* const* dx,
                          sast_stream_t stream);
 int sast_mask_token_fwd(float* x, const uint8_t* mask, const float* token, const float* pos_emb, int rows, int C, int L, sast_stream_t stream);
+struct SastBnProducer;
+int sast_mean_square_bwd_bn(const float* const* x, const size_t* n, int count, const float* d_partials, int d_stride, float* const* dx,
+                            const struct SastBnProducer* prods, sast_stream_t stream);
 int sast_mask_token_bwd(const float* dy, const uint8_t* mask, float* dx, float* d_token, int rows, int C, sast_stream_t stream);
 
 typedef struct SastDownArgs {
@@ -171,6 +174,7 @@
   const float* dy2;
   int32_t sync_phase, m_total;
   int32_t groups;
+  float* up_cat; const float* up_b; int32_t up_C2, up_reserved;
 } SastConvBnArgs;
 int sast_conv_bn_silu_fwd(const SastConvBnArgs* a, sast_stream_t stream);
 int sast_conv_bn_silu_bwd(const SastConvBnArgs* a, sast_stream_t stream);
@@ -196,6 +200,12 @@
 
 int sast_upsample_cat_fwd(const float* a, const float* b, float* out, int B, int H, int W, int C1, int C2, sast_stream_t stream);
 int sast_upsample_cat_bwd(const float* dout, float* da, float* db, int B, int H, int W, int C1, int C2, sast_stream_t stream);
+typedef struct SastBnProducer {
+  const float* conv_out; const float* stats; const float* bn_w; const float* bn_b; float* bn_ws;
+  int32_t C, reserved;
+} SastBnProducer;
+int sast_upsample_cat_bwd_bn(const float* dout, float* da, float* db, int B, int H, int W, int C1, int C2, const SastBnProducer* prod,
+                             sast_stream_t stream);
 int sast_cat2_fwd(const float* a, const float* b, float* out, int rows, int C1, int C2, sast_stream_t stream);
 int sast_cat2_bwd(const float* dout, float* da, float* db, int rows, int C1, int C2, sast_stream_t stream);
 
diff --git a/sast_amd/_lib.py b/sast_amd/_lib.py
--- a/sast_amd/_lib.py
+++ b/sast_amd/_lib.py
@@ -69,7 +69,9 @@
     (P, "x w bn_w bn_b run_mean run_var conv_out stats y dy dx dw d_bn_w d_bn_b bn_ws ws x2 dx2 "
         "p_conv_out p_stats p_bn_w p_bn_b p_bn_ws p2_conv_out p2_stats p2_bn_w p2_bn_b p2_bn_ws dy2"),
     (I32, "sync_phase m_total groups"),
-])
+    (P, "up_cat up_b"), (I32, "up_C2 up_reserved"),
+])
+SastBnProducer = _struct("SastBnProducer", [(P, "conv_out stats bn_w bn_b bn_ws"), (I32, "C reserved")])
 
 SastSampleGather = _struct("SastSampleGather", [
     (I32, "n_src n_out B _pad"), (C.c_size_t, "sample_floats"), (P * 32, "src"), (P * 32, "dsrc"), (P, "out"),
@@ -113,6 +115,7 @@
     "sast_add_rows": (C.c_int, [P, P, P, C.c_int, C.c_int, C.c_int, P]),
     "sast_mean_square_fwd": (C.c_int, [P, P, C.c_int, P, P]),
     "sast_mean_square_bwd": (C.c_int, [P, P, C.c_int, P, C.c_int, P, P]),
+    "sast_mean_square_bwd_bn": (C.c_int, [P, P, C.c_int, P, C.c_int, P, P, P]),
     "sast_downsample_ln_fwd": (C.c_int, [C.POINTER(SastDownArgs), P]),
     "sast_downsample_ln_bwd": (C.c_int, [C.POINTER(SastDownArgs), P]),
     "sast_score_stp_fwd": (C.c_int, [C.POINTER(SastScoreArgs), P]),
@@ -145,6 +148,7 @@
     "sast_conv_bn_silu2_bwd": (C.c_int, [C.POINTER(SastConvBn2Args), P]),
     "sast_upsample_cat_fwd": (C.c_int, [P, P, P, C.c_int, C.c_int, C.c_int, C.c_int, C.c_int, P]),
     "sast_upsample_cat_bwd": (C.c_int, [P, P, P, C.c_int, C.c_int, C.c_int, C.c_int, C.c_int, P]),
+    "sast_upsample_cat_bwd_bn": (C.c_int, [P, P, P, C.c_int, C.c_int, C.c_int, C.c_int, C.c_int, P, P]),
     "sast_cat2_fwd": (C.c_int, [P, P, P, C.c_int, C.c_int, C.c_int, P]),
     "sast_cat2_bwd": (C.c_int, [P, P, P, C.c_int, C.c_int, C.c_int, P]),
     "sast_gather_samples": (C.c_int, [C.POINTER(SastSampleGather), P]),
diff --git a/sast_amd/csrc/gemm.cuh b/sast_amd/csrc/gemm.cuh
--- a/sast_amd/csrc/gemm.cuh
+++ b/sast_amd/csrc/gemm.cuh
@@ -1556,6 +1556,29 @@
   }
 };
 
+struct EpStoreClassBnRed {
+  static constexpr bool COLSTATS = true;
+  float* c; int ldc; int H, W; ConvDxClasses k; BnProducer p;
+  using Col = BnCol;
+  struct Aux { int p; float x; };
+  __device__ __forceinline__ Col col(int j) const { return bn_col(p, j); }
+  __device__ __forceinline__ Aux pre(int m, int j) const {
+    const int cls = fast_div(m, k.Mc, k.mc_mul), ic = m - cls * k.Mc;
+    const int t = fast_div(ic, k.Wc, k.wc_mul), xx = ic - t * k.Wc, b = fast_div(t, k.Hc, k.hc_mul), yy = t - b * k.Hc;
+    const int q = 3 - cls;
+    const int px = (b * H + 2 * yy + (q >> 1)) * W + 2 * xx + (q & 1);
+    return Aux{px, p.x[(size_t)px * p.C + j]};
+  }
+  __device__ __forceinline__ void post(int, int j, const float (&v)[1], const Col&, const Aux& a) const {
+    c[(size_t)a.p * ldc + j] = v[0];
+  }
+  __device__ __forceinline__ void stat(float v, const Col& kc, const Aux& a, float& s, float& q) const { bn_stat(v, a.x, kc, s, q); }
+  __device__ __forceinline__ void flush(int copy, int j, int, float s, float q) const {
+    float* sp = p.sums + (size_t)copy * 2 * p.C;
+    atomicAdd(sp + j, s); atomicAdd(sp + p.C + j, q);
+  }
+};
+
 struct EpSplit2BnRed {
   static constexpr bool COLSTATS = true;
   float* a; float* b; int C1, C2; BnProducer pa, pb;
diff --git a/sast_amd/csrc/k_block.hip b/sast_amd/csrc/k_block.hip
--- a/sast_amd/csrc/k_block.hip
+++ b/sast_amd/csrc/k_block.hip
@@ -226,6 +226,13 @@
   if (!x || !n || !d_partials || !dx || count < 1 || count > 4 || (d_stride != 0 && d_stride != 1)) return SAST_EINVAL;
   for (int t = 0; t < count; ++t) if (!x[t] || !dx[t] || n[t] % 4) return SAST_EINVAL;
   return mean_square_launch(x, dx, n, count, SAST_MEAN_SQUARE_BLOCKS, nullptr, d_partials, d_stride, (hipStream_t)stream);
+}
+
+int sast_mean_square_bwd_bn(const float* const* x, const size_t* n, int count, const float* d_partials, int d_stride, float* const* dx,
+                            const SastBnProducer* prods, sast_stream_t stream) { SAST_ENTRY();
+  if (!x || !n || !d_partials || !dx || !prods || count < 1 || count > 4 || (d_stride != 0 && d_stride != 1)) return SAST_EINVAL;
+  for (int t = 0; t < count; ++t) if (!x[t] || !dx[t] || n[t] % 4) return SAST_EINVAL;
+  return mean_square_launch(x, dx, n, count, SAST_MEAN_SQUARE_BLOCKS, nullptr, d_partials, d_stride, (hipStream_t)stream, prods);
 }
 
 int sast_mask_token_fwd(float* x, const uint8_t* mask, const float* token, const float* pos_emb, int rows, int C, int L, sast_stream_t stream) { SAST_ENTRY();
diff --git a/sast_amd/csrc/k_conv.hip b/sast_amd/csrc/k_conv.hip
--- a/sast_amd/csrc/k_conv.hip
+++ b/sast_amd/csrc/k_conv.hip
@@ -11,6 +11,41 @@
   const float* x; const double* sums; float* run_mean; float* run_var; float* stats; const float* gamma; const float* beta;
   float* y; int ldy; float momentum, eps;
 };
+__device__ __forceinline__ void bn_fwd_stats(const BnFwdJob& jb, double invM, double unbias, int C, int training, float* __restrict__ bn_sm) {
+  const double* __restrict__ sums = jb.sums;
+  float* __restrict__ run_mean = jb.run_mean; float* __restrict__ run_var = jb.run_var; float* __restrict__ stats = jb.stats;
+  const float momentum = jb.momentum, eps = jb.eps;
+  for (int c = threadIdx.x; c < C; c += 256) {
+    float mu, rs;
+    if (training) {
+      double sk[BN_STAT_COPIES], qk[BN_STAT_COPIES];
+#pragma unroll
+      for (int k = 0; k < BN_STAT_COPIES; ++k) { sk[k] = sums[(size_t)k * 2 * C + c]; qk[k] = sums[(size_t)k * 2 * C + C + c]; }
+      double s = 0.0, q = 0.0;
+#pragma unroll
+      for (int k = 0; k < BN_STAT_COPIES; ++k) { s += sk[k]; q += qk[k]; }
+      const double mean = s * invM;
+      double var = q * invM - mean * mean;
+      if (var < 0) var = 0;
+      mu = (float)mean;
+#if SAST_FAST_DIV
+      rs = rsqrt_hw((float)var + eps);
+#else
+      rs = (float)(1.0 / sqrt(var + (double)eps));
+#endif
+      if (blockIdx.x == 0 && run_mean) {
+        const double unb = var * unbias;
+        run_mean[c] = (1.f - momentum) * run_mean[c] + momentum * (float)mean;
+        run_var[c] = (1.f - momentum) * run_var[c] + momentum * (float)unb;
+      }
+    } else {
+      mu = run_mean[c];
+      rs = rsqrt_hw(run_var[c] + eps);
+    }
+    if (blockIdx.x == 0) { stats[c] = mu; stats[C + c] = rs; }
+    bn_sm[c] = mu; bn_sm[C + c] = rs;
+  }
+}
 __global__ __launch_bounds__(256) void bn_silu_apply_kernel(BnFwdJob j0, BnFwdJob j1, double invM, double unbias, size_t n4, int C, int training, int iters,
                                                             unsigned c4_mul) {
   SAST_KERNARG_WARM_SELF(bn_silu_apply_kernel);
@@ -74,6 +109,42 @@
                            (v.w - mu.w) * rs.w * g.w + b.w);
     z.x *= sigmoid_hw(z.x); z.y *= sigmoid_hw(z.y); z.z *= sigmoid_hw(z.z); z.w *= sigmoid_hw(z.w);
     st4(y + m * ldy + c, z);
+  }
+}
+struct BnUpDst { float* cat; const float* b; int C2, H, W; unsigned nmain, n4b; };
+__global__ __launch_bounds__(256) void bn_silu_apply_up_kernel(BnFwdJob jb, BnUpDst u, double invM, double unbias, unsigned n4, int C, int iters,
+                                                               unsigned c4_mul) {
+  extern __shared__ float bn_sm[];
+  const int Ct = C + u.C2;
+  if (blockIdx.x >= u.nmain) {
+    const unsigned e0 = (blockIdx.x - u.nmain) * 256u * iters + threadIdx.x, c4b = (unsigned)(u.C2 / 4);
+    for (int it = 0; it < iters; ++it) {
+      const unsigned e = e0 + it * 256u;
+      if (e >= u.n4b) return;
+      const unsigned row = e / c4b; const int c = (int)(e - row * c4b) * 4;
+      st4(u.cat + (size_t)row * Ct + C + c, ld4(u.b + (size_t)row * u.C2 + c));
+    }
+    return;
+  }
+  const float* __restrict__ x = jb.x; const float* __restrict__ gamma = jb.gamma; const float* __restrict__ beta = jb.beta;
+  float* __restrict__ y = jb.y; float* __restrict__ cat = u.cat;
+  const int c4 = C / 4;
+  const unsigned e0 = blockIdx.x * 256u * iters + threadIdx.x;
+  bn_fwd_stats(jb, invM, unbias, C, 1, bn_sm);
+  __syncthreads();
+  for (int it = 0; it < iters; ++it) {
+    const unsigned e = e0 + it * 256u;
+    if (e >= n4) return;
+    const unsigned m = fast_div((int)e, c4, c4_mul); const int c = (int)(e - m * c4) * 4;
+    const float4 v = ld4(x + (size_t)m * C + c), g = ld4(gamma + c), b = ld4(beta + c);
+    const float4 mu = *(const float4*)(bn_sm + c), rs = *(const float4*)(bn_sm + C + c);
+    float4 z = make_float4((v.x - mu.x) * rs.x * g.x + b.x, (v.y - mu.y) * rs.y * g.y + b.y, (v.z - mu.z) * rs.z * g.z + b.z,
+                           (v.w - mu.w) * rs.w * g.w + b.w);
+    z.x *= sigmoid_hw(z.x); z.y *= sigmoid_hw(z.y); z.z *= sigmoid_hw(z.z); z.w *= sigmoid_hw(z.w);
+    st4(y + (size_t)m * C + c, z);
+    const unsigned t = m / (unsigned)u.W, px = m - t * (unsigned)u.W, bb = t / (unsigned)u.H, py = t - bb * (unsigned)u.H;
+    float* q = cat + ((size_t)(bb * 2 * u.H + 2 * py) * (2 * u.W) + 2 * px) * Ct + c;
+    st4(q, z); st4(q + Ct, z); st4(q + (size_t)2 * u.W * Ct, z); st4(q + (size_t)(2 * u.W + 1) * Ct, z);
   }
 }
 struct EpBnSilu {
@@ -289,6 +360,51 @@
   const float4 r = ld4(dout + (base + 2 * W) * Ct + c), s = ld4(dout + (base + 2 * W + 1) * Ct + c);
   st4(da + (size_t)row * C1 + c, make_float4((p.x + q.x) + (r.x + s.x), (p.y + q.y) + (r.y + s.y), (p.z + q.z) + (r.z + s.z), (p.w + q.w) + (r.w + s.w)));
 }
+template <class IDX>
+__global__ __launch_bounds__(256) void upsample_cat_bwd_bn_kernel(const float* __restrict__ dout, float* __restrict__ da, float* __restrict__ db,
+                                                                  int H, int W, int C1, int Ct, size_t n4, size_t n4b, BnProducer p) {
+  extern __shared__ float ucb_red[];
+  const size_t e64 = (size_t)blockIdx.x * 256 + threadIdx.x;
+  const bool has_a = (size_t)blockIdx.x * 256 < n4;
+  if (has_a) {
+    for (int c = threadIdx.x; c < 2 * C1; c += 256) ucb_red[c] = 0.f;
+    __syncthreads();
+  }
+  if (e64 >= n4) {
+    const size_t eb64 = e64 - n4;
+    if (eb64 < n4b) {
+      const IDX eb = (IDX)eb64;
+      const int C2 = Ct - C1;
+      const IDX c4b = (IDX)(C2 / 4);
+      const IDX row = eb / c4b; const int c = (int)(eb - row * c4b) * 4;
+      st4(db + (size_t)row * C2 + c, ld4(dout + (size_t)row * Ct + C1 + c));
+    }
+  } else {
+    const IDX e = (IDX)e64;
+    const IDX c4n = (IDX)(C1 / 4);
+    const IDX row = e / c4n; const int c = (int)(e - row * c4n) * 4;
+    const IDX t = row / (IDX)W; const int x = (int)(row - t * (IDX)W); const IDX bb = t / (IDX)H; const int y = (int)(t - bb * (IDX)H);
+    const size_t base = (((size_t)bb * 2 * H + 2 * y) * 2 * W + 2 * x);
+    const float4 xc = ld4(p.x + (size_t)row * C1 + c);
+    const float4 mu = ld4(p.stats + c), rs = ld4(p.stats + C1 + c), gm = ld4(p.gamma + c), bt = ld4(p.beta + c);
+    const float4 pp = ld4(dout + base * Ct + c), q = ld4(dout + (base + 1) * Ct + c);
+    const float4 r = ld4(dout + (base + 2 * W) * Ct + c), s = ld4(dout + (base + 2 * W + 1) * Ct + c);
+    const float4 d = make_float4((pp.x + q.x) + (r.x + s.x), (pp.y + q.y) + (r.y + s.y), (pp.z + q.z) + (r.z + s.z), (pp.w + q.w) + (r.w + s.w));
+    st4(da + (size_t)row * C1 + c, d);
+    float a[4] = {0.f, 0.f, 0.f, 0.f}, b[4] = {0.f, 0.f, 0.f, 0.f};
+    bn_stat(d.x, xc.x, BnCol{mu.x, rs.x, gm.x, bt.x}, a[0], b[0]);
+    bn_stat(d.y, xc.y, BnCol{mu.y, rs.y, gm.y, bt.y}, a[1], b[1]);
+    bn_stat(d.z, xc.z, BnCol{mu.z, rs.z, gm.z, bt.z}, a[2], b[2]);
+    bn_stat(d.w, xc.w, BnCol{mu.w, rs.w, gm.w, bt.w}, a[3], b[3]);
+#pragma unroll
+    for (int e2 = 0; e2 < 4; ++e2) { atomicAdd(&ucb_red[c + e2], a[e2]); atomicAdd(&ucb_red[C1 + c + e2], b[e2]); }
+  }
+  if (has_a) {
+    __syncthreads();
+    float* __restrict__ sums = p.sums + (size_t)(blockIdx.x % BN_STAT_COPIES) * 2 * C1;
+    for (int c = threadIdx.x; c < 2 * C1; c += 256) atomicAdd(sums + c, ucb_red[c]);
+  }
+}
 __global__ __launch_bounds__(256) void slice_copy_kernel(const float* __restrict__ src, int lds, int soff, float* __restrict__ dst,
                                                          int ldd, int doff, int Cs, size_t n4) {
   const size_t e = (size_t)blockIdx.x * 256 + threadIdx.x;
@@ -393,15 +509,16 @@
   if (!dx) return gemm_tn(ta, tb, dw, K, Cout, K, M, st);
   const int parity = SAST_KNOB("SAST_CONVDX_PARITY", 1);
   const int Mc = g.B * (g.H / 2) * (g.W / 2);
-  if (prod && prod->x) {
-    if (g.stride != 1 || lddx != g.Cin || prod->C != g.Cin) return SAST_EINVAL;
+  const bool par = parity && g.stride == 2 && k == 3 && g.pad == 1 && g.H % 2 == 0 && g.W % 2 == 0 && Mc % 64 == 0;
+  if (prod && prod->x && (lddx != g.Cin || prod->C != g.Cin || !(g.stride == 1 || (g.stride == 2 && k == 3)))) return SAST_EINVAL;
+  if (prod && prod->x && !par) {
     if (Cout % 16 == 0)
       return gemm_pair(ta, tb, dw, K, Cout, K, M, nullptr, nullptr, LdConvDxU{{dconv, g, Cout, Cout, shift}},
                        LdWeightConvDxU{{w, Cout, k * k, g.Cin, shift}}, EpStoreBnRed{dx, lddx, *prod}, g.B * g.H * g.W, g.Cin, k * k * Cout, nullptr, st, pair_tn_blocks_conv());
     return gemm_pair(ta, tb, dw, K, Cout, K, M, nullptr, nullptr, LdConvDx{dconv, g, Cout, Cout, shift},
                      LdWeightConvDx{w, Cout, k * k, g.Cin, shift}, EpStoreBnRed{dx, lddx, *prod}, g.B * g.H * g.W, g.Cin, k * k * Cout, nullptr, st, pair_tn_blocks_conv());
   }
-  if (!(parity && g.stride == 2 && k == 3 && g.pad == 1 && g.H % 2 == 0 && g.W % 2 == 0 && Mc % 64 == 0)) {
+  if (!par) {
     if (Cout % 16 == 0)
       return gemm_pair(ta, tb, dw, K, Cout, K, M, nullptr, nullptr, LdConvDxU{{dconv, g, Cout, Cout, shift}},
                        LdWeightConvDxU{{w, Cout, k * k, g.Cin, shift}}, EpStore{dx, lddx, nullptr}, g.B * g.H * g.W, g.Cin, k * k * Cout, nullptr, st, pair_tn_blocks_conv());
@@ -431,6 +548,10 @@
         }
     c.nslot[cls] = ny * nx;
   }
+  if (prod && prod->x)
+    return gemm_pair(ta, tb, dw, K, Cout, K, M, nullptr, nullptr, LdConvDxP{dconv, g, Cout, Cout, shift, c},
+                     LdWeightConvDxP{w, Cout, k * k, g.Cin, shift, g.KW, c}, EpStoreClassBnRed{dx, lddx, g.H, g.W, c, *prod}, 4 * Mc, g.Cin,
+                     4 * Cout, nullptr, st, pair_tn_blocks_conv());
   return gemm_pair(ta, tb, dw, K, Cout, K, M, nullptr, nullptr, LdConvDxP{dconv, g, Cout, Cout, shift, c},
                    LdWeightConvDxP{w, Cout, k * k, g.Cin, shift, g.KW, c}, EpStoreClass{dx, lddx, g.H, g.W, c}, 4 * Mc, g.Cin, 4 * Cout,
                    nullptr, st, pair_tn_blocks_conv());
@@ -558,7 +679,16 @@
   const size_t n4 = (size_t)M * (C / 4);
   int iters = (int)(n4 / (256 * 512));
   iters = iters < 1 ? 1 : (iters > 8 ? 8 : iters);
-  {
+  if (a->up_cat) {
+    const int C2 = a->up_C2;
+    const unsigned long long n4b = 4ull * M * (C2 / 4), ncat = 4ull * M * (C + C2);
+    if (!a->training || phase != 0 || !a->up_b || C2 < 4 || C2 % 4 || a->ldy != C || ncat >= (1ull << 31) || n4 + n4b >= (1ull << 31)) return SAST_EINVAL;
+    const unsigned per = 256u * iters, nmain = (unsigned)((n4 + per - 1) / per), ncopy = (unsigned)((n4b + per - 1) / per);
+    const BnFwdJob jb{a->conv_out, sums, a->run_mean, a->run_var, a->stats, a->bn_w, a->bn_b, a->y, a->ldy, a->momentum, a->eps};
+    const BnUpDst u{a->up_cat, a->up_b, C2, g.Ho, g.Wo, nmain, (unsigned)n4b};
+    SAST_LAUNCH(bn_silu_apply_up_kernel, dim3(nmain + ncopy), dim3(256), sizeof(float) * 2 * C, st, jb, u, 1.0 / (double)M, bn_unbias(M), (unsigned)n4, C,
+                       iters, div_mul_of((unsigned)(C / 4), n4));
+  } else {
     const BnFwdJob jb{a->conv_out, sums, a->run_mean, a->run_var, a->stats, a->bn_w, a->bn_b, a->y, a->ldy, a->momentum, a->eps};
     SAST_LAUNCH(bn_silu_apply_kernel, dim3((unsigned)((n4 + 256 * iters - 1) / (256 * iters)), 1), dim3(256), sizeof(float) * 2 * C, st,
                        jb, jb, 1.0 / (double)(phase == 2 ? a->m_total : M), bn_unbias(phase == 2 ? a->m_total : M), n4, C, a->training, iters,
@@ -602,7 +732,7 @@
     SAST_CHECK_LAUNCH();
     return SAST_OK;
   }
-  if (fold && (a->stride != 1 || (p1.x && !(p1.stats && p1.gamma && p1.beta && p1.sums)) || (p2.x && !(a->x2 && p2.stats && p2.gamma && p2.beta && p2.sums))))
+  if (fold && ((a->stride != 1 && !(a->stride == 2 && k == 3 && !a->x2 && !p2.x)) || (p1.x && !(p1.stats && p1.gamma && p1.beta && p1.sums)) || (p2.x && !(a->x2 && p2.stats && p2.gamma && p2.beta && p2.sums))))
     return SAST_EINVAL;
   if (k == 1 && a->stride == 1 && a->x2) {
     const LdRowsT2 tb{a->x, a->ldx, a->Cin1, a->x2, a->ldx2};
@@ -743,6 +873,21 @@
   SAST_CHECK_LAUNCH();
   return SAST_OK;
 }
+int sast_upsample_cat_bwd_bn(const float* dout, float* da, float* db, int B, int H, int W, int C1, int C2, const SastBnProducer* prod,
+                             sast_stream_t stream) { SAST_ENTRY();
+  hipStream_t st = (hipStream_t)stream;
+  if (!prod || !prod->conv_out) return sast_upsample_cat_bwd(dout, da, db, B, H, W, C1, C2, stream);
+  if (C1 % 4 || C2 % 4 || prod->C != C1 || !prod->stats || !prod->bn_w || !prod->bn_b || !prod->bn_ws || C1 > 4096) return SAST_EINVAL;
+  const BnProducer p{prod->conv_out, prod->stats, prod->bn_w, prod->bn_b, prod->bn_ws + 4 * BN_STAT_COPIES * C1, C1};
+  const size_t n4 = (size_t)B * H * W * (C1 / 4), n4b = (size_t)B * 4 * H * W * (C2 / 4);
+  const size_t lds = sizeof(float) * 2 * C1;
+  if (n4 + n4b < (1ull << 32)) SAST_LAUNCH(upsample_cat_bwd_bn_kernel<unsigned>, dim3((unsigned)((n4 + n4b + 255) / 256)), dim3(256), lds, st, dout, da, db, H, W,
+                     C1, C1 + C2, n4, n4b, p);
+  else SAST_LAUNCH(upsample_cat_bwd_bn_kernel<size_t>, dim3((unsigned)((n4 + n4b + 255) / 256)), dim3(256), lds, st, dout, da, db, H, W, C1, C1 + C2,
+                     n4, n4b, p);
+  SAST_CHECK_LAUNCH();
+  return SAST_OK;
+}
 int sast_cat2_fwd(const float* a, const float* b, float* out, int rows, int C1, int C2, sast_stream_t stream) { SAST_ENTRY();
   hipStream_t st = (hipStream_t)stream;
   if (C1 % 4 || C2 % 4) return SAST_EINVAL;
diff --git a/sast_amd/csrc/k_rows.hip b/sast_amd/csrc/k_rows.hip
--- a/sast_amd/csrc/k_rows.hip
+++ b/sast_amd/csrc/k_rows.hip
@@ -870,12 +870,90 @@
     st4(dx + 4 * i, make_float4(k * v.x, k * v.y, k * v.z, k * v.w));
   }
 }
+struct MsqBn { const float* x[4]; const float* stats[4]; const float* gamma[4]; const float* beta[4]; float* sums[4]; int C[4]; };
+__device__ __forceinline__ void msq_bn_stat(float dy, float x, float mu, float rs, float g, float b, float& s, float& q) {
+  const float xh = (x - mu) * rs;
+  const float z = xh * g + b, sg = sigmoid_hw(z);
+  const float dz = dy * sg * (1.f + z * (1.f - sg));
+  s += dz; q += dz * xh;
+}
+__global__ __launch_bounds__(1024) void mean_square_bwd_bn_kernel(MsqJob j, MsqBn p, const float* __restrict__ g, int g_stride) {
+  extern __shared__ float msq_red[];
+  const int t = blockIdx.y;
+  const float* __restrict__ x = j.x[t];
+  float* __restrict__ dx = j.dx[t];
+  const size_t n4 = j.n[t] / 4;
+  const float k = 2.f * g[(size_t)(t * gridDim.x + blockIdx.x) * g_stride] / (float)j.n[t];
+  const float* __restrict__ cx = p.x[t];
+  if (!cx) {
+    for (size_t i = (size_t)blockIdx.x * 1024 + threadIdx.x; i < n4; i += (size_t)gridDim.x * 1024) {
+      const float4 v = ld4(x + 4 * i);
+      st4(dx + 4 * i, make_float4(k * v.x, k * v.y, k * v.z, k * v.w));
+    }
+    return;
+  }
+  const int C = p.C[t], c4n = C / 4;
+  const float* __restrict__ stats = p.stats[t]; const float* __restrict__ gamma = p.gamma[t]; const float* __restrict__ beta = p.beta[t];
+  for (int c = threadIdx.x; c < 2 * C; c += 1024) msq_red[c] = 0.f;
+  __syncthreads();
+  const bool fixed = ((size_t)gridDim.x * 1024) % (size_t)c4n == 0;
+  float s[4] = {0.f, 0.f, 0.f, 0.f}, q[4] = {0.f, 0.f, 0.f, 0.f};
+  int c = (int)(((size_t)blockIdx.x * 1024 + threadIdx.x) % (size_t)c4n) * 4;
+  float4 mu = ld4(stats + c), rs = ld4(stats + C + c), gm = ld4(gamma + c), bt = ld4(beta + c);
+  for (size_t i = (size_t)blockIdx.x * 1024 + threadIdx.x; i < n4; i += (size_t)gridDim.x * 1024) {
+    if (!fixed) {
+      c = (int)(i % (size_t)c4n) * 4;
+      mu = ld4(stats + c); rs = ld4(stats + C + c); gm = ld4(gamma + c); bt = ld4(beta + c);
+    }
+    const float4 v = ld4(x + 4 * i), xc = ld4(cx + 4 * i);
+    const float4 d = make_float4(k * v.x, k * v.y, k * v.z, k * v.w);
+    st4(dx + 4 * i, d);
+    msq_bn_stat(d.x, xc.x, mu.x, rs.x, gm.x, bt.x, s[0], q[0]);
+    msq_bn_stat(d.y, xc.y, mu.y, rs.y, gm.y, bt.y, s[1], q[1]);
+    msq_bn_stat(d.z, xc.z, mu.z, rs.z, gm.z, bt.z, s[2], q[2]);
+    msq_bn_stat(d.w, xc.w, mu.w, rs.w, gm.w, bt.w, s[3], q[3]);
+    if (!fixed) {
+#pragma unroll
+      for (int e = 0; e < 4; ++e) { atomicAdd(&msq_red[c + e], s[e]); atomicAdd(&msq_red[C + c + e], q[e]); s[e] = 0.f; q[e] = 0.f; }
+    }
+  }
+  if (fixed) {
+    const bool shuf = c4n <= 64 && (c4n & (c4n - 1)) == 0;
+    if (shuf) {
+      for (int off = c4n; off < 64; off <<= 1) {
+#pragma unroll
+        for (int e = 0; e < 4; ++e) { s[e] += __shfl_xor(s[e], off, 64); q[e] += __shfl_xor(q[e], off, 64); }
+      }
+    }
+    if (!shuf || (int)(threadIdx.x & 63) < c4n) {
+#pragma unroll
+      for (int e = 0; e < 4; ++e) { atomicAdd(&msq_red[c + e], s[e]); atomicAdd(&msq_red[C + c + e], q[e]); }
+    }
+  }
+  __syncthreads();
+  float* __restrict__ sums = p.sums[t] + (size_t)(blockIdx.x % SAST_BN_STAT_COPIES) * 2 * C;
+  for (int cc = threadIdx.x; cc < 2 * C; cc += 1024) atomicAdd(sums + cc, msq_red[cc]);
+}
 int mean_square_launch(const float* const* x, float* const* dx, const size_t* n, int count, int blocks, float* partials,
-                       const float* g, int g_stride, hipStream_t st) {
+                       const float* g, int g_stride, hipStream_t st, const SastBnProducer* prods) {
   MsqJob j{};
   for (int t = 0; t < count; ++t) { j.x[t] = x[t]; j.dx[t] = dx ? dx[t] : nullptr; j.n[t] = n[t]; }
   if (!dx) SAST_LAUNCH(mean_square_fwd_kernel, dim3(blocks, count), dim3(1024), 0, st, j, partials);
-  else SAST_LAUNCH(mean_square_bwd_kernel, dim3(blocks, count), dim3(1024), 0, st, j, g, g_stride);
+  else if (!prods) SAST_LAUNCH(mean_square_bwd_kernel, dim3(blocks, count), dim3(1024), 0, st, j, g, g_stride);
+  else {
+    MsqBn p{};
+    int cmax = 0;
+    for (int t = 0; t < count; ++t) {
+      const SastBnProducer& h = prods[t];
+      if (!h.conv_out) continue;
+      if (!h.stats || !h.bn_w || !h.bn_b || !h.bn_ws || h.C < 4 || h.C % 4 || n[t] % (size_t)h.C) return SAST_EINVAL;
+      p.x[t] = h.conv_out; p.stats[t] = h.stats; p.gamma[t] = h.bn_w; p.beta[t] = h.bn_b; p.C[t] = h.C;
+      p.sums[t] = h.bn_ws + 4 * SAST_BN_STAT_COPIES * h.C;
+      cmax = h.C > cmax ? h.C : cmax;
+    }
+    if (cmax > 4096) return SAST_EINVAL;
+    SAST_LAUNCH(mean_square_bwd_bn_kernel, dim3(blocks, count), dim3(1024), sizeof(float) * 2 * cmax, st, j, p, g, g_stride);
+  }
   SAST_CHECK_LAUNCH();
   return SAST_OK;
 }
diff --git a/sast_amd/csrc/kernels.h b/sast_amd/csrc/kernels.h
--- a/sast_amd/csrc/kernels.h
+++ b/sast_amd/csrc/kernels.h
@@ -36,7 +36,7 @@
 int mask_token_bwd_launch(const float* dy, const unsigned char* mask, float* dx, float* dtoken, int rows, int C, hipStream_t st);
 int colsum_launch(const float* x, int ld, const int* idx, int rows, const int* drows, int C, float* out, hipStream_t st);
 int mean_square_launch(const float* const* x, float* const* dx, const size_t* n, int count, int blocks, float* partials,
-                       const float* g, int g_stride, hipStream_t st);
+                       const float* g, int g_stride, hipStream_t st, const SastBnProducer* prods = nullptr);
 int ls_linear_finish_launch(const float* w, const float* b, const float* gamma, const float* raw, const float* s, float* dw,
                             float* db, float* dgamma, int C, int K, hipStream_t st);
 int ls_linear_finish2_launch(const float* w0, const float* b0, const float* g0, const float* raw0, const float* s0, float* dw0, float* db0,
diff --git a/sast_amd/detection/network_blocks.py b/sast_amd/detection/network_blocks.py
--- a/sast_amd/detection/network_blocks.py
+++ b/sast_amd/detection/network_blocks.py
@@ -41,6 +41,22 @@
             else:
                 bn.num_batches_tracked.add_(1)
         return y
+
+    def forward_up_cat_nhwc(self, x, b, arena=None, sole=False):
+        bn = self.bn
+        ws = arena.take(SF.bn_ws_floats(bn.num_features)) if arena is not None else None
+        sync = self.sync_group()
+        if sync is not None and arena is None and self.training and sync.active():
+            x0 = x[0] if isinstance(x, (tuple, list)) else x
+            sync.exchange_batch(x0.shape[0], x0.device)
+        out = SF.conv_bn_silu_up_cat(x, b, self.conv.weight, bn.weight, bn.bias, bn.running_mean, bn.running_var, self.ksize, self.stride,
+                                     self.training, bn.momentum, bn.eps, ws, sole_consumer=sole, sync=sync)
+        if self.training and bn.num_batches_tracked is not None:
+            if arena is not None:
+                arena.counters.append(bn.num_batches_tracked)
+            else:
+                bn.num_batches_tracked.add_(1)
+        return out
 
     def sync_item(self, x, arena=None, sole=False, two_outputs=False):
         bn = self.bn
diff --git a/sast_amd/detection/yolo_head.py b/sast_amd/detection/yolo_head.py
--- a/sast_amd/detection/yolo_head.py
+++ b/sast_amd/detection/yolo_head.py
@@ -50,7 +50,8 @@
             for conv in list(self.cls_preds) + list(self.obj_preds):
                 conv.bias.fill_(-math.log((1 - prior_prob) / prior_prob))
 
-    def forward_train_nhwc(self, feats, labels):
+    def forward_train_nhwc(self, feats, labels, sole_feats=False):
+        sole_feats = bool(sole_feats) and SF.BN_FOLD_MULTI
         per_level, levels = [], []
         if not hasattr(self, "_bn_floats"):
             self._bn_floats = bn_scratch_floats(self)
@@ -70,7 +71,7 @@
                 levels.append((x.shape[1], x.shape[2], stride))
         else:
             for k, (x, stride) in enumerate(zip(feats, self.strides)):
-                x = self.stems[k].forward_nhwc(x, ar)
+                x = self.stems[k].forward_nhwc(x, ar, sole=sole_feats)
                 if SF.CONV_PAIR and not sync and not self.depthwise:
                     c0, r0 = self.cls_convs[k][0], self.reg_convs[k][0]
                     args = [(c.conv.weight, c.bn.weight, c.bn.bias, c.bn.running_mean, c.bn.running_var, c.bn.momentum, c.bn.eps) for c in (c0, r0)]
diff --git a/sast_amd/detection/yolo_pafpn.py b/sast_amd/detection/yolo_pafpn.py
--- a/sast_amd/detection/yolo_pafpn.py
+++ b/sast_amd/detection/yolo_pafpn.py
@@ -40,14 +40,14 @@
         token = None
         if grp is not None and grp.active():
             token = grp.exchange_batch(x0.shape[0], x0.device)
-        fpn_out0, fpn_out0b = self.lateral_conv0.forward_nhwc(x0, ar, two_outputs=True)
-        f_out0 = self.C3_p4.forward_nhwc(SF.upsample_cat(fpn_out0, x1), ar, sole_input=True)
-        fpn_out1, fpn_out1b = self.reduce_conv1.forward_nhwc(f_out0, ar, sole=True, two_outputs=True)
-        pan_out2, pan_out2b = self.C3_p3.forward_nhwc(SF.upsample_cat(fpn_out1, x2), ar, sole_input=True, two_outputs=True)
-        p_out1 = (self.bu_conv2.forward_nhwc(pan_out2b, ar), fpn_out1b)
-        pan_out1, pan_out1b = self.C3_n3.forward_nhwc(p_out1, ar, sole_input=(True, False), two_outputs=True)
-        p_out0 = (self.bu_conv1.forward_nhwc(pan_out1b, ar), fpn_out0b)
-        pan_out0 = self.C3_n4.forward_nhwc(p_out0, ar, sole_input=(True, False))
+        fpn_out0b, up0 = self.lateral_conv0.forward_up_cat_nhwc(x0, x1, ar)
+        f_out0 = self.C3_p4.forward_nhwc(up0, ar, sole_input=True)
+        fpn_out1b, up1 = self.reduce_conv1.forward_up_cat_nhwc(f_out0, x2, ar, sole=True)
+        pan_out2, pan_out2b = self.C3_p3.forward_nhwc(up1, ar, sole_input=True, two_outputs=True)
+        p_out1 = (self.bu_conv2.forward_nhwc(pan_out2b, ar, sole=True), fpn_out1b)
+        pan_out1, pan_out1b = self.C3_n3.forward_nhwc(p_out1, ar, sole_input=True, two_outputs=True)
+        p_out0 = (self.bu_conv1.forward_nhwc(pan_out1b, ar, sole=True), fpn_out0b)
+        pan_out0 = self.C3_n4.forward_nhwc(p_out0, ar, sole_input=True)
         ar.finish()
         if token is not None:
             pan_out2._sast_sync_pass = pan_out1._sast_sync_pass = pan_out0._sast_sync_pass = token
diff --git a/sast_amd/functional.py b/sast_amd/functional.py
--- a/sast_amd/functional.py
+++ b/sast_amd/functional.py
@@ -261,7 +261,7 @@
 
 class _MeanSquares(torch.autograd.Function):
     @staticmethod
-    def forward(ctx, *xs):
+    def forward(ctx, prods, *xs):
         _need_gpu(*xs)
         xs = tuple(x.contiguous() for x in xs)
         k = len(xs)
@@ -270,6 +270,7 @@
         partials = torch.empty(k * MEAN_SQUARE_BLOCKS, device=xs[0].device, dtype=torch.float32)
         L.check(L.lib().sast_mean_square_fwd(ptrs, ns, k, partials.data_ptr(), _stream()), "mean_square_fwd")
         ctx.save_for_backward(*xs)
+        ctx.prods = tuple(h.join() if (h is not None and x.numel() % h.cout == 0) else None for h, x in zip(prods, xs))
         return partials
 
     @staticmethod
@@ -285,14 +286,26 @@
         ptrs = (C.c_void_p * k)(*[x.data_ptr() for x in xs])
         dptrs = (C.c_void_p * k)(*[d.data_ptr() for d in dxs])
         ns = (C.c_size_t * k)(*[x.numel() for x in xs])
-        L.check(L.lib().sast_mean_square_bwd(ptrs, ns, k, g.data_ptr(), g_stride, dptrs, _stream()), "mean_square_bwd")
-        return dxs
-
-
-def mean_squares(*xs: torch.Tensor) -> torch.Tensor:
+        served = [h if (h is not None and h.ready()) else None for h in ctx.prods]
+        if any(h is not None for h in served):
+            ps = (L.SastBnProducer * k)(*[h.c_struct() if h is not None else L.SastBnProducer() for h in served])
+            L.check(L.lib().sast_mean_square_bwd_bn(ptrs, ns, k, g.data_ptr(), g_stride, dptrs, ps, _stream()), "mean_square_bwd_bn")
+            for h in served:
+                if h is not None:
+                    h.add()
+        else:
+            L.check(L.lib().sast_mean_square_bwd(ptrs, ns, k, g.data_ptr(), g_stride, dptrs, _stream()), "mean_square_bwd")
+        return (None,) + dxs
+
+
+def mean_squares(*xs: torch.Tensor, sole: bool = False) -> torch.Tensor:
     if not 1 <= len(xs) <= 4 or any(x.dtype != torch.float32 or x.numel() % 4 for x in xs):
         raise ValueError("mean_squares: 1..4 fp32 tensors with numel % 4 == 0")
-    return _MeanSquares.apply(*xs).sum()
+    prods = [None] * len(xs)
+    if sole and BN_FOLD and BN_FOLD_MULTI and torch.is_grad_enabled():
+        hs = [getattr(x, "_sast_bn", None) for x in xs]
+        prods = [h if (h is not None and h.wide and x.is_contiguous()) else None for h, x in zip(hs, xs)]
+    return _MeanSquares.apply(tuple(prods), *xs).sum()
 
 
 class _AddRows(torch.autograd.Function):
@@ -870,12 +883,28 @@
 
 
 class BnHandle:
-    __slots__ = ("conv_out", "stats", "bn_w", "bn_b", "bn_ws", "cout", "red_done")
-
-    def __init__(self):
+    __slots__ = ("conv_out", "stats", "bn_w", "bn_b", "bn_ws", "cout", "red_done", "consumers", "folders", "got", "wide")
+
+    def __init__(self, consumers=1, wide=False):
         self.conv_out = self.stats = self.bn_w = self.bn_b = self.bn_ws = None
         self.cout = -1
         self.red_done = False
+        self.consumers, self.folders, self.got, self.wide = int(consumers), 0, 0, bool(wide)
+
+    def join(self):
+        self.folders += 1
+        return self
+
+    def ready(self):
+        return self.folders == self.consumers and self.got < self.consumers
+
+    def add(self):
+        self.got += 1
+        self.red_done = True
+
+    def c_struct(self):
+        return _fill(L.SastBnProducer(), conv_out=self.conv_out, stats=self.stats, bn_w=self.bn_w, bn_b=self.bn_b, bn_ws=self.bn_ws,
+                     C=self.cout)
 
     def fill(self, conv_out, stats, bn_w, bn_b, bn_ws, cout):
         self.conv_out, self.stats, self.bn_w, self.bn_b, self.bn_ws, self.cout = conv_out, stats, bn_w, bn_b, bn_ws, cout
@@ -1039,11 +1068,14 @@
     B, H, W, Cin, Cin1, Cout, ksize, stride = st["meta"][:8]
     own = handle.fill(conv_out, stats, bn_w, bn_b, bn_ws, Cout) if (training and handle is not None) else None
     p1, p2 = producers if (training and stride == 1 and st["groups"] == 1) else (None, None)
+    if training and stride == 2 and ksize == 3 and st["groups"] == 1 and x2 is None and BN_FOLD_MULTI and producers[0] is not None and \
+            producers[0].wide:
+        p1 = producers[0]
     if p1 is not None and p1.cout != Cin1:
         p1 = None
     if p2 is not None and (x2 is None or p2.cout != Cin - Cin1):
         p2 = None
-    return own, (p1, p2)
+    return own, tuple(h.join() if h is not None else None for h in (p1, p2))
 
 
 def _cbs_bwd_args(saved, params, meta, groups, own, producers, need1, need2, dy, dy2):
@@ -1060,11 +1092,8 @@
     dx = torch.empty_like(x) if need else None
     dx2 = torch.empty_like(x2) if (need and x2 is not None) else None
     ws = torch.empty(M * Cout, device=x.device)
-    p1, p2 = producers if need else (None, None)
-    if p1 is not None and p1.red_done:
-        p1 = None
-    if p2 is not None and (p2.red_done or dx2 is None):
-        p2 = None
+    served = tuple(h if (h is not None and h.ready()) else None for h in producers)
+    p1, p2 = served if need else (None, None)
     pk = {}
     for pre, h in (("p_", p1), ("p2_", p2)):
         if h is not None:
@@ -1076,14 +1105,16 @@
               eps=eps, x=x, w=w, bn_w=bn_w, bn_b=bn_b, conv_out=conv_out, stats=stats, dy=dy, dx=_ptr(dx), dw=pg[0],
               d_bn_w=pg[1], d_bn_b=pg[2], bn_ws=bn_ws, ws=ws, x2=_ptr(x2), dx2=_ptr(dx2), Cin1=Cin1, ldx2=Cin - Cin1, dy2=_ptr(dy2),
               groups=groups, **pk)
-    return a, dx, dx2, pg, (p1, p2), (dy, dy2, ws)
+    return a, dx, dx2, pg, served, (dy, dy2, ws)
 
 
 class _ConvBnSilu(torch.autograd.Function):
     @staticmethod
     def forward(ctx, x, x2, w, bn_w, bn_b, run_mean, run_var, ksize, stride, training, momentum, eps, bn_ws, producers, handle, two_y,
-                sync=None):
+                sync=None, up=None):
         a, st = _cbs_fwd_args(x, x2, w, bn_w, bn_b, run_mean, run_var, ksize, stride, training, momentum, eps, bn_ws)
+        if up is not None:
+            _fill(a, up_cat=up[0], up_b=up[1], up_C2=up[1].shape[-1])
         M, B, Cout = st["meta"][11], st["meta"][0], st["meta"][5]
         bn_ws = st["saved"][4]
         m_total = 0
@@ -1118,8 +1149,8 @@
         _dw_hold((ctx.saved_tensors, _keep, pg))
         for h in served:
             if h is not None:
-                h.red_done = True
-        return (dx, dx2) + pg.out() + (None,) * 12
+                h.add()
+        return (dx, dx2) + pg.out() + (None,) * 13
 
 
 _CBS_UNIT_IN = 7
@@ -1176,7 +1207,7 @@
             L.check(L.lib().sast_conv_bn_silu_bwd(C.byref(a), _stream()), "conv_bn_silu_bwd")
             for h in served:
                 if h is not None:
-                    h.red_done = True
+                    h.add()
             grads.extend((dx, dx2) + pg.out() + (None, None))
         _dw_hold((sv, jobs))
         return tuple(grads)
@@ -1258,7 +1289,7 @@
             p1 = None
         if p2 is not None and (x2 is None or p2.cout != Cin - Cin1):
             p2 = None
-        ctx.producers = (p1, p2)
+        ctx.producers = tuple(h.join() if h is not None else None for h in (p1, p2))
         return ys[0], ys[1]
 
     @staticmethod
@@ -1273,11 +1304,8 @@
         dx = torch.empty_like(x) if need else None
         dx2 = torch.empty_like(x2) if (need and x2 is not None) else None
         dws = torch.empty(M, 2 * Cout, device=x.device)
-        p1, p2 = ctx.producers if need else (None, None)
-        if p1 is not None and p1.red_done:
-            p1 = None
-        if p2 is not None and (p2.red_done or dx2 is None):
-            p2 = None
+        served = tuple(h if (h is not None and h.ready()) else None for h in ctx.producers)
+        p1, p2 = served if need else (None, None)
         pk = {}
         for pre, h in (("p_", p1), ("p2_", p2)):
             if h is not None:
@@ -1292,9 +1320,9 @@
                   d_bn_w1=pg[4], d_bn_b0=pg[2], d_bn_b1=pg[5], ws0=dws, dx=_ptr(dx), dx2=_ptr(dx2), **pk)
         L.check(L.lib().sast_conv_bn_silu2_bwd(C.byref(a), _stream()), "conv_bn_silu2_bwd")
         _dw_hold((x, x2, co0, co1, st0, st1, ws0, ws1, dy0, dy1, dws, pg))
-        for h in (p1, p2):
+        for h in served:
             if h is not None:
-                h.red_done = True
+                h.add()
         g = pg.out()
         return (dx, dx2) + g[0:3] + (None, None) + g[3:6] + (None,) * 11
 
@@ -1345,6 +1373,8 @@
 TWO_OUT = os.environ.get("SAST_TWO_OUT", "1") != "0"
 CONV_PAIR = os.environ.get("SAST_CONV_PAIR", "1") != "0"
 BN_FOLD = os.environ.get("SAST_BN_FOLD", "1") != "0"
+BN_FOLD_MULTI = os.environ.get("SAST_BN_FOLD_MULTI", "1") != "0"
+UP_CAT_FUSED = os.environ.get("SAST_UP_CAT_FUSED", "1") != "0"
 SYNC_BN_GROUPS = os.environ.get("SAST_SYNC_BN_GROUPS", "1") != "0"
 
 
@@ -1355,14 +1385,21 @@
         sync = None
     if two_outputs and (not TWO_OUT or not training or not torch.is_grad_enabled()):
         y = conv_bn_silu(x_nhwc, w, bn_w, bn_b, run_mean, run_var, ksize, stride, training, momentum, eps, bn_ws, sole_consumer, sync=sync)
+        if getattr(y, "_sast_bn", None) is not None:
+            y._sast_bn.consumers = 2
         return y, y
     if not training and not (torch.is_grad_enabled() and any(t is not None and t.requires_grad for t in (x, x2, w, bn_w, bn_b))):
         return _conv_bn_silu_infer(x, x2, w, bn_w, bn_b, run_mean, run_var, ksize, stride, float(eps))
     prods = _producers(x, x2, sole_consumer)
+    wide = BN_FOLD and BN_FOLD_MULTI and sync is None
     if two_outputs:
-        return _ConvBnSilu.apply(x, x2, w, bn_w, bn_b, run_mean, run_var, ksize, stride, True, float(momentum), float(eps), bn_ws, prods,
-                                 None, True, sync)
-    handle = BnHandle() if training else None
+        handle = BnHandle(consumers=2, wide=True) if wide else None
+        ys = _ConvBnSilu.apply(x, x2, w, bn_w, bn_b, run_mean, run_var, ksize, stride, True, float(momentum), float(eps), bn_ws, prods,
+                               handle, True, sync)
+        if handle is not None:
+            ys[0]._sast_bn = ys[1]._sast_bn = handle
+        return ys
+    handle = BnHandle(wide=wide) if training else None
     y = _ConvBnSilu.apply(x, x2, w, bn_w, bn_b, run_mean, run_var, ksize, stride, bool(training), float(momentum), float(eps), bn_ws, prods,
                           handle, False, sync)
     if handle is not None:
@@ -1395,15 +1432,20 @@
 
 class _UpsampleCat(torch.autograd.Function):
     @staticmethod
-    def forward(ctx, a, b):
+    def forward(ctx, a, b, prod=None, built=None):
         _need_gpu(a, b)
         a, b = a.contiguous(), b.contiguous()
         B, H, W, C1 = a.shape
         C2 = b.shape[-1]
         assert b.shape[:3] == (B, 2 * H, 2 * W)
-        out = torch.empty(B, 2 * H, 2 * W, C1 + C2, device=a.device)
-        L.check(L.lib().sast_upsample_cat_fwd(a.data_ptr(), b.data_ptr(), out.data_ptr(), B, H, W, C1, C2, _stream()), "upsample_cat_fwd")
+        if built is not None:
+            out = built[0]
+            assert out.shape == (B, 2 * H, 2 * W, C1 + C2)
+        else:
+            out = torch.empty(B, 2 * H, 2 * W, C1 + C2, device=a.device)
+            L.check(L.lib().sast_upsample_cat_fwd(a.data_ptr(), b.data_ptr(), out.data_ptr(), B, H, W, C1, C2, _stream()), "upsample_cat_fwd")
         ctx.meta = (B, H, W, C1, C2)
+        ctx.prod = prod.join() if (prod is not None and prod.cout == C1) else None
         return out
 
     @staticmethod
@@ -1412,12 +1454,44 @@
         dout = dout.contiguous()
         da = torch.empty(B, H, W, C1, device=dout.device)
         db = torch.empty(B, 2 * H, 2 * W, C2, device=dout.device)
-        L.check(L.lib().sast_upsample_cat_bwd(dout.data_ptr(), da.data_ptr(), db.data_ptr(), B, H, W, C1, C2, _stream()), "upsample_cat_bwd")
-        return da, db
-
-
-def upsample_cat(a, b):
-    return _UpsampleCat.apply(a, b)
+        h = ctx.prod
+        if h is not None and h.ready():
+            ps = h.c_struct()
+            L.check(L.lib().sast_upsample_cat_bwd_bn(dout.data_ptr(), da.data_ptr(), db.data_ptr(), B, H, W, C1, C2, C.byref(ps), _stream()),
+                    "upsample_cat_bwd_bn")
+            h.add()
+        else:
+            L.check(L.lib().sast_upsample_cat_bwd(dout.data_ptr(), da.data_ptr(), db.data_ptr(), B, H, W, C1, C2, _stream()), "upsample_cat_bwd")
+        return da, db, None, None
+
+
+def upsample_cat(a, b, sole_a=False):
+    h = getattr(a, "_sast_bn", None) if (sole_a and BN_FOLD and BN_FOLD_MULTI) else None
+    return _UpsampleCat.apply(a, b, h if (h is not None and h.wide) else None, None)
+
+
+def conv_bn_silu_up_cat(x_nhwc, b, w, bn_w, bn_b, run_mean, run_var, ksize, stride, training, momentum=0.1, eps=1e-5, bn_ws=None,
+                        sole_consumer=False, sync=None):
+    if sync is not None and not (training and sync.active()):
+        sync = None
+    x, x2 = x_nhwc if isinstance(x_nhwc, (tuple, list)) else (x_nhwc, None)
+    if not (UP_CAT_FUSED and TWO_OUT and training and sync is None and torch.is_grad_enabled() and b.dtype == torch.float32):
+        y, yb = conv_bn_silu(x_nhwc, w, bn_w, bn_b, run_mean, run_var, ksize, stride, training, momentum, eps, bn_ws, sole_consumer,
+                             two_outputs=True, sync=sync)
+        return yb, upsample_cat(y, b, sole_a=True)
+    _need_gpu(b)
+    b = b.contiguous()
+    pad = (ksize - 1) // 2
+    Ho, Wo = (x.shape[1] + 2 * pad - ksize) // stride + 1, (x.shape[2] + 2 * pad - ksize) // stride + 1
+    if b.shape[:3] != (x.shape[0], 2 * Ho, 2 * Wo) or b.shape[-1] % 4:
+        raise RuntimeError("sast_amd: conv_bn_silu_up_cat needs a second source of twice the conv's output size")
+    cat = torch.empty(x.shape[0], 2 * Ho, 2 * Wo, w.shape[0] + b.shape[-1], device=x.device)
+    handle = BnHandle(consumers=2, wide=True) if (BN_FOLD and BN_FOLD_MULTI) else None
+    y, yb = _ConvBnSilu.apply(x, x2, w, bn_w, bn_b, run_mean, run_var, ksize, stride, True, float(momentum), float(eps), bn_ws,
+                              _producers(x, x2, sole_consumer), handle, True, None, (cat, b.detach()))
+    if handle is not None:
+        y._sast_bn = yb._sast_bn = handle
+    return yb, _UpsampleCat.apply(y, b, handle, (cat,))
 
 
 class _Cat2(torch.autograd.Function):
diff --git a/sast_amd/training.py b/sast_amd/training.py
--- a/sast_amd/training.py
+++ b/sast_amd/training.py
@@ -86,10 +86,10 @@
             leaves = {k: v.detach().requires_grad_(True) for k, v in fpn_in.items()}
         outs = self.fpn.forward_nhwc(leaves if leaves is not None else fpn_in)
         if labels is not None:
-            _pred, self.losses = self.head.forward_train_nhwc(outs, labels)
+            _pred, self.losses = self.head.forward_train_nhwc(outs, labels, sole_feats=True)
             loss = self.losses["loss"]
         else:
-            loss = SF.mean_squares(*outs)
+            loss = SF.mean_squares(*outs, sole=True)
         self.loss, self.P, self.states = loss, Ps[-1], states
         self._seg_state = (loss, fpn_in, leaves, cut)
         return loss
```

Measured after the change: 862.9 frames/s, median of 6. Within noise of the previous version (+0.4%).
